# chrischoy/DeepGlobalRegistration

Measured on AMD Instinct MI355X. Metric: pair registrations/sec (FCGF x2 + 1-NN + 6-D inlier net + gate + weighted Procrustes + SE(3) refinement), higher is better.
Workload: dtype f32 results via 2 x f16 split operands (3 f16 MFMA products per MAC, f32 accumulate); k = 1 convs, kNN re-evaluation and registration in exact f32, SVD in f64

## Files before the change

### deepglobalregistration_amd/_lib.py

```python
import ctypes as C
import os
import threading

import torch

_HERE = os.path.dirname(os.path.abspath(__file__))
LIB_PATH = os.environ.get('DGR_HIP_LIB') or os.path.join(_HERE, 'lib', 'libdgr_hip.so')

DGR_OK, DGR_EINVAL, DGR_EHIP, DGR_ENOMEM, DGR_ESVD, DGR_EINTERNAL = 0, -1, -2, -3, -4, -5
STATUS_OK, STATUS_LOW_CONFIDENCE, STATUS_SVD_FAILED, STATUS_SAFEGUARD = 0, 1, 2, 3
STATUS_FLAG_ICP_SKIPPED, STATUS_MASK = 0x100, 0xff

c_i32p, c_i64p, c_f32p, c_f64p = (C.POINTER(C.c_int32), C.POINTER(C.c_int64),
                                  C.POINTER(C.c_float), C.POINTER(C.c_double))
vp = C.c_void_p


class WeightDesc(C.Structure):
    _fields_ = [('name', C.c_char_p), ('data', vp), ('numel', C.c_int64)]


class Params(C.Structure):
    _fields_ = [('clip_weight_thresh', C.c_float), ('voxel_size', C.c_float),
                ('inlier_feature_type', C.c_int), ('max_iter', C.c_int),
                ('max_break_count', C.c_int), ('break_threshold_ratio', C.c_double),
                ('skip_refinement', C.c_int), ('safeguard', C.c_int), ('ransac_hypotheses', C.c_int64),
                ('ransac_seed', C.c_uint32), ('use_icp', C.c_int)]


class PgParams(C.Structure):
    _fields_ = [('mu', C.c_double), ('reference_node', C.c_int), ('max_iter', C.c_int), ('rel_tol', C.c_double)]


SIGNATURES = {
    'dgr_last_error': (C.c_char_p, []),
    'dgr_version': (C.c_char_p, []),
    'dgr_ctx_create': (C.c_int, [C.c_int, C.POINTER(vp)]),
    'dgr_ctx_destroy': (None, [vp]),
    'dgr_ctx_workspace_bytes': (C.c_int64, [vp]),
    'dgr_ctx_create_partition_stream': (C.c_int, [vp, C.c_int, C.c_int, C.POINTER(vp)]),
    'dgr_voxelize': (C.c_int, [vp, vp, C.c_int, C.c_int64, C.c_double, C.c_int32, vp, vp, vp, c_i64p, vp]),
    'dgr_net_create': (C.c_int, [vp, C.c_int, C.c_int, C.c_int, C.c_int, C.c_int,
                                 C.POINTER(WeightDesc), C.c_int, C.POINTER(vp)]),
    'dgr_net_create_device': (C.c_int, [vp, C.c_int, C.c_int, C.c_int, C.c_int, C.c_int,
                                        C.POINTER(WeightDesc), C.c_int, C.POINTER(vp)]),
    'dgr_net_destroy': (None, [vp]),
    'dgr_net_param_bytes': (C.c_int64, [vp]),
    'dgr_net_share': (C.c_int, [vp, vp, C.POINTER(vp)]),
    'dgr_net_sharers': (C.c_int, [vp]),
    'dgr_resunet_forward': (C.c_int, [vp, vp, vp, vp, C.c_int64, vp, vp]),
    'dgr_net_get_intermediate': (C.c_int, [vp, vp, C.c_char_p, vp, C.c_int64, c_i64p, c_i64p]),
    'dgr_net_get_tensor': (C.c_int, [vp, vp, C.c_char_p, C.c_int, vp, C.c_int64, c_i64p, c_i64p]),
    'dgr_net_layer_stats': (C.c_int, [vp, vp, C.c_int, c_i64p]),
    'dgr_net_num_layers': (C.c_int, [vp]),
    'dgr_net_rerun_layer': (C.c_int, [vp, vp, C.c_int, C.c_int, c_f32p, c_f32p]),
    'dgr_maps_create': (C.c_int, [vp, vp, C.c_int64, C.c_int, C.c_int, C.POINTER(vp), vp]),
    'dgr_maps_destroy': (None, [vp]),
    'dgr_maps_get_coords': (C.c_int, [vp, C.c_int, vp, C.c_int64, c_i64p]),
    'dgr_maps_get_kernel_map': (C.c_int, [vp, C.c_int, C.c_int, vp, C.c_int64, vp, vp, C.c_int64,
                                          c_i64p, c_i64p]),
    'dgr_maps_create_ex': (C.c_int, [vp, vp, C.c_int64, C.c_int, C.c_int, C.c_int, C.POINTER(vp), vp]),
    'dgr_maps_get_raw': (C.c_int, [vp, C.c_char_p, C.c_int, C.c_char_p, vp, C.c_int64, c_i64p, c_i64p]),
    'dgr_knn1_l2': (C.c_int, [vp, vp, C.c_int64, vp, C.c_int64, C.c_int, C.c_int, vp, vp, vp]),
    'dgr_knn1_l2_batch': (C.c_int, [vp, vp, c_i64p, vp, c_i64p, C.c_int, C.c_int, C.c_int, vp, vp, vp]),
    'dgr_knn_l2': (C.c_int, [vp, vp, C.c_int64, vp, C.c_int64, C.c_int, C.c_int, C.c_int, vp, vp, vp]),
    'dgr_knn_l2_batch': (C.c_int, [vp, vp, c_i64p, vp, c_i64p, C.c_int, C.c_int, C.c_int, C.c_int, vp, vp,
                                   vp]),
    'dgr_inlier_inputs': (C.c_int, [vp, vp, vp, C.c_int64, vp, vp, C.c_int64, vp, C.c_int, vp, vp, vp]),
    'dgr_sigmoid_clip_sum': (C.c_int, [vp, vp, C.c_int64, C.c_float, vp, c_f64p, vp]),
    'dgr_gather_rows3': (C.c_int, [vp, vp, vp, C.c_int64, vp, vp]),
    'dgr_weighted_procrustes': (C.c_int, [vp, vp, vp, vp, C.c_int64, C.c_float, c_f32p, c_f32p, vp]),
    'dgr_se3_refine': (C.c_int, [vp, vp, vp, vp, C.c_int64, C.c_float, C.c_int, C.c_int, C.c_double,
                                 c_f32p, c_f32p, c_i32p, c_f32p, c_i32p, vp]),
    'dgr_register_batch': (C.c_int, [vp, vp, vp, vp, vp, c_i64p, vp, vp, c_i64p, C.c_int,
                                     C.POINTER(Params), vp, vp, c_f32p, c_i32p, c_f32p, vp]),
    'dgr_register_pairs': (C.c_int, [vp, vp, vp, vp, vp, c_i64p, C.c_int, C.c_int, c_i32p, C.c_int,
                                     C.POINTER(Params), vp, vp, c_f32p, c_i32p, c_f32p, vp]),
    'dgr_register_batch_f64': (C.c_int, [vp, c_f64p, C.c_int64, c_i64p]),
    'dgr_register_batch_output': (C.c_int, [vp, C.c_int, vp, C.c_int64, c_i64p, vp]),
    'dgr_ctx_set_profiling': (C.c_int, [vp, C.c_int]),
    'dgr_icp_point_to_point': (C.c_int, [vp, vp, C.c_int64, vp, C.c_int64, C.c_double, c_f64p, C.c_int, C.c_double,
                                          C.c_double, c_f64p, c_f64p, vp]),
    'dgr_ransac_correspondence': (C.c_int, [vp, vp, vp, C.c_int64, C.c_double, C.c_int64, C.c_uint32, c_f64p, c_f64p, vp]),
    'dgr_ctx_stage_times': (C.c_int, [vp, c_f32p]),
    'dgr_ctx_stage_times_v2': (C.c_int, [vp, c_f32p, C.c_int, C.POINTER(C.c_int)]),
    'dgr_ctx_conv_launches': (C.c_int64, [vp]),
    'dgr_ctx_conv_launch_times': (C.c_int, [vp, c_f32p, c_f32p, C.c_int64, C.POINTER(C.c_int64)]),
    'dgr_ctx_conv_launch_kernel_us': (C.c_int, [vp, c_f32p, C.c_int64, C.POINTER(C.c_int64)]),
    'dgr_ctx_conv_launch_kinds': (C.c_int, [vp, C.c_char_p, C.c_int64, C.POINTER(C.c_int64)]),
    'dgr_radius_pairs_batch': (C.c_int, [vp, vp, c_i64p, vp, c_i64p, C.c_int, c_f64p, C.c_double, C.c_int, vp, vp,
                                         C.c_int64, c_i64p, vp]),
    'dgr_pairs_isin_batch': (C.c_int, [vp, vp, c_i64p, vp, c_i64p, C.c_int, c_i64p, vp, vp]),
    'dgr_validation_counts': (C.c_int, [vp, vp, vp, C.c_float, c_i64p, C.c_int, c_i64p, vp]),
    'dgr_score_pairs': (C.c_int, [vp, vp, c_i64p, C.c_int, c_i32p, C.c_int, c_f64p, C.c_double, c_f64p, vp]),
    'dgr_pose_graph_optimize': (C.c_int, [vp, C.c_int, c_i64p, c_i64p, c_i32p, c_f64p, c_f64p, C.POINTER(C.c_uint8), c_f64p,
                                          C.POINTER(PgParams), c_f64p, c_f64p, c_f64p, vp]),
    'dgr_voxel_mean': (C.c_int, [vp, vp, C.c_int, c_i64p, C.c_int, c_i32p, C.c_int, c_f64p, c_f64p, C.c_double, vp, vp, vp, vp,
                                 vp, c_i64p, c_i64p, vp]),
    'dgr_tsdf_fragment': (C.c_int, [vp, vp, C.c_int, C.c_int, C.c_int, c_f64p, c_f64p, c_f64p, C.c_double, C.c_double,
                                    C.c_double, C.c_double, C.c_int, C.c_int, C.c_int, vp, C.c_int64, vp, vp, vp, C.c_int64,
                                    c_i64p, c_i64p, c_i64p, vp]),
    'dgr_tsdf_mesh': (C.c_int, [vp, vp, C.c_int64, vp, vp, C.c_int, C.c_double, C.c_int, vp, vp, C.c_int64, vp, C.c_int64,
                                c_i64p, c_i64p, vp]),
    'dgr_debug_ortho2rotation': (C.c_int, [vp, vp, C.c_int64, vp, vp, vp, vp]),
    'dgr_debug_se3_refine_from': (C.c_int, [vp, vp, vp, vp, C.c_int64, C.c_float, C.c_int, C.c_int, C.c_double,
                                            c_f64p, c_f64p, vp]),
    'dgr_debug_smooth_l1': (C.c_int, [vp, vp, vp, C.c_int64, C.c_float, vp, vp]),
    'dgr_debug_conv_layer': (C.c_int, [vp, vp, C.c_int, vp, vp, C.c_int, C.c_int64, vp, vp]),
}

_lib = None


def load():
    global _lib
    if _lib is not None:
        return _lib
    if not os.path.exists(LIB_PATH):
        raise RuntimeError(
            f'{LIB_PATH} not found: the HIP extension is not built.  Run '
            '`python -c "import __graft_entry__ as g; g.build()"` (or `make -C '
            'deepglobalregistration_amd/csrc`).  There is no CPU fallback.')
    lib = C.CDLL(LIB_PATH)
    for name, (res, args) in SIGNATURES.items():
        fn = getattr(lib, name)
        fn.restype = res
        fn.argtypes = args
    _lib = lib
    return lib


class DgrError(RuntimeError):
    def __init__(self, code, message):
        super().__init__(f'libdgr_hip error {code}: {message}')
        self.code = code


class DgrInvalidArgument(DgrError, ValueError):

    def __init__(self, message):
        RuntimeError.__init__(self, f'libdgr_hip: {message}')
        self.code = DGR_EINVAL


def check(rc):
    if rc == DGR_OK:
        return
    msg = load().dgr_last_error().decode('utf-8', 'replace')
    if rc == DGR_EINVAL:
        raise DgrInvalidArgument(msg)
    raise DgrError(rc, msg)


_ctxs = {}
_tls = threading.local()


def new_ctx(device):
    lib = load()
    device = torch.device(device)
    idx = device.index if device.index is not None else torch.cuda.current_device()
    h = vp()
    check(lib.dgr_ctx_create(idx, C.byref(h)))
    return h


def use_ctx(handle):
    _tls.ctx = handle


def get_ctx(device=None):
    lib = load()
    if getattr(_tls, 'ctx', None) is not None:
        return _tls.ctx
    if not torch.cuda.is_available():
        raise RuntimeError('deepglobalregistration_amd needs a ROCm GPU (torch.cuda.is_available() is '
                           'False); there is no CPU fallback')
    if device is None:
        idx = torch.cuda.current_device()
    else:
        device = torch.device(device)
        if device.type != 'cuda':
            raise RuntimeError(f'deepglobalregistration_amd runs on the GPU only, got device {device}')
        idx = device.index if device.index is not None else torch.cuda.current_device()
    if idx not in _ctxs:
        h = vp()
        check(lib.dgr_ctx_create(idx, C.byref(h)))
        _ctxs[idx] = h
    return _ctxs[idx]


def stream_ptr(device_index=None):
    return vp(torch.cuda.current_stream(device_index).cuda_stream)


def ptr(t):
    if t is None:
        return vp(0)
    assert t.is_contiguous(), 'tensor must be contiguous'
    return vp(t.data_ptr())
```

### deepglobalregistration_amd/csrc/dgr_internal.h

```cpp
#pragma once
#include <hip/hip_runtime.h>
#include <stdint.h>
#include <stdio.h>
#include <stdlib.h>
#include <string>
#include <vector>

#include "../../include/dgr_hip.h"

void dgr_set_error(const char *fmt, ...);

#define DGR_HIP_CHECK(expr)                                                                  \
  do {                                                                                       \
    hipError_t _e = (expr);                                                                  \
    if (_e != hipSuccess) {                                                                  \
      dgr_set_error("%s:%d: %s failed: %s", __FILE__, __LINE__, #expr, hipGetErrorString(_e)); \
      return DGR_EHIP;                                                                       \
    }                                                                                        \
  } while (0)

#define DGR_CHECK(expr)          \
  do {                           \
    int _r = (expr);             \
    if (_r != DGR_OK) return _r; \
  } while (0)

#define DGR_REQUIRE(cond, ...)     \
  do {                             \
    if (!(cond)) {                 \
      dgr_set_error(__VA_ARGS__);  \
      return DGR_EINVAL;           \
    }                              \
  } while (0)

#define DGR_LAUNCH_CHECK() DGR_HIP_CHECK(hipGetLastError())

inline bool dgr_exact_f32() {
  static const bool on = getenv("DGR_EXACT_F32") != nullptr;
  return on;
}

struct DgrArena {
  struct Chunk {
    char *base;
    size_t size;
  };
  std::vector<Chunk> chunks;
  size_t cur = 0;
  size_t offset = 0;
  size_t high_water = 0, used_total = 0;
  uint64_t generation = 0;

  struct Mark {
    size_t cur, offset, used_total;
  };
  Mark mark() const { return {cur, offset, used_total}; }
  void rewind(const Mark &m) { cur = m.cur; offset = m.offset; used_total = m.used_total; }
  void *alloc(size_t bytes);
  int reset();
  void release();
  size_t reserved() const;
  template <typename T>
  T *get(size_t n) {
    return static_cast<T *>(alloc(n * sizeof(T)));
  }
};

#define DGR_ALLOC(ptr, arena, T, n)                       \
  do {                                                    \
    (ptr) = (arena).get<T>((size_t)(n) > 0 ? (size_t)(n) : 1); \
    if (!(ptr)) return DGR_ENOMEM;                        \
  } while (0)

constexpr int DGR_TILE_M = 64;

struct DgrCoordMap {
  int32_t *coords = nullptr;
  int32_t *n_dev = nullptr;
  int64_t n_cap = 0;
  int ts = 1;
  int32_t *table = nullptr;
  uint32_t table_mask = 0;
  int32_t *canon = nullptr;
};

struct DgrHalfBuckets {
  int32_t *bkeys = nullptr;
  int32_t *table = nullptr;
  uint32_t mask = 0;
  int32_t *start = nullptr;
  int4 *second = nullptr;
  bool built = false;
};

struct DgrKernelMap {
  int K = 0;
  int32_t *rule_ptr = nullptr;
  int32_t *tile_ptr = nullptr;
  int4 *tile_desc = nullptr;
  int64_t tile_cap = 0;
  int32_t *pair_in = nullptr;
  int32_t *pair_out = nullptr;
  int32_t *out_ptr = nullptr, *out_pos = nullptr;
  uint16_t *pair_k = nullptr;
  int32_t *in_ptr = nullptr, *in_pos = nullptr;
  int64_t pair_cap = 0;
  bool built = false;
};

constexpr int DGR_OS_ROWS = 64;
struct DgrNbrTable {
  int32_t *nbr = nullptr;
  int64_t n_pad = 0;
  int K = 27;
  bool built = false;
  int32_t *perm = nullptr, *cls_count = nullptr;
  int64_t cls_cap = 0;
};

struct DgrMapSet {
  int D = 3, nc = 4, conv1_ks = 3;
  bool use_nbr = false;
  DgrNbrTable nsame[4];
  DgrNbrTable ndown[3];
  DgrNbrTable nup[3];
  DgrCoordMap cm[4];
  DgrHalfBuckets hb[4];
  DgrKernelMap same[4];
  DgrKernelMap conv1;
  DgrKernelMap down[3];
  int32_t *overflow = nullptr;
};

int dgr_build_maps(DgrArena &arena, const int32_t *coords, int64_t N, int D, int conv1_ks,
                   DgrMapSet *ms, hipStream_t stream, bool skip_conv1_map = false, bool lean = false,
                   bool nbr_tables = false);
int dgr_nbr_counts(const DgrNbrTable &t, const int32_t *n_out_dev, int64_t counts[27]);
int dgr_conv1_probe(DgrArena &arena, const DgrCoordMap &cm, int ks, const float *in, int in_ld, int cin,
                    const float *w_tiled, const float *shift, float *out, int out_ld, int32_t *pair_count,
                    hipStream_t stream, const float *w_compact = nullptr, const char **kernel_name = nullptr,
                    uint32_t *out_amax = nullptr);
constexpr int32_t DGR_ROW_DROPPED = -1, DGR_ROW_PENDING = -2;
int dgr_unique_rows(DgrArena &arena, const int32_t *keys, int64_t n, int nc, const int32_t *state, int32_t *held,
                    int32_t *first_flag, int32_t *rank, int32_t *n_unique_dev, int32_t **table_out, uint32_t *mask_out,
                    hipStream_t stream);
int dgr_exclusive_scan_i32(DgrArena &arena, const int32_t *in, int32_t *out, int64_t n,
                           int32_t *total_out, hipStream_t stream);
constexpr int DGR_SCAN_MAX = 24;
int dgr_exclusive_scan_multi(DgrArena &arena, int count, const int32_t *const *in, int32_t *const *out, const int64_t *n,
                             int32_t *const *total_out, hipStream_t stream);

struct DgrConvLaunch {
  const float *in;
  int in_ld;
  int in_relu;
  float *out;
  int out_ld;
  float *y;
  const float *shift;
  const float *w;
  int cin, cin_pad, cout, cout_pad, K;
  const int32_t *pair_in, *pair_out, *tile_ptr, *rule_ptr;
  const int4 *tile_desc;
  const int32_t *n_rows_dev;
  int64_t tile_bound;
  int l2_normalize = 0;
  unsigned long long *clk = nullptr;
};
int dgr_conv_launch(const DgrConvLaunch &a, int num_cus, hipStream_t stream, const char **kernel_name = nullptr);
struct DgrSplitRows {
  unsigned char *planes = nullptr;
  float *scale = nullptr;
  int channels = 0;
};
bool dgr_conv_wide_supported(int cin_pad, int cin, int cout);
int dgr_conv_wide_launch(const DgrConvLaunch &a, const DgrSplitRows &in, const void *wb, int64_t piece_stride,
                         float w_unscale, int num_cus, hipStream_t stream, const char **kernel_name = nullptr);
int dgr_row_amax(const float *in, int in_ld, int cin, int relu, const int32_t *n_dev, int64_t n_cap, uint32_t *out,
                 hipStream_t stream);
int dgr_split_rows(const float *in, int in_ld, int relu, const int32_t *n_dev, int64_t n_cap, const DgrSplitRows &out,
                   hipStream_t stream);
int dgr_reduce_rows(const float *y, int cout, const int32_t *ptr, const int32_t *pos, const int32_t *n_dev,
                    int64_t n_cap, float *out, int out_ld, const float *shift, const float *res, int res_ld,
                    int res_relu, hipStream_t stream, const DgrSplitRows *split = nullptr, int out_relu = 0);
int dgr_conv_small_cin(const float *in, int in_ld, int in_relu, int cin, const float *w_tiled, const float *w_quad,
                       const float *shift, const DgrKernelMap &km, const int32_t *n_out_dev, int64_t n_out_cap, float *out,
                       int out_ld, hipStream_t stream);
struct DgrConvOsLaunch {
  const float *in; int in_ld, in_relu;
  float *out; int out_ld, out_relu;
  const float *w16, *shift;
  const void *wb3; int64_t piece_stride;
  const void *wbd = nullptr;
  const uint32_t *row_amax = nullptr; float w_unscale = 1.f;
  uint32_t *out_amax = nullptr, *out_amax2 = nullptr;
  int64_t n_in_cap = 0;
  const float *res; int res_ld, res_relu;
  int rows_per_block;
  int phase_channels = 64;
  const DgrNbrTable *nbr;
  const int32_t *n_out_dev;
  int64_t n_out_cap;
  int cin, cin_pad, cout;
  bool dense = false;
  bool up = false;
  const unsigned char *in_dsplit = nullptr;
  unsigned char *out_dsplit = nullptr;
};
inline bool dgr_fits_32bit_offsets(int64_t rows, int64_t ld) { return rows * ld * 4 < (1ll << 31); }
int dgr_conv_os_launch(const DgrConvOsLaunch &a, hipStream_t stream, const char **kernel_name = nullptr);
bool dgr_conv_dense_supported(int cin, int cin_pad, int cout);
int dgr_conv_dense_launch(const DgrConvOsLaunch &a, hipStream_t stream, const char **kernel_name = nullptr);
bool dgr_conv_up_supported(int cin, int cin_pad, int cout);
int dgr_conv_up_launch(const DgrConvOsLaunch &a, hipStream_t stream, const char **kernel_name = nullptr);
int dgr_l2_normalize_rows(const float *in, int in_ld, float *out, int out_ld, int c, int relu,
                          const int32_t *n_dev, int64_t n_cap, hipStream_t stream);

struct DgrBatchOutputs {
  const void *ptr[5] = {nullptr, nullptr, nullptr, nullptr, nullptr};
  int64_t numel[5] = {0, 0, 0, 0, 0};
  uint64_t generation = 0;
};

struct DgrEventPool {
  std::vector<hipEvent_t> ev;
  size_t used = 0;
  hipEvent_t next();
  void release();
};

struct dgr_ctx {
  int device = 0;
  int num_cus = 256;
  DgrArena arena;
  bool profiling = false;
  float stage_ms[9] = {0, 0, 0, 0, 0, 0, 0, 0, 0};
  int64_t conv_launches = 0;
  DgrBatchOutputs last;
  std::vector<double> last_T64;
  DgrEventPool events;
  std::vector<std::pair<hipEvent_t, hipEvent_t>> conv_spans, gemm_spans, map3_spans, map6_spans;
  std::vector<float> conv_span_ms, gemm_span_ms;
  std::vector<unsigned long long *> conv_clks;
  std::vector<float> conv_clk_us;
  std::vector<const char *> conv_kinds;
  int32_t *flag_dev = nullptr;
  hipEvent_t wait_ev = nullptr;
  long last_wait_ns = 0;
  double batch_ns_per_row = 0;
  double pairs_ns_per_row = 0;
  unsigned char *pin = nullptr;
  size_t pin_bytes = 0;
  hipStream_t part_stream = nullptr;
  int all_cus = 256;
};

int dgr_ctx_pinned(dgr_ctx *ctx, size_t bytes, unsigned char **out);
int dgr_flag_error(int32_t flag);

int dgr_ctx_wait(dgr_ctx *ctx, hipStream_t stream, long predicted_ns = 0);

int dgr_resunet_forward_impl(dgr_ctx *ctx, dgr_net *net, const int32_t *coords, const float *feats,
                             int64_t N, float *out, hipStream_t stream);
int dgr_ctx_collect_profile(dgr_ctx *ctx);
void dgr_ctx_begin_profile(dgr_ctx *ctx);

int dgr_knn1_batch_impl(dgr_ctx *ctx, const float *F0, const int64_t *off0, const float *F1, const int64_t *off1,
                        int npairs, int C, int squared, int64_t *idx_out, float *dist_out, hipStream_t stream);
int dgr_knn1_impl(dgr_ctx *ctx, const float *F0, int64_t N0, const float *F1, int64_t N1, int C,
                  int squared, int64_t *idx_out, float *dist_out, hipStream_t stream);
int dgr_inlier_inputs_impl(const int32_t *coords0, const float *xyz0, int64_t N0,
                           const int32_t *coords1, const float *xyz1, const int64_t *idx1,
                           int feature_type, int32_t *coords6, float *feats, hipStream_t stream);
int dgr_icp_impl(dgr_ctx *ctx, const float *src, int64_t N0, const float *dst, int64_t N1, double max_dist,
                 const double *T_init, int max_iter, double rel_fitness, double rel_rmse, double *T_out,
                 double *stats_out, hipStream_t stream);
int dgr_ransac_impl(dgr_ctx *ctx, const float *X, const float *Y, int64_t N, double max_dist, int64_t num_hypotheses,
                    uint32_t seed, double *T_out, double *stats_out, hipStream_t stream);
struct DgrIcpJob {
  const float *src = nullptr, *dst = nullptr;
  int64_t N0 = 0, N1 = 0;
  double max_dist = 0;
  int nblocks = 0;
  void *st = nullptr;
  double *P = nullptr, *sorted = nullptr, *partial = nullptr;
  int32_t ncell = 0;
  double host_state[64];
};
int dgr_icp_begin(dgr_ctx *ctx, const float *src, int64_t N0, const float *dst, int64_t N1, double max_dist,
                  const double *T_init_dev , DgrIcpJob *job, hipStream_t stream);
int dgr_icp_run(dgr_ctx *ctx, DgrIcpJob *job, int max_iter, double rel_fitness, double rel_rmse, hipStream_t stream);
void dgr_icp_finish(const DgrIcpJob *job, double *T_out, double *stats_out);
constexpr int DGR_RANSAC_RESULT_DOUBLES = 19;
int dgr_ransac_begin(dgr_ctx *ctx, const float *X, const float *Y, int64_t N, double max_dist, int64_t num_hypotheses,
                     uint32_t seed, double **result_dev, hipStream_t stream);
struct DgrRegResult {
  float R[9];
  float t[3];
  float loss;
  float wsum;
  int32_t iterations;
  int32_t break_count;
  int32_t status;
  int32_t pad;
};
static inline int64_t dgr_ceil_div(int64_t a, int64_t b) { return (a + b - 1) / b; }
```

### deepglobalregistration_amd/csrc/kmap.hip

```cpp
#include <string.h>

#include <algorithm>

#include "dgr_internal.h"
#include "hash.h"

constexpr int KM_THREADS = 256;

template <int D>
__device__ __forceinline__ void offset_of(int k, int ks, int ts, int32_t *delta) {
  const int half = ks >> 1;
#pragma unroll
  for (int d = 0; d < D; ++d) {
    delta[d] = ((k % ks) - half) * ts;
    k /= ks;
  }
}

template <int D>
__device__ __forceinline__ int probe(const int32_t *__restrict__ out_coords, int64_t o,
                                     const int32_t *delta, const int32_t *__restrict__ in_coords,
                                     const int32_t *__restrict__ in_table, uint32_t in_mask) {
  constexpr int NC = D + 1;
  int32_t q[NC];
// ... 504 lines not shown
}

struct Kmap6Job {
  const DgrCoordMap *in, *out;
  const DgrHalfBuckets *hb;
  const DgrHalfBuckets *hb_out;
  bool need_in_csr, want_pair_out, want_pair_k;
  DgrKernelMap *km;
};
static int build_kernel_maps6(DgrArena &arena, const Kmap6Job *jobs, int nj, int max_pairs_per_row, int32_t *overflow,
                              hipStream_t stream) {
  constexpr int K = 729, KW = (K + 31) / 32;
  DGR_REQUIRE(nj >= 1 && nj <= KM_MAXJOBS, "6-D kernel maps: %d jobs", nj);
  struct Tr {
    int RB, symmetric;
    int64_t n_cap, n_in_cap, hit_waves;
    int32_t *counts, *base, *total, *cnt_out, *cnt_in;
    uint32_t *mask_out, *mask_in;
    int4 *cell;
    HitList hl;
    unsigned short *wpre_out, *wpre_in;
  } t[KM_MAXJOBS];
  for (int m = 0; m < nj; ++m) {
    const Kmap6Job &J = jobs[m];
    t[m].n_cap = J.out->n_cap; t[m].n_in_cap = J.in->n_cap;
    DGR_REQUIRE(t[m].n_cap < (1ll << 27) && t[m].n_in_cap < (1ll << 27), "6-D kernel maps: more than 2^27 rows");
    DGR_CHECK(alloc_kernel_map(arena, K, t[m].n_cap, t[m].n_in_cap, max_pairs_per_row, J.need_in_csr, J.want_pair_out,
                               J.want_pair_k, J.km));
  }
  DgrArena::Mark mk = arena.mark();
  {
    size_t words = 0;
    for (int m = 0; m < nj; ++m)
      words += (size_t)(t[m].n_cap + 1) * KW + (jobs[m].need_in_csr ? (size_t)(t[m].n_in_cap + 1) * KW : 0) + (size_t)(t[m].n_cap + 1);
    uint32_t *pool;
    DGR_ALLOC(pool, arena, uint32_t, words);
    DGR_HIP_CHECK(hipMemsetAsync(pool, 0, words * sizeof(uint32_t), stream));
    for (int m = 0; m < nj; ++m) {
      t[m].mask_out = pool; pool += (size_t)(t[m].n_cap + 1) * KW;
      t[m].mask_in = nullptr;
      if (jobs[m].need_in_csr) { t[m].mask_in = pool; pool += (size_t)(t[m].n_in_cap + 1) * KW; }
      t[m].cnt_out = reinterpret_cast<int32_t *>(pool); pool += (size_t)(t[m].n_cap + 1);
    }
  }
  for (int m = 0; m < nj; ++m) {
    const Kmap6Job &J = jobs[m];
    Tr &r = t[m];
    r.RB = (int)dgr_ceil_div(r.n_cap, KM_THREADS);
    r.symmetric = (J.in->coords == J.out->coords && !J.need_in_csr) ? 1 : 0;
    DGR_REQUIRE(J.hb && J.hb->built && J.hb_out && J.hb_out->built, "6-D kernel map: first-half buckets missing");
    DGR_ALLOC(r.counts, arena, int32_t, (int64_t)K * r.RB);
    DGR_ALLOC(r.base, arena, int32_t, (int64_t)K * r.RB);
    DGR_ALLOC(r.total, arena, int32_t, 1);
    r.cnt_in = nullptr;
    if (J.need_in_csr) DGR_ALLOC(r.cnt_in, arena, int32_t, r.n_in_cap + 1);
    DGR_ALLOC(r.cell, arena, int4, (int64_t)r.RB * (KM_THREADS / 64) * K);
    const int64_t search_blocks = dgr_ceil_div(r.n_cap * (r.symmetric ? 14 : 27), KM_THREADS);
    r.hit_waves = search_blocks * (KM_THREADS / 64);
    r.hl.region = (J.in->ts >= 8 && r.symmetric) ? 2 * KM_REGION : KM_REGION / 2;
    DGR_REQUIRE(r.hit_waves < (1ll << 31), "6-D kernel map: too many search waves");
    DGR_ALLOC(r.hl.recs, arena, unsigned long long, r.hit_waves * r.hl.region);
    DGR_ALLOC(r.hl.wave_count, arena, int32_t, r.hit_waves);
    DGR_ALLOC(r.wpre_out, arena, unsigned short, (r.n_cap + 1) * KW);
    r.wpre_in = nullptr;
    if (J.need_in_csr) DGR_ALLOC(r.wpre_in, arena, unsigned short, (r.n_in_cap + 1) * KW);
  }
  static_assert(KM_JOBS6 >= KM_MAXJOBS, "multi-job launch tables");
  {
    Bits6Jobs bj = {};
    Colmask6Jobs cj = {};
    int max_sb = 0, max_rb = 0;
    for (int m = 0; m < nj; ++m) {
      const Kmap6Job &J = jobs[m];
      Tr &r = t[m];
      bj.pa[m] = PrunedArgs{J.out->coords, J.out->n_dev, J.hb_out->second, r.n_cap, *J.hb, J.in->ts, r.symmetric};
      bj.mask_out[m] = r.mask_out; bj.mask_in[m] = r.mask_in; bj.hl[m] = r.hl;
      bj.blocks[m] = (int)(r.hit_waves / (KM_THREADS / 64));
      max_sb = std::max(max_sb, bj.blocks[m]);
      cj.mask_out[m] = r.mask_out; cj.n_out_dev[m] = J.out->n_dev; cj.RB[m] = r.RB; cj.cell[m] = r.cell;
      cj.counts[m] = r.counts; cj.row_cnt[m] = r.cnt_out; cj.wpre[m] = r.wpre_out;
      max_rb = std::max(max_rb, r.RB);
    }
    kmap_bits_pruned6<<<dim3((unsigned)max_sb, (unsigned)nj), KM_THREADS, 0, stream>>>(bj, KW);
    kmap_colmask<<<dim3((unsigned)max_rb, (unsigned)nj), KM_THREADS, 0, stream>>>(cj, K, KW);
    {
      MaskCountJobs mj = {};
      int nm = 0;
      long long max_rows = 0;
      for (int m = 0; m < nj; ++m)
        if (jobs[m].need_in_csr) {
          mj.mask[nm] = t[m].mask_in; mj.n_dev[nm] = jobs[m].in->n_dev; mj.n_cap[nm] = t[m].n_in_cap + 1;
          mj.cnt[nm] = t[m].cnt_in; mj.wpre[nm] = t[m].wpre_in;
          max_rows = std::max(max_rows, mj.n_cap[nm]);
          ++nm;
        }
      static_assert(KM_MC_JOBS >= KM_MAXJOBS, "mask-count job table");
      if (nm) mask_count_multi<KW><<<dim3((unsigned)dgr_ceil_div(max_rows, 256), (unsigned)nm), 256, 0, stream>>>(mj);
    }
  }
  DGR_LAUNCH_CHECK();
  {
    const int32_t *ins[DGR_SCAN_MAX];
    int32_t *outs[DGR_SCAN_MAX], *tots[DGR_SCAN_MAX];
    int64_t ns[DGR_SCAN_MAX];
    int c = 0;
    for (int m = 0; m < nj; ++m) {
      ins[c] = t[m].cnt_out; outs[c] = jobs[m].km->out_ptr; tots[c] = nullptr; ns[c++] = t[m].n_cap + 1;
      ins[c] = t[m].counts; outs[c] = t[m].base; tots[c] = t[m].total; ns[c++] = (int64_t)K * t[m].RB;
      if (jobs[m].need_in_csr) { ins[c] = t[m].cnt_in; outs[c] = jobs[m].km->in_ptr; tots[c] = nullptr; ns[c++] = t[m].n_in_cap + 1; }
    }
    DGR_CHECK(dgr_exclusive_scan_multi(arena, c, ins, outs, ns, tots, stream));
  }
  FinalizeJobs fj = {};
  int64_t max_tiles = 0;
  for (int m = 0; m < nj; ++m) {
    finalize_job(fj, m, t[m].base, t[m].total, K, t[m].RB, jobs[m].km);
    max_tiles = std::max<int64_t>(max_tiles, jobs[m].km->tile_cap);
  }
  kmap_finalize<<<nj, 1024, 0, stream>>>(fj);
  tile_desc_kernel<<<dim3((unsigned)dgr_ceil_div(max_tiles, 256), nj), 256, 0, stream>>>(fj);
  {
    Place6Jobs pj = {};
    int max_pb = 0;
    for (int m = 0; m < nj; ++m) {
      const Kmap6Job &J = jobs[m];
      Tr &r = t[m];
      DgrKernelMap *km = J.km;
      pj.p[m] = PlaceArgs{K, KW, r.RB, r.mask_out, km->out_ptr, r.cell, r.base, km->pair_in, km->pair_out, km->pair_k, km->out_pos,
                          km->pair_cap, overflow, r.mask_in, km->in_ptr, km->in_pos, r.wpre_out, r.wpre_in};
      pj.replay[m] = PrunedArgs{J.out->coords, J.out->n_dev, J.hb_out->second, r.n_cap, *J.hb, J.in->ts, r.symmetric};
      pj.h[m] = r.hl;
      pj.n_waves[m] = (int)r.hit_waves;
      pj.blocks[m] = (int)std::min<int64_t>(dgr_ceil_div(r.hit_waves, KM_THREADS / 64), 16384);
      max_pb = std::max(max_pb, pj.blocks[m]);
      km->built = true;
    }
    kmap_place_hits<<<dim3((unsigned)max_pb, (unsigned)nj), KM_THREADS, 0, stream>>>(pj);
  }
  DGR_LAUNCH_CHECK();
  arena.rewind(mk);
  return DGR_OK;
}

constexpr int NBR_JOBS = 10;
struct NbrJobs {
  const int32_t *out_coords[NBR_JOBS], *n_out_dev[NBR_JOBS], *in_coords[NBR_JOBS], *in_table[NBR_JOBS];
  uint32_t in_mask[NBR_JOBS];
  int ts[NBR_JOBS];
  long long n_pad[NBR_JOBS];
  int32_t *nbr[NBR_JOBS];
};
__global__ void __launch_bounds__(KM_THREADS) nbr_search3(NbrJobs J) {
  const int jm = blockIdx.z;
  const int64_t n_pad = J.n_pad[jm];
  const int64_t o = (int64_t)blockIdx.x * KM_THREADS + threadIdx.x;
  if (o >= n_pad) return;
  int32_t *__restrict__ nbr = J.nbr[jm];
  const int kz = blockIdx.y;
  if (o >= *J.n_out_dev[jm]) {
#pragma unroll
    for (int u = 0; u < 9; ++u) nbr[(int64_t)(9 * kz + u) * n_pad + o] = -1;
    return;
  }
  const int sts = J.ts[jm];
  const int4 c = *reinterpret_cast<const int4 *>(J.out_coords[jm] + o * 4);
  int32_t q[9][4];
#pragma unroll
  for (int u = 0; u < 9; ++u) {
    q[u][0] = c.x;
    q[u][1] = c.y + ((u % 3) - 1) * sts;
    q[u][2] = c.z + ((u / 3) - 1) * sts;
    q[u][3] = c.w + (kz - 1) * sts;
  }
  int hit[9];
  dgr_lookup_many<4, 9>(J.in_table[jm], J.in_mask[jm], J.in_coords[jm], q, hit);
#pragma unroll
  for (int u = 0; u < 9; ++u) nbr[(int64_t)(9 * kz + u) * n_pad + o] = hit[u];
}

struct ClsJobs {
  const int32_t *coords[3], *n_dev[3];
  int ts[3], nb[3];
  int32_t *blk_cnt[3], *perm[3], *cls_count[3];
  long long cls_cap[3];
};
__device__ __forceinline__ int parity_class(const int32_t *coords, int64_t o, int ts) {
  const int4 c = *reinterpret_cast<const int4 *>(coords + o * 4);
  return ((c.y / ts) & 1) | (((c.z / ts) & 1) << 1) | (((c.w / ts) & 1) << 2);
}
__global__ void __launch_bounds__(KM_THREADS) cls_count_kernel(ClsJobs J) {
  __shared__ int wcnt[KM_THREADS / 64][8];
  const int l = blockIdx.y, b = blockIdx.x;
  if (b >= J.nb[l]) return;
  const int64_t o = (int64_t)b * KM_THREADS + threadIdx.x;
  const int cls = o < *J.n_dev[l] ? parity_class(J.coords[l], o, J.ts[l]) : 8;
#pragma unroll
  for (int c = 0; c < 8; ++c) {
    const unsigned long long m = __ballot(cls == c);
    if ((threadIdx.x & 63) == 0) wcnt[threadIdx.x >> 6][c] = __popcll(m);
  }
  __syncthreads();
  if (threadIdx.x < 8) {
    int n = 0;
    for (int w = 0; w < KM_THREADS / 64; ++w) n += wcnt[w][threadIdx.x];
    J.blk_cnt[l][b * 8 + threadIdx.x] = n;
  }
}
__global__ void __launch_bounds__(KM_THREADS) cls_fill_kernel(ClsJobs J) {
  __shared__ int part[KM_THREADS / 64][8], before[8], wcnt[KM_THREADS / 64][8];
  const int l = blockIdx.y, b = blockIdx.x;
  if (b >= J.nb[l]) return;
  const int lane = threadIdx.x & 63, wave = threadIdx.x >> 6;
  int acc[8] = {0, 0, 0, 0, 0, 0, 0, 0};
  for (int bb = threadIdx.x; bb < b; bb += KM_THREADS) {
    const int4 lo = *reinterpret_cast<const int4 *>(J.blk_cnt[l] + bb * 8), hi = *reinterpret_cast<const int4 *>(J.blk_cnt[l] + bb * 8 + 4);
    acc[0] += lo.x; acc[1] += lo.y; acc[2] += lo.z; acc[3] += lo.w;
    acc[4] += hi.x; acc[5] += hi.y; acc[6] += hi.z; acc[7] += hi.w;
  }
#pragma unroll
  for (int c = 0; c < 8; ++c) {
    int v = acc[c];
    for (int d = 32; d > 0; d >>= 1) v += __shfl_down(v, d, 64);
    if (lane == 0) part[wave][c] = v;
  }
  const int64_t o = (int64_t)b * KM_THREADS + threadIdx.x;
  const int cls = o < *J.n_dev[l] ? parity_class(J.coords[l], o, J.ts[l]) : 8;
  int rank = 0;
#pragma unroll
  for (int c = 0; c < 8; ++c) {
    const unsigned long long m = __ballot(cls == c);
    if (lane == 0) wcnt[wave][c] = __popcll(m);
    if (cls == c) rank = __popcll(m & ((1ull << lane) - 1ull));
  }
  __syncthreads();
  if (threadIdx.x < 8) {
    int n = 0;
    for (int w = 0; w < KM_THREADS / 64; ++w) n += part[w][threadIdx.x];
    before[threadIdx.x] = n;
    if (b == J.nb[l] - 1) {
      for (int w = 0; w < KM_THREADS / 64; ++w) n += wcnt[w][threadIdx.x];
      J.cls_count[l][threadIdx.x] = n;
    }
  }
  __syncthreads();
  if (cls < 8) {
    int pos = before[cls] + rank;
    for (int w = 0; w < wave; ++w) pos += wcnt[w][cls];
    J.perm[l][(int64_t)cls * J.cls_cap[l] + pos] = (int32_t)o;
  }
}

static int build_nbr_table(DgrArena &arena, const DgrCoordMap &in, const DgrCoordMap &out, int ts, int sign,
                           DgrNbrTable *t, NbrJobs *jobs, int *nj, int32_t *cls_count = nullptr) {
  t->K = 27;
  t->n_pad = dgr_ceil_div(out.n_cap, DGR_OS_ROWS) * DGR_OS_ROWS;
  DGR_ALLOC(t->nbr, arena, int32_t, t->n_pad * 27);
  t->perm = nullptr; t->cls_count = nullptr; t->cls_cap = 0;
  if (cls_count) {
    t->cls_cap = t->n_pad;
    t->cls_count = cls_count;
    DGR_ALLOC(t->perm, arena, int32_t, 8 * t->cls_cap);
  }
  DGR_REQUIRE(*nj < NBR_JOBS, "neighbour tables: more than %d per launch", NBR_JOBS);
  const int m = (*nj)++;
  jobs->out_coords[m] = out.coords; jobs->n_out_dev[m] = out.n_dev; jobs->in_coords[m] = in.coords;
  jobs->in_table[m] = in.table; jobs->in_mask[m] = in.table_mask; jobs->ts[m] = sign > 0 ? ts : -ts;
  jobs->n_pad[m] = t->n_pad; jobs->nbr[m] = t->nbr;
  t->built = true;
  return DGR_OK;
}
static int nbr_tables_launch(const NbrJobs &jobs, int nj, hipStream_t stream) {
  long long n_max = 0;
  for (int m = 0; m < nj; ++m) n_max = std::max(n_max, jobs.n_pad[m]);
  if (nj == 0) return DGR_OK;
  nbr_search3<<<dim3((unsigned)dgr_ceil_div(n_max, KM_THREADS), 3, (unsigned)nj), KM_THREADS, 0, stream>>>(jobs);
  DGR_LAUNCH_CHECK();
  return DGR_OK;
}

__global__ void nbr_count_kernel(const int32_t *__restrict__ nbr, int64_t n_pad, const int32_t *n_out_dev,
                                 unsigned long long *__restrict__ counts) {
  const int k = blockIdx.y;
  const int n = *n_out_dev;
  int c = 0;
  for (int64_t o = (int64_t)blockIdx.x * blockDim.x + threadIdx.x; o < n; o += (int64_t)gridDim.x * blockDim.x)
    c += nbr[(int64_t)k * n_pad + o] >= 0;
  for (int d = 32; d > 0; d >>= 1) c += __shfl_down(c, d, 64);
  if ((threadIdx.x & 63) == 0 && c) atomicAdd(&counts[k], (unsigned long long)c);
}

int dgr_nbr_counts(const DgrNbrTable &t, const int32_t *n_out_dev, int64_t counts[27]) {
  unsigned long long *dev;
  DGR_HIP_CHECK(hipMalloc((void **)&dev, 27 * sizeof(unsigned long long)));
  DGR_HIP_CHECK(hipMemset(dev, 0, 27 * sizeof(unsigned long long)));
  nbr_count_kernel<<<dim3(64, 27), 256>>>(t.nbr, t.n_pad, n_out_dev, dev);
  unsigned long long host[27];
  hipError_t e = hipMemcpy(host, dev, sizeof(host), hipMemcpyDeviceToHost);
  (void)hipFree(dev);
  DGR_HIP_CHECK(e);
  for (int k = 0; k < 27; ++k) counts[k] = (int64_t)host[k];
  return DGR_OK;
}

int dgr_build_coord_maps(DgrArena &arena, const int32_t *coords, int64_t N, DgrMapSet *ms,
                         hipStream_t stream);
int dgr_build_half_buckets(DgrArena &arena, DgrCoordMap *cm, DgrHalfBuckets *hb, int levels, int renumber_from, hipStream_t stream);

int dgr_build_maps(DgrArena &arena, const int32_t *coords, int64_t N, int D, int conv1_ks,
                   DgrMapSet *ms, hipStream_t stream, bool skip_conv1_map, bool lean, bool nbr_tables) {
  DGR_REQUIRE(D == 3 || D == 6, "D=%d not supported (the DGR path uses D=3 and D=6)", D);
  DGR_REQUIRE(conv1_ks % 2 == 1 && conv1_ks >= 1, "conv1 kernel size must be odd");
  DGR_REQUIRE(N > 0 && N < (1ll << 30), "N=%lld out of range", (long long)N);
  ms->D = D;
  ms->nc = D + 1;
  ms->conv1_ks = conv1_ks;
  if (!ms->overflow) {
    DGR_ALLOC(ms->overflow, arena, int32_t, 1);
    DGR_HIP_CHECK(hipMemsetAsync(ms->overflow, 0, sizeof(int32_t), stream));
  }
  DGR_CHECK(dgr_build_coord_maps(arena, coords, N, ms, stream));
  if (nbr_tables) {
    DGR_REQUIRE(D == 3, "neighbour tables are a D = 3 structure");
    ms->use_nbr = true;
    NbrJobs nbj = {};
    int n_nbj = 0;
    int32_t *cls;
    DGR_ALLOC(cls, arena, int32_t, 3 * 8);
    for (int l = 0; l < 4; ++l) DGR_CHECK(build_nbr_table(arena, ms->cm[l], ms->cm[l], ms->cm[l].ts, +1, &ms->nsame[l], &nbj, &n_nbj));
    for (int l = 0; l < 3; ++l) {
      DGR_CHECK(build_nbr_table(arena, ms->cm[l], ms->cm[l + 1], ms->cm[l].ts, +1, &ms->ndown[l], &nbj, &n_nbj));
      DGR_CHECK(build_nbr_table(arena, ms->cm[l + 1], ms->cm[l], ms->cm[l].ts, -1, &ms->nup[l], &nbj, &n_nbj, cls + 8 * l));
    }
    DGR_CHECK(nbr_tables_launch(nbj, n_nbj, stream));
    {
      ClsJobs cj = {};
      int max_nb = 0;
      for (int l = 0; l < 3; ++l) {
        cj.coords[l] = ms->cm[l].coords; cj.n_dev[l] = ms->cm[l].n_dev; cj.ts[l] = ms->cm[l].ts;
        cj.nb[l] = (int)dgr_ceil_div(ms->cm[l].n_cap, KM_THREADS);
        DGR_ALLOC(cj.blk_cnt[l], arena, int32_t, (int64_t)cj.nb[l] * 8);
        cj.perm[l] = ms->nup[l].perm; cj.cls_count[l] = ms->nup[l].cls_count; cj.cls_cap[l] = ms->nup[l].cls_cap;
        max_nb = std::max(max_nb, cj.nb[l]);
      }
      cls_count_kernel<<<dim3((unsigned)max_nb, 3), KM_THREADS, 0, stream>>>(cj);
      cls_fill_kernel<<<dim3((unsigned)max_nb, 3), KM_THREADS, 0, stream>>>(cj);
      DGR_LAUNCH_CHECK();
    }
    if (lean) {
      if (conv1_ks != 3 && !skip_conv1_map)
        DGR_CHECK(build_kernel_map3(arena, ms->cm[0], ms->cm[0], conv1_ks, 1024, false, false, true, &ms->conv1, ms->overflow,
                                    stream));
      return DGR_OK;
    }
  }
  const int cap_row = (D == 3) ? 1024 : 160;
  if (D == 6) {
    DGR_REQUIRE(conv1_ks == 3, "6-D kernel maps support kernel size 3 only (got %d)", conv1_ks);
    DGR_CHECK(dgr_build_half_buckets(arena, ms->cm, ms->hb, 4, 1, stream));
    Kmap6Job jobs[7];
    for (int l = 0; l < 4; ++l) jobs[l] = {&ms->cm[l], &ms->cm[l], &ms->hb[l], &ms->hb[l], false, !lean, !lean || l == 0, &ms->same[l]};
    for (int l = 0; l < 3; ++l) jobs[4 + l] = {&ms->cm[l], &ms->cm[l + 1], &ms->hb[l], &ms->hb[l + 1], true, true, !lean, &ms->down[l]};
    DGR_CHECK(build_kernel_maps6(arena, jobs, 7, cap_row, ms->overflow, stream));
    ms->conv1 = ms->same[0];
    return DGR_OK;
  }
  auto build = [&](const DgrCoordMap &in, const DgrCoordMap &out, int ks, bool rev, bool want_k, DgrKernelMap *km) -> int {
    const bool want_out = !lean || rev, want_pk = !lean || want_k;
    return build_kernel_map3(arena, in, out, ks, cap_row, rev, want_out, want_pk, km, ms->overflow, stream);
  };
  for (int l = 0; l < 4; ++l) DGR_CHECK(build(ms->cm[l], ms->cm[l], 3, false, l == 0, &ms->same[l]));
  if (conv1_ks == 3)
    ms->conv1 = ms->same[0];
  else if (!skip_conv1_map)
    DGR_CHECK(build(ms->cm[0], ms->cm[0], conv1_ks, false, true, &ms->conv1));
  for (int l = 0; l < 3; ++l) DGR_CHECK(build(ms->cm[l], ms->cm[l + 1], 3, true, false, &ms->down[l]));
  return DGR_OK;
}

struct dgr_maps {
  dgr_ctx *ctx;
  DgrArena arena;
  DgrMapSet ms;
  int32_t *coords_copy = nullptr;
  hipStream_t stream;
};

static int maps_create(dgr_ctx *ctx, const int32_t *coords, int64_t N, int D, int conv1_kernel_size, int flags,
                       dgr_maps **out, dgr_stream stream_) {
  DGR_REQUIRE(ctx && coords && out, "dgr_maps_create: NULL argument");
  DGR_REQUIRE((flags & ~DGR_MAPS_LEAN) == 0, "dgr_maps_create_ex: unknown flags 0x%x", flags);
  const bool lean = (flags & DGR_MAPS_LEAN) != 0;
  const bool skip_conv1_map = lean && D == 3;
  hipStream_t stream = (hipStream_t)stream_;
  DGR_HIP_CHECK(hipSetDevice(ctx->device));
  dgr_maps *m = new dgr_maps();
  m->ctx = ctx;
  m->stream = stream;
  int rc = DGR_OK;
  do {
    m->coords_copy = m->arena.get<int32_t>((size_t)N * (D + 1));
    if (!m->coords_copy) { rc = DGR_ENOMEM; break; }
    if (hipMemcpyAsync(m->coords_copy, coords, (size_t)N * (D + 1) * sizeof(int32_t),
                       hipMemcpyDeviceToDevice, stream) != hipSuccess) { rc = DGR_EHIP; break; }
    rc = dgr_build_maps(m->arena, m->coords_copy, N, D, conv1_kernel_size, &m->ms, stream, skip_conv1_map, lean, D == 3);
    if (rc != DGR_OK) break;
    int32_t flag = 0;
    if (hipMemcpyAsync(&flag, m->ms.overflow, sizeof(int32_t), hipMemcpyDeviceToHost, stream) != hipSuccess ||
        hipStreamSynchronize(stream) != hipSuccess) { rc = DGR_EHIP; dgr_set_error("maps sync failed"); break; }
    if (flag == 1) { dgr_set_error("duplicate coordinates in the sparse tensor input"); rc = DGR_EINVAL; break; }
    if (flag == 2) { dgr_set_error("kernel-map capacity exceeded"); rc = DGR_ENOMEM; break; }
  } while (0);
  if (rc != DGR_OK) {
    m->arena.release();
    delete m;
    return rc;
  }
  *out = m;
  return DGR_OK;
}

extern "C" int dgr_maps_create(dgr_ctx *ctx, const int32_t *coords, int64_t N, int D,
                               int conv1_kernel_size, dgr_maps **out, dgr_stream stream_) {
  return maps_create(ctx, coords, N, D, conv1_kernel_size, 0, out, stream_);
}

extern "C" int dgr_maps_create_ex(dgr_ctx *ctx, const int32_t *coords, int64_t N, int D, int conv1_kernel_size,
                                  int flags, dgr_maps **out, dgr_stream stream_) {
  return maps_create(ctx, coords, N, D, conv1_kernel_size, flags, out, stream_);
}

extern "C" void dgr_maps_destroy(dgr_maps *m) {
  if (!m) return;
  (void)hipDeviceSynchronize();
  m->arena.release();
  delete m;
}

static int level_of(int ts) { return ts == 1 ? 0 : ts == 2 ? 1 : ts == 4 ? 2 : ts == 8 ? 3 : -1; }

extern "C" int dgr_maps_get_coords(dgr_maps *m, int ts, int32_t *host_out, int64_t capacity,
                                   int64_t *n) {
  DGR_REQUIRE(m && n, "NULL argument");
  int l = level_of(ts);
  DGR_REQUIRE(l >= 0, "tensor stride %d not in {1,2,4,8}", ts);
  int32_t n32 = 0;
  DGR_HIP_CHECK(hipMemcpy(&n32, m->ms.cm[l].n_dev, sizeof(int32_t), hipMemcpyDeviceToHost));
  *n = n32;
  if (host_out) {
    DGR_REQUIRE(capacity >= (int64_t)n32 * m->ms.nc, "host buffer too small");
    const int nc = m->ms.nc;
    if (!m->ms.cm[l].canon) {
      DGR_HIP_CHECK(hipMemcpy(host_out, m->ms.cm[l].coords, (size_t)n32 * nc * sizeof(int32_t), hipMemcpyDeviceToHost));
    } else {
      std::vector<int32_t> tmp((size_t)n32 * nc), canon(n32);
      DGR_HIP_CHECK(hipMemcpy(tmp.data(), m->ms.cm[l].coords, tmp.size() * sizeof(int32_t), hipMemcpyDeviceToHost));
      DGR_HIP_CHECK(hipMemcpy(canon.data(), m->ms.cm[l].canon, canon.size() * sizeof(int32_t), hipMemcpyDeviceToHost));
      for (int32_t p = 0; p < n32; ++p) memcpy(host_out + (size_t)canon[p] * nc, tmp.data() + (size_t)p * nc, nc * sizeof(int32_t));
    }
  }
  return DGR_OK;
}

extern "C" int dgr_maps_get_kernel_map(dgr_maps *m, int kind, int ts, int32_t *rule_ptr,
                                       int64_t rule_cap, int32_t *pair_in, int32_t *pair_out,
                                       int64_t pair_cap, int64_t *K, int64_t *P) {
  DGR_REQUIRE(m && K && P, "NULL argument");
  int l = level_of(ts);
  DGR_REQUIRE(l >= 0, "tensor stride %d not in {1,2,4,8}", ts);
  if (kind >= 3 && kind <= 5) {
    const DgrNbrTable *t = kind == 3 ? &m->ms.nsame[l] : (l < 3 ? (kind == 4 ? &m->ms.ndown[l] : &m->ms.nup[l]) : nullptr);
    DGR_REQUIRE(t && t->built, "no such neighbour table (kind %d, ts %d)", kind, ts);
    const DgrCoordMap &om = kind == 4 ? m->ms.cm[l + 1] : m->ms.cm[l];
    int32_t n_out = 0;
    DGR_HIP_CHECK(hipMemcpy(&n_out, om.n_dev, sizeof(int32_t), hipMemcpyDeviceToHost));
    std::vector<int32_t> tab((size_t)t->n_pad * 27);
    DGR_HIP_CHECK(hipMemcpy(tab.data(), t->nbr, tab.size() * sizeof(int32_t), hipMemcpyDeviceToHost));
    *K = 27;
    int64_t total = 0;
    for (int k = 0; k < 27; ++k) {
      if (rule_ptr && k < rule_cap) rule_ptr[k] = (int32_t)total;
      for (int o = 0; o < n_out; ++o) {
        const int32_t v = tab[(size_t)k * t->n_pad + o];
        if (v < 0) continue;
        if (pair_in && pair_out) {
          DGR_REQUIRE(total < pair_cap, "pair buffers too small");
          pair_in[total] = v;
          pair_out[total] = o;
        }
        ++total;
      }
    }
    if (rule_ptr) {
      DGR_REQUIRE(rule_cap >= 28, "rule_ptr buffer too small");
      rule_ptr[27] = (int32_t)total;
    }
    for (int64_t o = n_out; o < t->n_pad; ++o)
      for (int k = 0; k < 27; ++k) DGR_REQUIRE(tab[(size_t)k * t->n_pad + o] == -1, "neighbour table padding is not -1");
    *P = total;
    return DGR_OK;
  }
  const DgrKernelMap *km = nullptr;
  if (kind == 0) km = &m->ms.same[l];
  else if (kind == 1) km = &m->ms.conv1;
  else if (kind == 2 && l < 3) km = &m->ms.down[l];
  DGR_REQUIRE(km && km->built, "no such kernel map (kind %d, ts %d)", kind, ts);
  *K = km->K;
  int32_t total = 0;
  DGR_HIP_CHECK(hipMemcpy(&total, km->rule_ptr + km->K, sizeof(int32_t), hipMemcpyDeviceToHost));
  *P = total;
  if (rule_ptr) {
    DGR_REQUIRE(rule_cap >= km->K + 1, "rule_ptr buffer too small");
    DGR_HIP_CHECK(hipMemcpy(rule_ptr, km->rule_ptr, (size_t)(km->K + 1) * sizeof(int32_t),
                            hipMemcpyDeviceToHost));
  }
  if (pair_in && pair_out) {
    DGR_REQUIRE(pair_cap >= total, "pair buffers too small");
    DGR_REQUIRE(km->pair_out, "this build kept no pair_out for the map (kind %d, ts %d): read it raw", kind, ts);
    DGR_HIP_CHECK(hipMemcpy(pair_in, km->pair_in, (size_t)total * sizeof(int32_t), hipMemcpyDeviceToHost));
    DGR_HIP_CHECK(hipMemcpy(pair_out, km->pair_out, (size_t)total * sizeof(int32_t), hipMemcpyDeviceToHost));
    const DgrCoordMap &cin = m->ms.cm[l], &cout = m->ms.cm[kind == 2 ? l + 1 : l];
    if (cin.canon || cout.canon) {
      auto fetch = [&](const DgrCoordMap &c, std::vector<int32_t> &v) -> int {
        if (!c.canon) return DGR_OK;
        int32_t n = 0;
        DGR_HIP_CHECK(hipMemcpy(&n, c.n_dev, sizeof(int32_t), hipMemcpyDeviceToHost));
        v.resize(n);
        DGR_HIP_CHECK(hipMemcpy(v.data(), c.canon, (size_t)n * sizeof(int32_t), hipMemcpyDeviceToHost));
        return DGR_OK;
      };
      std::vector<int32_t> ci, co, rp(km->K + 1);
      DGR_CHECK(fetch(cin, ci));
      DGR_CHECK(fetch(cout, co));
      DGR_HIP_CHECK(hipMemcpy(rp.data(), km->rule_ptr, rp.size() * sizeof(int32_t), hipMemcpyDeviceToHost));
      std::vector<std::pair<int32_t, int32_t>> tmp;
      for (int k = 0; k < km->K; ++k) {
        tmp.clear();
        for (int32_t q = rp[k]; q < rp[k + 1]; ++q)
          tmp.push_back({cout.canon ? co[pair_out[q]] : pair_out[q], cin.canon ? ci[pair_in[q]] : pair_in[q]});
        std::sort(tmp.begin(), tmp.end());
        for (size_t u = 0; u < tmp.size(); ++u) { pair_out[rp[k] + u] = tmp[u].first; pair_in[rp[k] + u] = tmp[u].second; }
      }
    }
  }
  return DGR_OK;
}

extern "C" int dgr_maps_get_raw(dgr_maps *m, const char *kind, int ts, const char *field, void *host_out,
                                int64_t capacity_bytes, int64_t *count, int64_t *elem_bytes) {
  DGR_REQUIRE(m && kind && field && count && elem_bytes, "dgr_maps_get_raw: NULL argument");
  const int l = level_of(ts);
  DGR_REQUIRE(l >= 0, "tensor stride %d not in {1,2,4,8}", ts);
  DGR_HIP_CHECK(hipSetDevice(m->ctx->device));
  DGR_HIP_CHECK(hipStreamSynchronize(m->stream));
  const DgrMapSet &ms = m->ms;
  const auto is = [](const char *a, const char *b) { return strcmp(a, b) == 0; };
  const void *dev = nullptr;
  int64_t n = 0, eb = 4;
  bool scalar = false;
  int64_t value = 0;
  const auto rows_of = [](const DgrCoordMap &c, int64_t *rows) -> int {
    int32_t n32 = 0;
    DGR_HIP_CHECK(hipMemcpy(&n32, c.n_dev, sizeof(int32_t), hipMemcpyDeviceToHost));
    *rows = n32;
    return DGR_OK;
  };
  if (is(kind, "level")) {
    const DgrCoordMap &c = ms.cm[l];
    int64_t rows = 0;
    DGR_CHECK(rows_of(c, &rows));
    if (is(field, "coords")) { dev = c.coords; n = rows * ms.nc; }
    else if (is(field, "canon")) {
      DGR_REQUIRE(c.canon, "level ts %d is not renumbered: it has no canon", ts);
      dev = c.canon; n = rows;
    }
    else if (is(field, "table")) { dev = c.table; n = (int64_t)c.table_mask + 1; }
    else if (is(field, "n")) { scalar = true; value = rows; }
    else if (is(field, "mask")) { scalar = true; value = c.table_mask; }
    else DGR_REQUIRE(false, "no field '%s' in a level", field);
  } else if (is(kind, "same") || is(kind, "conv1") || is(kind, "down")) {
    const bool down = is(kind, "down");
    DGR_REQUIRE(!down || l < 3, "no strided map at ts %d", ts);
    DGR_REQUIRE(!is(kind, "conv1") || l == 0, "the conv1 map lives at ts 1");
    const DgrKernelMap *km = down ? &ms.down[l] : is(kind, "conv1") ? &ms.conv1 : &ms.same[l];
    DGR_REQUIRE(km->built, "this build made no '%s' map at ts %d", kind, ts);
    const DgrCoordMap &cin = ms.cm[l], &cout = ms.cm[down ? l + 1 : l];
    int32_t tot[2] = {0, 0};
    DGR_HIP_CHECK(hipMemcpy(&tot[0], km->rule_ptr + km->K, sizeof(int32_t), hipMemcpyDeviceToHost));
    DGR_HIP_CHECK(hipMemcpy(&tot[1], km->tile_ptr + km->K, sizeof(int32_t), hipMemcpyDeviceToHost));
    const int64_t P = std::min<int64_t>(std::max<int64_t>(tot[0], 0), km->pair_cap);
    const int64_t T = std::min<int64_t>(std::max<int64_t>(tot[1], 0), km->tile_cap);
    if (is(field, "rule_ptr")) { dev = km->rule_ptr; n = km->K + 1; }
    else if (is(field, "tile_ptr")) { dev = km->tile_ptr; n = km->K + 1; }
    else if (is(field, "tile_desc")) { dev = km->tile_desc; n = 4 * T; }
    else if (is(field, "pair_in")) { dev = km->pair_in; n = P; }
    else if (is(field, "pair_out")) {
      DGR_REQUIRE(km->pair_out, "this build kept no pair_out for the '%s' map at ts %d", kind, ts);
      dev = km->pair_out; n = P;
    }
    else if (is(field, "pair_k")) {
      DGR_REQUIRE(km->pair_k, "this build kept no pair_k for the '%s' map at ts %d", kind, ts);
      dev = km->pair_k; n = P; eb = 2;
    }
    else if (is(field, "out_ptr")) { dev = km->out_ptr; n = cout.n_cap + 1; }
    else if (is(field, "out_pos")) { dev = km->out_pos; n = P; }
    else if (is(field, "in_ptr") || is(field, "in_pos")) {
      DGR_REQUIRE(km->in_ptr && km->in_pos, "the '%s' map at ts %d has no in-major CSR", kind, ts);
      if (is(field, "in_ptr")) { dev = km->in_ptr; n = cin.n_cap + 1; } else { dev = km->in_pos; n = P; }
    }
    else if (is(field, "pair_cap")) { scalar = true; value = km->pair_cap; }
    else if (is(field, "n_cap")) { scalar = true; value = cout.n_cap; }
    else if (is(field, "K")) { scalar = true; value = km->K; }
    else DGR_REQUIRE(false, "no field '%s' in a kernel map", field);
  } else if (is(kind, "nbr_same") || is(kind, "nbr_down") || is(kind, "nbr_up")) {
    DGR_REQUIRE(is(kind, "nbr_same") || l < 3, "no such neighbour table at ts %d", ts);
    const DgrNbrTable *t = is(kind, "nbr_same") ? &ms.nsame[l] : is(kind, "nbr_down") ? &ms.ndown[l] : &ms.nup[l];
    DGR_REQUIRE(t->built, "this build made no '%s' table at ts %d", kind, ts);
    if (is(field, "nbr")) { dev = t->nbr; n = t->n_pad * t->K; }
    else if (is(field, "n_pad")) { scalar = true; value = t->n_pad; }
    else if (is(field, "perm") || is(field, "cls_count") || is(field, "cls_cap")) {
      DGR_REQUIRE(t->perm && t->cls_count, "the '%s' table at ts %d has no parity classes", kind, ts);
      if (is(field, "perm")) { dev = t->perm; n = 8 * t->cls_cap; }
      else if (is(field, "cls_count")) { dev = t->cls_count; n = 8; }
      else { scalar = true; value = t->cls_cap; }
    }
    else DGR_REQUIRE(false, "no field '%s' in a neighbour table", field);
  } else {
    DGR_REQUIRE(false, "no kind '%s'", kind);
  }
  if (scalar) { n = 1; eb = 8; }
  *count = n;
  *elem_bytes = eb;
  if (!host_out) return DGR_OK;
  DGR_REQUIRE(capacity_bytes >= n * eb, "host buffer too small (%lld < %lld bytes)", (long long)capacity_bytes, (long long)(n * eb));
  if (scalar) {
    memcpy(host_out, &value, sizeof(int64_t));
  } else if (n > 0) {
    DGR_REQUIRE(dev, "field '%s' of '%s' at ts %d was not built", field, kind, ts);
    DGR_HIP_CHECK(hipMemcpy(host_out, dev, (size_t)(n * eb), hipMemcpyDeviceToHost));
  }
  return DGR_OK;
}
```

### deepglobalregistration_amd/csrc/net.hip

```cpp
#include <math.h>
#include <stdlib.h>
#include <string.h>

#include <algorithm>
#include <map>
#include <memory>
#include <string>

#include "dgr_internal.h"

static const int CH[5] = {0, 32, 64, 128, 256};
static const int TR[5] = {0, 64, 64, 64, 128};
static constexpr float BN_EPS = 1e-5f;

struct DgrLayer {
  std::string name;
  int K, cin, cout, cin_pad, cout_pad;
  float *w = nullptr;
  float *w16 = nullptr;
  void *w16b = nullptr;
  void *w16d = nullptr;
  int64_t w16b_piece = 0;
  float *wc = nullptr;
  float *wq = nullptr;
  void *wb = nullptr;
  int64_t wb_piece = 0;
  float w_unscale = 1.f;
  float *shift = nullptr;
};

struct LayerRun {
  const int32_t *rule_ptr = nullptr;
  const int32_t *n_in = nullptr, *n_out = nullptr;
  int K = 1;
  DgrConvLaunch launch;
  DgrSplitRows split_in, split_out;
  int out_relu = 0;
  bool split_only = false;
  bool small_cin = false;
  const int32_t *fused_pairs = nullptr;
  bool os = false;
  DgrConvOsLaunch os_launch;
  DgrNbrTable nbr;
  DgrKernelMap km;
  bool has_reduce = false;
  const int32_t *red_ptr = nullptr, *red_pos = nullptr;
  int64_t n_out_cap = 0;
  const float *res = nullptr;
  int res_ld = 0, res_relu = 0;
};

struct DgrTensorRef {
  const float *ptr = nullptr;
  int ld = 0, cols = 0;
  const int32_t *n_dev = nullptr;
  const int32_t *canon = nullptr;
};

struct DgrTensorRec {
  const float *f32 = nullptr;
  int ld = 0, cols = 0;
  const uint32_t *amax = nullptr;
  const unsigned char *planes = nullptr;
  const float *scale = nullptr;
  const unsigned char *dsplit = nullptr;
  const int32_t *n_dev = nullptr, *canon = nullptr;
};

struct DgrWeights {
  std::vector<DgrLayer> layers;
  std::vector<void *> allocs;
  int64_t param_bytes = 0;
  int device = 0;
  template <class T> int alloc(T **p, size_t n) {
    DGR_HIP_CHECK(hipMalloc((void **)p, n * sizeof(T)));
    allocs.push_back(*p);
    return DGR_OK;
  }
  ~DgrWeights() {
    int cur = -1;
    (void)hipGetDevice(&cur);
    (void)hipSetDevice(device);
    (void)hipDeviceSynchronize();
    for (void *p : allocs) (void)hipFree(p);
    if (cur >= 0 && cur != device) (void)hipSetDevice(cur);
  }
};

struct dgr_net {
  dgr_ctx *ctx;
  int D, cin, cout, conv1_ks, normalize;
  std::shared_ptr<DgrWeights> W;
  LayerRun runs[23];
  std::map<std::string, DgrTensorRef> inter;
  std::map<std::string, DgrTensorRec> tensors;
  uint64_t run_generation = 0;
};

static int round_up(int v, int m) { return (v + m - 1) / m * m; }

static const dgr_weight_desc *find_desc(const dgr_weight_desc *w, int n, const std::string &name) {
  for (int i = 0; i < n; ++i)
    if (name == w[i].name) return &w[i];
  return nullptr;
}

template <class F>
__global__ void __launch_bounds__(256) dgr_fill_kernel(int64_t n, F f) {
  for (int64_t o = (int64_t)blockIdx.x * 256 + threadIdx.x; o < n; o += (int64_t)gridDim.x * 256) f(o);
}
template <class F>
static int dgr_fill(hipStream_t s, int64_t n, F f) {
  if (n <= 0) return DGR_OK;
  const int64_t blocks = std::min<int64_t>((n + 255) / 256, 1 << 16);
  dgr_fill_kernel<<<(int)blocks, 256, 0, s>>>(n, f);
  DGR_LAUNCH_CHECK();
  return DGR_OK;
}
__device__ __forceinline__ uint16_t dgr_f16_bits_dev(float x) {
  const _Float16 h = (_Float16)x;
  return __builtin_bit_cast(uint16_t, h);
}
__device__ __forceinline__ float dgr_f16_val_dev(float x) { return (float)(_Float16)x; }
__global__ void __launch_bounds__(256) dgr_absmax_scaled_kernel(const float *__restrict__ w, const float *__restrict__ scale,
                                                                int64_t n, int cout, uint32_t *out_bits) {
  float mx = 0.f;
  for (int64_t o = (int64_t)blockIdx.x * 256 + threadIdx.x; o < n; o += (int64_t)gridDim.x * 256)
    mx = fmaxf(mx, fabsf(__fmul_rn(w[o], scale[o % cout])));
  for (int d = 32; d > 0; d >>= 1) mx = fmaxf(mx, __shfl_xor(mx, d, 64));
  if ((threadIdx.x & 63) == 0) atomicMax(out_bits, __float_as_uint(mx));
}

struct WeightPrep {
  bool dev;
  hipStream_t s = nullptr;
  float *sc = nullptr;
  uint32_t *mxb = nullptr;
  float *staging = nullptr;
  size_t staging_n = 0;
  ~WeightPrep() {
    if (s) (void)hipStreamSynchronize(s);
    (void)hipFree(sc); (void)hipFree(mxb); (void)hipFree(staging);
    if (s) (void)hipStreamDestroy(s);
  }
};

static int make_layer(dgr_net *net, WeightPrep &P, const dgr_weight_desc *descs, int nd, const std::string &name, int K,
                      int cin, int cout, const char *bn, bool bias) {
  DgrLayer L;
  L.name = name;
  L.K = K; L.cin = cin; L.cout = cout;
  L.cin_pad = round_up(cin, 8);
  L.cout_pad = cout <= 32 ? 32 : cout <= 64 ? 64 : cout <= 128 ? 128 : 256;
  if (L.cout_pad == 32 && L.cin_pad > 8) {
    DGR_REQUIRE(cin <= 64, "%s: %d input channels (at most 64 into a 32-channel layer)", name.c_str(), cin);
    L.cin_pad = cin <= 32 ? 32 : 64;
  }
  DGR_REQUIRE(cout <= 256 && cin <= 256, "%s: channel count above 256 not supported", name.c_str());
  const dgr_weight_desc *kd = find_desc(descs, nd, name + ".kernel");
  DGR_REQUIRE(kd != nullptr, "state_dict is missing '%s.kernel'", name.c_str());
  DGR_REQUIRE(kd->numel == (int64_t)K * cin * cout, "'%s.kernel' has %lld elements, expected %d x %d x %d",
              name.c_str(), (long long)kd->numel, K, cin, cout);
  std::vector<float> scale(cout, 1.f), shift(cout, 0.f);
  bool has_shift = false;
  std::vector<std::vector<float>> small;
  auto host_of = [&](const dgr_weight_desc *d) -> const float * {
    if (!P.dev) return d->data;
    small.emplace_back((size_t)d->numel);
    if (hipMemcpy(small.back().data(), d->data, (size_t)d->numel * sizeof(float), hipMemcpyDeviceToHost) != hipSuccess) return nullptr;
    return small.back().data();
  };
  if (bn) {
    std::string p = std::string(bn) + ".bn.";
    const dgr_weight_desc *g = find_desc(descs, nd, p + "weight"), *b = find_desc(descs, nd, p + "bias"),
                          *m = find_desc(descs, nd, p + "running_mean"),
                          *v = find_desc(descs, nd, p + "running_var");
    DGR_REQUIRE(g && b && m && v, "state_dict is missing batch-norm tensors '%s*'", p.c_str());
    DGR_REQUIRE(g->numel == cout && b->numel == cout && m->numel == cout && v->numel == cout,
                "batch-norm '%s' has the wrong width", p.c_str());
    const float *gd = host_of(g), *bd2 = host_of(b), *md = host_of(m), *vd = host_of(v);
    DGR_REQUIRE(gd && bd2 && md && vd, "batch-norm '%s': device tensors could not be read", p.c_str());
    for (int c = 0; c < cout; ++c) {
      float s = gd[c] / sqrtf(vd[c] + BN_EPS);
      scale[c] = s;
      shift[c] = bd2[c] - md[c] * s;
    }
    has_shift = true;
  }
  if (bias) {
    const dgr_weight_desc *bd = find_desc(descs, nd, name + ".bias");
    DGR_REQUIRE(bd && bd->numel == cout, "state_dict is missing '%s.bias' [1,%d]", name.c_str(), cout);
    const float *bh = host_of(bd);
    DGR_REQUIRE(bh, "'%s.bias': device tensor could not be read", name.c_str());
    for (int c = 0; c < cout; ++c) shift[c] += bh[c];
    has_shift = true;
  }
  DgrWeights &W = *net->W;
  hipStream_t s = P.s;
  const float *src = kd->data;
  if (!P.dev) {
    const size_t n = (size_t)kd->numel;
    if (n > P.staging_n) {
      DGR_HIP_CHECK(hipStreamSynchronize(s));
      DGR_HIP_CHECK(hipFree(P.staging));
      P.staging = nullptr;
      DGR_HIP_CHECK(hipMalloc((void **)&P.staging, n * sizeof(float)));
      P.staging_n = n;
    }
    DGR_HIP_CHECK(hipMemcpyAsync(P.staging, kd->data, n * sizeof(float), hipMemcpyHostToDevice, s));
    src = P.staging;
  }
  const float *sc = P.sc;
  DGR_HIP_CHECK(hipMemcpyAsync(P.sc, scale.data(), (size_t)cout * sizeof(float), hipMemcpyHostToDevice, s));
  if (has_shift) {
    DGR_CHECK(W.alloc(&L.shift, cout));
    DGR_HIP_CHECK(hipMemcpyAsync(L.shift, shift.data(), (size_t)cout * sizeof(float), hipMemcpyHostToDevice, s));
  }
  const int64_t nw = (int64_t)K * cin * cout;
  DGR_HIP_CHECK(hipMemsetAsync(P.mxb, 0, sizeof(uint32_t), s));
  dgr_absmax_scaled_kernel<<<(int)std::min<int64_t>((nw + 255) / 256, 4096), 256, 0, s>>>(src, sc, nw, cout, P.mxb);
  DGR_LAUNCH_CHECK();
  uint32_t bits = 0;
  DGR_HIP_CHECK(hipMemcpyAsync(&bits, P.mxb, sizeof(bits), hipMemcpyDeviceToHost, s));
  DGR_HIP_CHECK(hipStreamSynchronize(s));
  float mx;
  memcpy(&mx, &bits, 4);
  int ex = 0;
  if (mx > 0.f && std::isfinite(mx)) (void)frexpf(mx, &ex);
  ex = std::min(std::max(ex, -100), 100);
  const float w_scale = ldexpf(1.f, 15 - ex);
  L.w_unscale = ldexpf(1.f, ex - 15);
  const bool use_wide = K > 1 && !dgr_exact_f32() && dgr_conv_wide_supported(L.cin_pad, cin, cout) && !(net->D == 3 && K == 27);
  if (use_wide) {
    const int S16 = cin / 16, NB32 = cout / 32;
    L.wb_piece = (int64_t)K * S16 * NB32 * 64;
    const int64_t ne = L.wb_piece * 8;
    uint16_t *dst;
    DGR_CHECK(W.alloc(&dst, (size_t)2 * ne));
    L.wb = dst;
    DGR_CHECK(dgr_fill(s, ne, [=] __device__(int64_t o) {
      const int e = (int)(o & 7), lane = (int)((o >> 3) & 63);
      const int64_t r = o >> 9;
      const int nb = (int)(r % NB32), s2 = (int)((r / NB32) % S16), k = (int)(r / ((int64_t)NB32 * S16));
      const int col = 32 * nb + (lane & 31), row = 16 * s2 + 8 * (lane >> 5) + e;
      const float xs = __fmul_rn(__fmul_rn(src[((size_t)k * cin + row) * cout + col], sc[col]), w_scale);
      dst[o] = dgr_f16_bits_dev(xs);
      dst[ne + o] = dgr_f16_bits_dev(xs - dgr_f16_val_dev(xs));
    }));
    W.param_bytes += (size_t)2 * ne * sizeof(uint16_t);
  } else {
    const int S = L.cin_pad / 8, NBLK = L.cout_pad / 32;
    const int64_t ne = (int64_t)K * S * NBLK * 256;
    DGR_CHECK(W.alloc(&L.w, ne));
    float *const dst = L.w;
    DGR_CHECK(dgr_fill(s, ne, [=] __device__(int64_t o) {
      const int c = (int)(o & 3), lane = (int)((o >> 2) & 63);
      const int64_t r = o >> 8;
      const int nb = (int)(r % NBLK), s2 = (int)((r / NBLK) % S), k = (int)(r / ((int64_t)NBLK * S));
      const int row = 8 * s2 + 4 * (lane >> 5) + c, col = 32 * nb + (lane & 31);
      dst[o] = (row < cin && col < cout) ? __fmul_rn(src[((size_t)k * cin + row) * cout + col], sc[col]) : 0.f;
    }));
    W.param_bytes += (size_t)ne * sizeof(float);
  }
  if (net->D == 3 && K == 27 && L.cin_pad % 16 == 0 && cout % 32 == 0) {
    const int GT = L.cin_pad / 16, NB = cout / 16;
    {
      const int64_t ne = (int64_t)K * GT * NB * 256;
      DGR_CHECK(W.alloc(&L.w16, ne));
      float *const dst = L.w16;
      DGR_CHECK(dgr_fill(s, ne, [=] __device__(int64_t o) {
        const int c = (int)(o & 3), lane = (int)((o >> 2) & 63);
        const int64_t r = o >> 8;
        const int jb = (int)(r % NB), g = (int)((r / NB) % GT), k = (int)(r / ((int64_t)NB * GT));
        const int col = 16 * jb + (lane & 15), row = 16 * g + 4 * (lane >> 4) + c;
        dst[o] = row < cin ? __fmul_rn(src[((size_t)k * cin + row) * cout + col], sc[col]) : 0.f;
      }));
      W.param_bytes += (size_t)ne * sizeof(float);
    }
    if (cin % 32 == 0) {
      const int S32 = cin / 32;
      L.w16b_piece = (int64_t)K * S32 * NB * 64;
      const int64_t ne = L.w16b_piece * 8;
      uint16_t *pcs;
      DGR_CHECK(W.alloc(&pcs, (size_t)2 * ne));
      L.w16b = pcs;
      DGR_CHECK(dgr_fill(s, ne, [=] __device__(int64_t o) {
        const int e = (int)(o & 7), lane = (int)((o >> 3) & 63);
        const int64_t r = o >> 9;
        const int jb = (int)(r % NB), sI = (int)((r / NB) % S32), k = (int)(r / ((int64_t)NB * S32));
        const int col = 16 * jb + (lane & 15), row = 32 * sI + 8 * (lane >> 4) + e;
        const float xs = __fmul_rn(__fmul_rn(src[((size_t)k * cin + row) * cout + col], sc[col]), w_scale);
        pcs[o] = dgr_f16_bits_dev(xs);
        pcs[ne + o] = dgr_f16_bits_dev(xs - dgr_f16_val_dev(xs));
      }));
      W.param_bytes += (size_t)2 * ne * sizeof(uint16_t);
      if (net->D == 3 && K == 27 && (dgr_conv_dense_supported(cin, L.cin_pad, cout) || dgr_conv_up_supported(cin, L.cin_pad, cout))) {
        uint16_t *pd;
        DGR_CHECK(W.alloc(&pd, (size_t)2 * ne));
        L.w16d = pd;
        DGR_CHECK(dgr_fill(s, 2 * ne, [=] __device__(int64_t o) {
          const int e = (int)(o & 3), h = (int)((o >> 2) & 1);
          const int64_t f = o >> 3, base = f & ~(int64_t)63;
          const int lane = (int)(f & 63), col = lane & 15, lq = lane >> 4;
          const int64_t srcf = base + col + 16 * ((lq >> 1) + 2 * h);
          pd[o] = pcs[srcf * 8 + 4 * (lq & 1) + e];
        }));
        W.param_bytes += (size_t)2 * ne * sizeof(uint16_t);
      }
    }
  }
  if (net->D == 3 && name == "conv1" && cin == 1 && cout == 32 && K <= 343) {
    int ks = 1;
    while (ks * ks * ks < K) ++ks;
    const int ks2 = ks * ks, steps = (ks2 + 3) / 4;
    const int64_t ne = (int64_t)ks * steps * 128;
    DGR_CHECK(W.alloc(&L.wc, ne));
    float *const dst = L.wc;
    DGR_CHECK(dgr_fill(s, ne, [=] __device__(int64_t o) {
      const int j = (int)(o & 1), lane = (int)((o >> 1) & 63);
      const int64_t r = o >> 7;
      const int s2 = (int)(r % steps), kz = (int)(r / steps);
      const int kk = 4 * s2 + (lane >> 4), col = (lane & 15) + 16 * j;
      dst[o] = kk < ks2 ? __fmul_rn(src[(size_t)(kz * ks2 + kk) * cout + col], sc[col]) : 0.f;
    }));
  }
  if (name == "conv1" && cin == 6 && cout == 32 && K > 1) {
    const int64_t ne = (int64_t)K * 192;
    DGR_CHECK(W.alloc(&L.wq, ne));
    float *const dst = L.wq;
    DGR_CHECK(dgr_fill(s, ne, [=] __device__(int64_t o) {
      const int e = (int)(o & 3), q = (int)((o >> 2) & 3);
      const int i = (int)((o >> 4) % 12), k = (int)(o / 192);
      const int ci = i >> 1, co = 8 * q + 4 * (i & 1) + e;
      dst[o] = __fmul_rn(src[((size_t)k * cin + ci) * cout + co], sc[co]);
    }));
    W.param_bytes += (size_t)ne * sizeof(float);
  }
  W.layers.push_back(L);
  return DGR_OK;
}

static int net_create(dgr_ctx *ctx, int D, int in_channels, int out_channels, int conv1_kernel_size, int normalize_feature,
                      const dgr_weight_desc *weights, int n_weights, dgr_net **out, bool dev) {
  DGR_REQUIRE(ctx && weights && out, "dgr_net_create: NULL argument");
  if (dev) {
    for (int i = 0; i < n_weights; ++i) {
      hipPointerAttribute_t at;
      const hipError_t e = hipPointerGetAttributes(&at, weights[i].data);
      if (e != hipSuccess) (void)hipGetLastError();
      DGR_REQUIRE(e == hipSuccess && at.type == hipMemoryTypeDevice && at.device == ctx->device,
                  "dgr_net_create_device: '%s' is not a device pointer on device %d (use dgr_net_create for host tensors)",
                  weights[i].name ? weights[i].name : "?", ctx->device);
    }
  }
  DGR_REQUIRE(D == 3 || D == 6, "dgr_net_create: D=%d (ResUNetBN2C is used with D=3 and D=6)", D);
  DGR_REQUIRE(in_channels >= 1 && in_channels <= 256 && out_channels >= 1 && out_channels <= 64,
              "dgr_net_create: unsupported channel counts in=%d out=%d", in_channels, out_channels);
  DGR_REQUIRE(conv1_kernel_size % 2 == 1, "conv1 kernel size must be odd");
  DGR_HIP_CHECK(hipSetDevice(ctx->device));
  WeightPrep P{dev};
  DGR_HIP_CHECK(hipStreamCreate(&P.s));
  DGR_HIP_CHECK(hipMalloc((void **)&P.sc, 256 * sizeof(float)));
  DGR_HIP_CHECK(hipMalloc((void **)&P.mxb, sizeof(uint32_t)));
  dgr_net *net = new dgr_net();
  net->ctx = ctx;
  net->W = std::make_shared<DgrWeights>();
  net->W->device = ctx->device;
  net->D = D; net->cin = in_channels; net->cout = out_channels;
  net->conv1_ks = conv1_kernel_size; net->normalize = normalize_feature;
  int k3 = 1, k1 = 1;
  for (int d = 0; d < D; ++d) { k3 *= 3; k1 *= conv1_kernel_size; }
  int rc = DGR_OK;
  auto L = [&](const std::string &name, int K, int ci, int co, const char *bn, bool bias = false) {
    if (rc == DGR_OK) rc = make_layer(net, P, weights, n_weights, name, K, ci, co, bn, bias);
  };
  auto block = [&](const std::string &b, int c) {
    L(b + ".conv1", k3, c, c, (b + ".norm1").c_str());
    L(b + ".conv2", k3, c, c, (b + ".norm2").c_str());
  };
  L("conv1", k1, in_channels, CH[1], "norm1");          block("block1", CH[1]);
  L("conv2", k3, CH[1], CH[2], "norm2");                block("block2", CH[2]);
  L("conv3", k3, CH[2], CH[3], "norm3");                block("block3", CH[3]);
  L("conv4", k3, CH[3], CH[4], "norm4");                block("block4", CH[4]);
  L("conv4_tr", k3, CH[4], TR[4], "norm4_tr");          block("block4_tr", TR[4]);
  L("conv3_tr", k3, CH[3] + TR[4], TR[3], "norm3_tr");  block("block3_tr", TR[3]);
  L("conv2_tr", k3, CH[2] + TR[3], TR[2], "norm2_tr");  block("block2_tr", TR[2]);
  L("conv1_tr", 1, CH[1] + TR[2], TR[1], nullptr);
  L("final", 1, TR[1], out_channels, nullptr, true);
  if (rc == DGR_OK) rc = [&] { DGR_HIP_CHECK(hipStreamSynchronize(P.s)); return DGR_OK; }();
  if (rc != DGR_OK) {
    dgr_net_destroy(net);
    return rc;
  }
  *out = net;
  return DGR_OK;
}

extern "C" int dgr_net_create(dgr_ctx *ctx, int D, int in_channels, int out_channels,
                              int conv1_kernel_size, int normalize_feature,
                              const dgr_weight_desc *weights, int n_weights, dgr_net **out) {
  return net_create(ctx, D, in_channels, out_channels, conv1_kernel_size, normalize_feature, weights, n_weights, out, false);
}

extern "C" int dgr_net_create_device(dgr_ctx *ctx, int D, int in_channels, int out_channels,
                                     int conv1_kernel_size, int normalize_feature,
                                     const dgr_weight_desc *weights, int n_weights, dgr_net **out) {
  return net_create(ctx, D, in_channels, out_channels, conv1_kernel_size, normalize_feature, weights, n_weights, out, true);
}

extern "C" void dgr_net_destroy(dgr_net *net) {
  if (!net) return;
  delete net;
}

extern "C" int dgr_net_share(dgr_ctx *ctx, const dgr_net *src, dgr_net **out) {
  DGR_REQUIRE(ctx && src && out, "dgr_net_share: NULL argument");
  DGR_REQUIRE(ctx->device == src->W->device, "dgr_net_share: the weights live on device %d, the context on device %d",
              src->W->device, ctx->device);
  dgr_net *net = new dgr_net();
  net->ctx = ctx;
  net->D = src->D; net->cin = src->cin; net->cout = src->cout;
  net->conv1_ks = src->conv1_ks; net->normalize = src->normalize;
  net->W = src->W;
  *out = net;
  return DGR_OK;
}

extern "C" int dgr_net_sharers(const dgr_net *net) { return net ? (int)net->W.use_count() : 0; }
extern "C" int64_t dgr_net_param_bytes(const dgr_net *net) { return net ? net->W->param_bytes : 0; }
extern "C" int dgr_net_num_layers(const dgr_net *net) { return net ? (int)net->W->layers.size() : 0; }

struct Tensor {
  float *ptr;
  int ld;
  int relu;
  DgrSplitRows split;
  bool split_only = false;
  uint32_t *amax = nullptr, *amax2 = nullptr;
  unsigned char *dsplit = nullptr;
  bool dsplit_only = false;
};

struct Fwd {
  dgr_ctx *ctx;
  dgr_net *net;
  hipStream_t stream;
  DgrMapSet ms;
  bool prof;
  bool l2_next = false;

  float *ybuf = nullptr;

  int conv(int li, const Tensor &in, const DgrKernelMap *km, bool swapped, int lvl_in, int lvl_out,
           const Tensor &out, const Tensor *res) {
    const DgrLayer &L = net->W->layers[li];
    const DgrCoordMap &cin_map = ms.cm[lvl_in], &cout_map = ms.cm[lvl_out];
    DgrConvLaunch a;
    a.in = in.ptr; a.in_ld = in.ld; a.in_relu = in.relu;
    a.out = out.ptr; a.out_ld = out.ld;
    a.y = ybuf; a.shift = L.shift;
    a.w = L.w;
    a.cin = L.cin; a.cin_pad = L.cin_pad; a.cout = L.cout; a.cout_pad = L.cout_pad; a.K = L.K;
    if (km && ms.use_nbr) {
      a.pair_in = a.pair_out = a.tile_ptr = a.rule_ptr = nullptr;
      a.tile_desc = nullptr; a.n_rows_dev = nullptr; a.tile_bound = 0;
    } else if (km) {
      a.pair_in = swapped ? km->pair_out : km->pair_in;
      a.pair_out = swapped ? km->pair_in : km->pair_out;
      a.tile_ptr = km->tile_ptr; a.rule_ptr = km->rule_ptr; a.tile_desc = km->tile_desc;
      a.n_rows_dev = nullptr;
      a.tile_bound = km->pair_cap / DGR_TILE_M + km->K;
      DGR_REQUIRE(km->K == L.K, "layer %s: kernel volume mismatch", L.name.c_str());
      DGR_REQUIRE(!swapped || km->in_ptr, "layer %s: map has no in-major CSR", L.name.c_str());
    } else {
      DGR_REQUIRE(res == nullptr, "identity conv with residual not supported");
      a.pair_in = a.pair_out = a.tile_ptr = a.rule_ptr = nullptr;
      a.tile_desc = nullptr;
      a.n_rows_dev = cout_map.n_dev;
      a.tile_bound = dgr_ceil_div(cout_map.n_cap, DGR_TILE_M);
      a.l2_normalize = l2_next ? 1 : 0;
      l2_next = false;
    }
    hipEvent_t e0 = nullptr, em = nullptr, e1 = nullptr;
    if (prof) {
      e0 = ctx->events.next(); em = ctx->events.next(); e1 = ctx->events.next();
      if (!e0 || !em || !e1) return DGR_EHIP;
      DGR_HIP_CHECK(hipEventRecord(e0, stream));
    }
    if (km && ms.use_nbr) {
      const DgrNbrTable *t = nullptr;
      for (int l = 0; l < 4; ++l)
        if (km == &ms.same[l]) t = &ms.nsame[l];
      for (int l = 0; l < 3; ++l)
        if (km == &ms.down[l]) t = swapped ? &ms.nup[l] : &ms.ndown[l];
      DGR_REQUIRE(t && t->built && L.w16, "layer %s: no neighbour table / 16x16 weights", L.name.c_str());
      DgrConvOsLaunch o;
      o.in = in.ptr; o.in_ld = in.ld; o.in_relu = in.relu;
      o.out = out.ptr; o.out_ld = out.ld; o.out_relu = out.relu;
      o.rows_per_block = lvl_out <= 1 ? 64 : lvl_out == 2 ? (L.cin_pad >= 128 ? 64 : 32) : 16;
      o.phase_channels = (L.cin_pad >= 256 || (L.cin_pad == 128 && lvl_out >= 2)) ? 128 : 64;
      if (const char *e = getenv(lvl_out == 2 ? "DGR_OS_MB2" : lvl_out == 3 ? "DGR_OS_MB3" : "DGR_OS_MB01")) o.rows_per_block = atoi(e);
      if (const char *e = getenv("DGR_OS_CK")) o.phase_channels = atoi(e);
      o.w16 = L.w16; o.shift = L.shift;
      o.wb3 = L.w16b; o.piece_stride = L.w16b_piece;
      o.wbd = L.w16d;
      o.w_unscale = L.w_unscale; o.n_in_cap = cin_map.n_cap;
      if (L.w16b && !dgr_exact_f32()) {
        o.row_amax = in.amax;
        if (!o.row_amax) {
          uint32_t *mx;
          DGR_ALLOC(mx, ctx->arena, uint32_t, cin_map.n_cap);
          DGR_CHECK(dgr_row_amax(in.ptr, in.ld, L.cin, in.relu, cin_map.n_dev, cin_map.n_cap, mx, stream));
          o.row_amax = mx;
        }
      }
      o.out_amax = out.amax; o.out_amax2 = out.amax2;
      o.res = res ? res->ptr : nullptr; o.res_ld = res ? res->ld : 0; o.res_relu = res ? res->relu : 0;
      o.nbr = t; o.n_out_dev = cout_map.n_dev; o.n_out_cap = cout_map.n_cap;
      o.cin = L.cin; o.cin_pad = L.cin_pad; o.cout = L.cout;
      static const bool os_lists = getenv("DGR_OS_LISTS") != nullptr;
      bool same_stride = false;
      for (int l = 0; l < 4; ++l) same_stride = same_stride || t == &ms.nsame[l];
      o.dense = same_stride && o.row_amax && o.wbd && !os_lists && dgr_conv_dense_supported(L.cin, L.cin_pad, L.cout) &&
                dgr_fits_32bit_offsets(cin_map.n_cap, in.ld);
      DGR_REQUIRE(o.dense || (!in.dsplit_only && !out.dsplit_only), "layer %s: dense split rows outside the dense-tile kernel", L.name.c_str());
      static const bool no_up = getenv("DGR_NO_UP") != nullptr;
      o.up = swapped && !o.dense && !no_up && !os_lists && o.row_amax && o.wbd && t->perm && res == nullptr &&
             dgr_conv_up_supported(L.cin, L.cin_pad, L.cout) && dgr_fits_32bit_offsets(cin_map.n_cap, in.ld);
      if (o.dense) {
        o.in_dsplit = in.dsplit;
        o.out_dsplit = out.dsplit;
        if (out.dsplit_only) o.out = nullptr;
      }
      const char *kname = "sparse_conv_os";
      DGR_CHECK(dgr_conv_os_launch(o, stream, &kname));
      if (prof) {
        DGR_HIP_CHECK(hipEventRecord(e1, stream));
        ctx->conv_spans.push_back({e0, e1});
        ctx->gemm_spans.push_back({e0, e1});
        ctx->conv_kinds.push_back(kname);
      }
      LayerRun &r = net->runs[li];
      r = LayerRun();
      r.os = true;
      r.os_launch = o;
      r.nbr = *t;
      r.os_launch.nbr = &r.nbr;
      r.n_in = cin_map.n_dev; r.n_out = cout_map.n_dev; r.K = L.K;
      r.n_out_cap = cout_map.n_cap;
      return DGR_OK;
    }
    const bool small_cin = km && !swapped && !res && L.cin <= 8 && L.cout == 32 && L.cin_pad == 8;
    const char *kname = (L.cin == 6 && L.wq) ? "conv_cin6_quad_kernel" : L.cin == 1 ? "conv_small_cin_row_kernel" : "conv_small_cin_kernel";
    unsigned long long *clk = nullptr;
    const bool wide = L.wb && km;
    if (small_cin)
      DGR_CHECK(dgr_conv_small_cin(in.ptr, in.ld, in.relu, L.cin, L.w, L.wq, L.shift, *km, cout_map.n_dev, cout_map.n_cap,
                                   out.ptr, out.ld, stream));
    else if (wide) {
      DGR_REQUIRE(in.split.planes, "layer %s: the wide-layer kernel needs its input as split rows", L.name.c_str());
      if (prof) {
        DGR_ALLOC(a.clk, ctx->arena, unsigned long long, 2);
        DGR_HIP_CHECK(hipMemsetAsync(a.clk, 0xff, sizeof(unsigned long long), stream));
        DGR_HIP_CHECK(hipMemsetAsync(a.clk + 1, 0, sizeof(unsigned long long), stream));
        clk = a.clk;
      }
      DGR_CHECK(dgr_conv_wide_launch(a, in.split, L.wb, L.wb_piece, L.w_unscale, ctx->num_cus, stream, &kname));
    } else
      DGR_CHECK(dgr_conv_launch(a, ctx->num_cus, stream, &kname));
    if (prof) DGR_HIP_CHECK(hipEventRecord(em, stream));
    DGR_REQUIRE(!out.split.planes || (km && !small_cin), "layer %s: only a reduction can write split rows", L.name.c_str());
    if (km && !small_cin)
      DGR_CHECK(dgr_reduce_rows(ybuf, L.cout, swapped ? km->in_ptr : km->out_ptr, swapped ? km->in_pos : km->out_pos,
                                cout_map.n_dev, cout_map.n_cap, out.split_only ? nullptr : out.ptr, out.ld, L.shift, res ? res->ptr : nullptr,
                                res ? res->ld : 0, res ? res->relu : 0, stream, out.split.planes ? &out.split : nullptr,
                                out.relu));
    if (prof) {
      DGR_HIP_CHECK(hipEventRecord(e1, stream));
      ctx->conv_spans.push_back({e0, e1});
      ctx->gemm_spans.push_back({e0, em});
      ctx->conv_kinds.push_back(kname);
      ctx->conv_clks.resize(ctx->conv_spans.size(), nullptr);
      ctx->conv_clks.back() = clk;
    }
    LayerRun &r = net->runs[li];
    a.clk = nullptr;
    r.launch = a;
    r.split_in = wide ? in.split : DgrSplitRows();
    r.split_out = out.split;
    r.out_relu = out.relu;
    r.split_only = out.split_only;
    r.has_reduce = km != nullptr;
    r.small_cin = small_cin;
    if (km) r.km = *km;
    if (km) {
      r.red_ptr = swapped ? km->in_ptr : km->out_ptr;
      r.red_pos = swapped ? km->in_pos : km->out_pos;
    }
    r.n_out_cap = cout_map.n_cap;
    r.res = res ? res->ptr : nullptr; r.res_ld = res ? res->ld : 0; r.res_relu = res ? res->relu : 0;
    r.rule_ptr = km ? km->rule_ptr : nullptr;
    r.n_in = cin_map.n_dev; r.n_out = cout_map.n_dev; r.K = L.K;
    return DGR_OK;
  }
};

int dgr_resunet_forward_impl(dgr_ctx *ctx, dgr_net *net, const int32_t *coords, const float *feats,
                             int64_t N, float *out, hipStream_t stream) {
  DgrArena &A = ctx->arena;
  Fwd f;
  f.ctx = ctx; f.net = net; f.stream = stream; f.prof = ctx->profiling;
  hipEvent_t m0 = nullptr, m1 = nullptr;
  if (f.prof) {
    m0 = ctx->events.next(); m1 = ctx->events.next();
    DGR_HIP_CHECK(hipEventRecord(m0, stream));
  }
  f.ms.overflow = ctx->flag_dev;
  const bool use_nbr = net->D == 3 && net->cin <= 8 && net->conv1_ks <= 7;
  const bool conv1_fused = use_nbr;
  DGR_CHECK(dgr_build_maps(A, coords, N, net->D, net->conv1_ks, &f.ms, stream, conv1_fused, true, use_nbr));
  if (f.prof) {
    DGR_HIP_CHECK(hipEventRecord(m1, stream));
    (net->D == 3 ? ctx->map3_spans : ctx->map6_spans).push_back({m0, m1});
  }
  {
    const DgrMapSet &m = f.ms;
    int64_t need = m.use_nbr ? 64 : m.conv1.pair_cap * 32;
    const int64_t same_c[4] = {64, 64, 128, 256}, down_c[3] = {64, 128, 256};
    for (int l = 0; l < 4; ++l) need = std::max(need, m.same[l].pair_cap * same_c[l]);
    for (int l = 0; l < 3; ++l) need = std::max(need, m.down[l].pair_cap * down_c[l]);
    DGR_ALLOC(f.ybuf, A, float, need);
  }
  const DgrMapSet &ms = f.ms;
  const int64_t n1 = ms.cm[0].n_cap, n2 = ms.cm[1].n_cap, n4 = ms.cm[2].n_cap, n8 = ms.cm[3].n_cap;
  auto buf = [&](int64_t rows, int cols) -> float * { return A.get<float>((size_t)rows * cols); };
  float *t1 = buf(n1, 32), *y1 = buf(n1, 32), *cat1 = buf(n1, 96);
  float *t2 = buf(n2, 64), *y2 = buf(n2, 64), *cat2 = buf(n2, 128);
  float *t4 = buf(n4, 128), *y4 = buf(n4, 128), *cat4 = buf(n4, 256);
  float *t8 = buf(n8, 256), *y8 = buf(n8, 256), *s8 = buf(n8, 256);
  float *u4 = buf(n4, 128), *v4 = buf(n4, 128);
  float *u2 = buf(n2, 64), *v2 = buf(n2, 64);
  float *u1 = buf(n1, 64), *v1 = buf(n1, 64);
  float *h = buf(n1, 64);
  const bool fuse_l2 = net->normalize && net->cout <= 32;
  float *fin = (net->normalize && !fuse_l2) ? buf(n1, net->cout) : out;
  if (!t1 || !y1 || !cat1 || !t2 || !y2 || !cat2 || !t4 || !y4 || !cat4 || !t8 || !y8 || !s8 || !u4 ||
      !v4 || !u2 || !v2 || !u1 || !v1 || !h || !fin)
    return DGR_ENOMEM;

  const Tensor X{const_cast<float *>(feats), net->cin, 0};
  Tensor T1{t1, 32, 0}, Y1{y1, 32, 1}, S1{cat1 + 64, 96, 1};
  Tensor T2{t2, 64, 0}, Y2{y2, 64, 1};
  Tensor S2{cat2 + 64, 128, 1};
  Tensor T4{t4, 128, 0}, Y4{y4, 128, 1}, S4{cat4 + 128, 256, 1};
  Tensor T8{t8, 256, 0}, Y8{y8, 256, 1}, S8{s8, 256, 1};
  Tensor U4{u4, 128, 0}, V4{v4, 128, 1};
  Tensor U2{u2, 64, 0}, V2{v2, 64, 1};
  Tensor U1{u1, 64, 0}, V1{v1, 64, 1};
  Tensor S4T{cat4, 256, 1};
  {
    struct { Tensor *t; int consumer, channels; int64_t rows; bool middle; } sp[] = {
        {&T2, 4, 64, n2, false}, {&Y2, 5, 64, n2, true},
        {&S2, 6, 64, n2, false}, {&T4, 7, 128, n4, false}, {&Y4, 8, 128, n4, true}, {&S4, 9, 128, n4, false},
        {&T8, 10, 256, n8, false}, {&Y8, 11, 256, n8, true}, {&S8, 12, 256, n8, false}, {&U4, 13, 128, n4, false},
        {&V4, 14, 128, n4, true}, {&U2, 16, 64, n2, false}, {&V2, 17, 64, n2, true}, {&U1, 19, 64, n1, false},
        {&V1, 20, 64, n1, true}};
    for (auto &e : sp) {
      if (!net->W->layers[e.consumer].wb) continue;
      e.t->split.channels = e.channels;
      e.t->split_only = e.middle;
      DGR_ALLOC(e.t->split.planes, A, unsigned char, (size_t)e.rows * 4 * e.channels);
      DGR_ALLOC(e.t->split.scale, A, float, e.rows);
    }
  }
  Tensor S2T{cat2, 128, 1};
  const Tensor S1T{cat1, 96, 1};
  const Tensor H{h, 64, 1}, FIN{fin, net->cout, 0};
  Tensor CAT4{cat4, 256, 1}, CAT2{cat2, 128, 1};
  if (use_nbr) {
    const int64_t words = 5 * n1 + 6 * n2 + 6 * n4 + 3 * n8;
    uint32_t *pool;
    DGR_ALLOC(pool, A, uint32_t, words);
    DGR_HIP_CHECK(hipMemsetAsync(pool, 0, (size_t)words * sizeof(uint32_t), stream));
    auto take = [&](int64_t n) { uint32_t *p = pool; pool += n; return p; };
    for (Tensor *t : {&T1, &Y1, &S1, &U1, &V1}) t->amax = take(n1);
    for (Tensor *t : {&T2, &Y2, &S2, &CAT2, &U2, &V2}) t->amax = take(n2);
    for (Tensor *t : {&T4, &Y4, &S4, &CAT4, &U4, &V4}) t->amax = take(n4);
    for (Tensor *t : {&T8, &Y8, &S8}) t->amax = take(n8);
    S2.amax2 = CAT2.amax; S2T.amax2 = CAT2.amax;
    S4.amax2 = CAT4.amax; S4T.amax2 = CAT4.amax;
  }

  if (use_nbr && !getenv("DGR_NO_DSPLIT")) {
    static const bool os_lists = getenv("DGR_OS_LISTS") != nullptr;
    auto dense_layer = [&](int l, int64_t rows) {
      const DgrLayer &L = net->W->layers[l];
      return L.w16b && L.w16d && !dgr_exact_f32() && !os_lists && dgr_conv_dense_supported(L.cin, L.cin_pad, L.cout) &&
             dgr_fits_32bit_offsets(rows, L.cin);
    };
    struct { Tensor *t; int producer; int64_t rows; } mid[] = {{&Y1, 1, n1}, {&Y2, 4, n2}, {&V2, 16, n2}, {&V1, 19, n1}};
    for (auto &e : mid)
      if (dense_layer(e.producer, e.rows) && dense_layer(e.producer + 1, e.rows) && e.t->ld == net->W->layers[e.producer].cout) {
        e.t->dsplit = reinterpret_cast<unsigned char *>(e.t->ptr);
        e.t->dsplit_only = true;
      }
  }

  int li = 0;
  if (conv1_fused) {
    const DgrLayer &L0 = net->W->layers[0];
    int32_t *pc;
    DGR_ALLOC(pc, A, int32_t, 1);
    hipEvent_t e0 = nullptr, e1 = nullptr;
    if (f.prof) {
      e0 = ctx->events.next(); e1 = ctx->events.next();
      DGR_HIP_CHECK(hipEventRecord(e0, stream));
    }
    const char *k1name = "conv1_grid_kernel";
    DGR_CHECK(dgr_conv1_probe(A, ms.cm[0], net->conv1_ks, feats, net->cin, net->cin, L0.w, L0.shift, t1, 32, pc, stream,
                              L0.wc, &k1name, T1.amax));
    if (f.prof) {
      DGR_HIP_CHECK(hipEventRecord(e1, stream));
      ctx->conv_spans.push_back({e0, e1});
      ctx->gemm_spans.push_back({e0, e1});
      ctx->conv_kinds.push_back(k1name);
    }
    LayerRun &r0 = net->runs[0];
    r0 = LayerRun();
    r0.n_in = r0.n_out = ms.cm[0].n_dev;
    r0.K = L0.K;
    r0.fused_pairs = pc;
    li++;
  } else {
    DGR_CHECK(f.conv(li++, X, &ms.conv1, false, 0, 0, T1, nullptr));
  }
  DGR_CHECK(f.conv(li++, T1, &ms.same[0], false, 0, 0, Y1, nullptr));
  DGR_CHECK(f.conv(li++, Y1, &ms.same[0], false, 0, 0, S1, &T1));
  DGR_CHECK(f.conv(li++, S1, &ms.down[0], false, 0, 1, T2, nullptr));
  DGR_CHECK(f.conv(li++, T2, &ms.same[1], false, 1, 1, Y2, nullptr));
  DGR_CHECK(f.conv(li++, Y2, &ms.same[1], false, 1, 1, S2, &T2));
  DGR_CHECK(f.conv(li++, S2, &ms.down[1], false, 1, 2, T4, nullptr));
  DGR_CHECK(f.conv(li++, T4, &ms.same[2], false, 2, 2, Y4, nullptr));
  DGR_CHECK(f.conv(li++, Y4, &ms.same[2], false, 2, 2, S4, &T4));
  DGR_CHECK(f.conv(li++, S4, &ms.down[2], false, 2, 3, T8, nullptr));
  DGR_CHECK(f.conv(li++, T8, &ms.same[3], false, 3, 3, Y8, nullptr));
  DGR_CHECK(f.conv(li++, Y8, &ms.same[3], false, 3, 3, S8, &T8));
  DGR_CHECK(f.conv(li++, S8, &ms.down[2], true, 3, 2, U4, nullptr));
  DGR_CHECK(f.conv(li++, U4, &ms.same[2], false, 2, 2, V4, nullptr));
  DGR_CHECK(f.conv(li++, V4, &ms.same[2], false, 2, 2, S4T, &U4));
  DGR_CHECK(f.conv(li++, CAT4, &ms.down[1], true, 2, 1, U2, nullptr));
  DGR_CHECK(f.conv(li++, U2, &ms.same[1], false, 1, 1, V2, nullptr));
  DGR_CHECK(f.conv(li++, V2, &ms.same[1], false, 1, 1, S2T, &U2));
  DGR_CHECK(f.conv(li++, CAT2, &ms.down[0], true, 1, 0, U1, nullptr));
  DGR_CHECK(f.conv(li++, U1, &ms.same[0], false, 0, 0, V1, nullptr));
  DGR_CHECK(f.conv(li++, V1, &ms.same[0], false, 0, 0, S1T, &U1));
  const Tensor CAT1{cat1, 96, 1};
  DGR_CHECK(f.conv(li++, CAT1, nullptr, false, 0, 0, H, nullptr));
  f.l2_next = fuse_l2;
  DGR_CHECK(f.conv(li++, H, nullptr, false, 0, 0, FIN, nullptr));
  if (net->normalize && !fuse_l2)
    DGR_CHECK(dgr_l2_normalize_rows(fin, net->cout, out, net->cout, net->cout, 0, ms.cm[0].n_dev, n1, stream));

  auto &I = net->inter;
  net->run_generation = ctx->arena.generation;
  I.clear();
  I["s1"] = {S1.ptr, 96, 32, ms.cm[0].n_dev};
  I["s2"] = {S2.ptr, 128, 64, ms.cm[1].n_dev, ms.cm[1].canon};
  I["s4"] = {S4.ptr, 256, 128, ms.cm[2].n_dev, ms.cm[2].canon};
  I["s8"] = {S8.ptr, 256, 256, ms.cm[3].n_dev, ms.cm[3].canon};
  I["s4_tr"] = {cat4, 256, 128, ms.cm[2].n_dev, ms.cm[2].canon};
  I["s2_tr"] = {cat2, 128, 64, ms.cm[1].n_dev, ms.cm[1].canon};
  I["s1_tr"] = {cat1, 96, 64, ms.cm[0].n_dev};
  auto reg =[&](const char *name, const Tensor &t, int cols, int lvl) {
    DgrTensorRec r;
    r.f32 = (t.split_only || t.dsplit_only) ? nullptr : t.ptr;
    r.ld = t.ld; r.cols = cols;
    r.amax = t.amax;
    r.planes = t.split.planes; r.scale = t.split.scale;
    r.dsplit = t.dsplit;
    r.n_dev = ms.cm[lvl].n_dev; r.canon = ms.cm[lvl].canon;
    net->tensors[name] = r;
  };
  reg("T1", T1, 32, 0); reg("Y1", Y1, 32, 0); reg("S1", S1, 32, 0);
  reg("T2", T2, 64, 1); reg("Y2", Y2, 64, 1); reg("S2", S2, 64, 1);
  reg("T4", T4, 128, 2); reg("Y4", Y4, 128, 2); reg("S4", S4, 128, 2);
  reg("T8", T8, 256, 3); reg("Y8", Y8, 256, 3); reg("S8", S8, 256, 3);
  reg("U4", U4, 128, 2); reg("V4", V4, 128, 2); reg("S4T", S4T, 128, 2); reg("CAT4", CAT4, 256, 2);
  reg("U2", U2, 64, 1); reg("V2", V2, 64, 1); reg("S2T", S2T, 64, 1); reg("CAT2", CAT2, 128, 1);
  reg("U1", U1, 64, 0); reg("V1", V1, 64, 0); reg("S1T", S1T, 64, 0); reg("CAT1", CAT1, 96, 0);
  reg("H", H, 64, 0);
  reg("OUT", Tensor{out, net->cout, 0}, net->cout, 0);

  return DGR_OK;
}

void dgr_ctx_begin_profile(dgr_ctx *ctx) {
  ctx->events.used = 0;
  ctx->conv_spans.clear();
  ctx->gemm_spans.clear();
  ctx->conv_kinds.clear();
  ctx->conv_clks.clear();
  ctx->map3_spans.clear();
  ctx->map6_spans.clear();
  ctx->conv_launches = 0;
}

int dgr_ctx_collect_profile(dgr_ctx *ctx) {
  auto total = [](const std::vector<std::pair<hipEvent_t, hipEvent_t>> &v, float *out) -> int {
    float s = 0.f, t = 0.f;
    for (auto &sp : v) {
      DGR_HIP_CHECK(hipEventElapsedTime(&t, sp.first, sp.second));
      s += t;
    }
    *out = s;
    return DGR_OK;
  };
  DGR_CHECK(total(ctx->map3_spans, &ctx->stage_ms[5]));
  DGR_CHECK(total(ctx->map6_spans, &ctx->stage_ms[6]));
  DGR_CHECK(total(ctx->conv_spans, &ctx->stage_ms[7]));
  ctx->conv_launches = (int64_t)ctx->conv_spans.size();
  ctx->conv_span_ms.clear();
  ctx->gemm_span_ms.clear();
  for (auto &sp : ctx->conv_spans) {
    float t = 0.f;
    DGR_HIP_CHECK(hipEventElapsedTime(&t, sp.first, sp.second));
    ctx->conv_span_ms.push_back(t);
  }
  for (auto &sp : ctx->gemm_spans) {
    float t = 0.f;
    DGR_HIP_CHECK(hipEventElapsedTime(&t, sp.first, sp.second));
    ctx->gemm_span_ms.push_back(t);
  }
  ctx->conv_clk_us.assign(ctx->conv_spans.size(), 0.f);
  for (size_t i = 0; i < ctx->conv_clks.size() && i < ctx->conv_clk_us.size(); ++i)
    if (ctx->conv_clks[i]) {
      unsigned long long c[2] = {0, 0};
      DGR_HIP_CHECK(hipMemcpy(c, ctx->conv_clks[i], sizeof(c), hipMemcpyDeviceToHost));
      if (c[1] > c[0]) ctx->conv_clk_us[i] = (float)((double)(c[1] - c[0]) * 0.01);
    }
  return DGR_OK;
}

int dgr_flag_error(int32_t flag) {
  if (flag == 1) {
    dgr_set_error("duplicate coordinates in the sparse tensor input");
    return DGR_EINVAL;
  }
  if (flag == 2) {
    dgr_set_error("kernel-map capacity exceeded (more than the reserved pairs per output row)");
    return DGR_ENOMEM;
  }
  return DGR_OK;
}

static int check_flag(dgr_ctx *ctx, const int32_t *flag_dev, hipStream_t stream) {
  unsigned char *pin;
  DGR_CHECK(dgr_ctx_pinned(ctx, 64, &pin));
  DGR_HIP_CHECK(hipMemcpyAsync(pin, flag_dev, sizeof(int32_t), hipMemcpyDeviceToHost, stream));
  DGR_CHECK(dgr_ctx_wait(ctx, stream));
  return dgr_flag_error(*reinterpret_cast<volatile int32_t *>(pin));
}

int dgr_ctx_new_flag(dgr_ctx *ctx, hipStream_t stream) {
  DGR_ALLOC(ctx->flag_dev, ctx->arena, int32_t, 1);
  DGR_HIP_CHECK(hipMemsetAsync(ctx->flag_dev, 0, sizeof(int32_t), stream));
  return DGR_OK;
}

int dgr_ctx_check_flag(dgr_ctx *ctx, hipStream_t stream) {
  if (!ctx->flag_dev) return DGR_OK;
  return check_flag(ctx, ctx->flag_dev, stream);
}

void dgr_net_invalidate_runs(dgr_net *net) { net->run_generation = ~0ull; }
int dgr_net_out_channels(const dgr_net *net) { return net->cout; }
int dgr_net_in_channels(const dgr_net *net) { return net->cin; }
int dgr_net_dim(const dgr_net *net) { return net->D; }
const dgr_ctx *dgr_net_ctx(const dgr_net *net) { return net->ctx; }

extern "C" int dgr_resunet_forward(dgr_ctx *ctx, dgr_net *net, const int32_t *coords, const float *feats,
                                   int64_t N, float *out, dgr_stream stream_) {
  DGR_REQUIRE(ctx && net && coords && feats && out, "dgr_resunet_forward: NULL argument");
  DGR_REQUIRE(net->ctx == ctx, "dgr_resunet_forward: the net object belongs to another context (one dgr_net per context: "
                               "dgr_net_share gives a second context its own over the same weights)");
  DGR_REQUIRE(N > 0, "dgr_resunet_forward: empty sparse tensor (N=%lld)", (long long)N);
  hipStream_t stream = (hipStream_t)stream_;
  DGR_HIP_CHECK(hipSetDevice(ctx->device));
  DGR_CHECK(ctx->arena.reset());
  DGR_CHECK(dgr_ctx_new_flag(ctx, stream));
  dgr_ctx_begin_profile(ctx);
  DGR_CHECK(dgr_resunet_forward_impl(ctx, net, coords, feats, N, out, stream));
  DGR_CHECK(dgr_ctx_check_flag(ctx, stream));
  if (ctx->profiling) {
    memset(ctx->stage_ms, 0, sizeof(ctx->stage_ms));
    DGR_CHECK(dgr_ctx_collect_profile(ctx));
  }
  return DGR_OK;
}

extern "C" int dgr_debug_conv_layer(dgr_ctx *ctx, dgr_net *net, int layer, const int32_t *coords, const float *in,
                                    int in_relu, int64_t N, float *out, dgr_stream stream_) {
  DGR_REQUIRE(ctx && net && coords && in && out && N > 0, "dgr_debug_conv_layer: bad argument");
  DGR_REQUIRE(layer >= 0 && layer < (int)net->W->layers.size(), "layer %d out of range", layer);
  const DgrLayer &L = net->W->layers[layer];
  int k3 = 1;
  for (int d = 0; d < net->D; ++d) k3 *= 3;
  DGR_REQUIRE(L.K == k3 && L.cin >= 32, "dgr_debug_conv_layer: layer %s is not a 3^D conv with >= 32 input channels", L.name.c_str());
  hipStream_t stream = (hipStream_t)stream_;
  DGR_HIP_CHECK(hipSetDevice(ctx->device));
  DGR_CHECK(ctx->arena.reset());
  DGR_CHECK(dgr_ctx_new_flag(ctx, stream));
  dgr_ctx_begin_profile(ctx);
  DgrArena &A = ctx->arena;
  Fwd f;
  f.ctx = ctx; f.net = net; f.stream = stream; f.prof = false;
  f.ms.overflow = ctx->flag_dev;
  DGR_CHECK(dgr_build_maps(A, coords, N, net->D, 3, &f.ms, stream, false, true, net->D == 3));
  const int64_t n_cap = f.ms.cm[0].n_cap;
  if (!f.ms.use_nbr) DGR_ALLOC(f.ybuf, A, float, f.ms.same[0].pair_cap * L.cout);
  Tensor tin{const_cast<float *>(in), L.cin, in_relu}, tout{out, L.cout, 0};
  if (L.wb) {
    tin.split.channels = L.cin;
    DGR_ALLOC(tin.split.planes, A, unsigned char, (size_t)n_cap * 4 * L.cin);
    DGR_ALLOC(tin.split.scale, A, float, n_cap);
    DGR_CHECK(dgr_split_rows(in, L.cin, in_relu, f.ms.cm[0].n_dev, n_cap, tin.split, stream));
  }
  DGR_CHECK(f.conv(layer, tin, &f.ms.same[0], false, 0, 0, tout, nullptr));
  DGR_CHECK(dgr_ctx_check_flag(ctx, stream));
  dgr_net_invalidate_runs(net);
  return DGR_OK;
}

extern "C" int dgr_net_get_intermediate(dgr_ctx *ctx, dgr_net *net, const char *name, float *host_out,
                                        int64_t capacity, int64_t *rows, int64_t *cols) {
  DGR_REQUIRE(ctx && net && name && rows && cols, "NULL argument");
  auto it = net->inter.find(name);
  DGR_REQUIRE(it != net->inter.end() && it->second.n_dev, "no intermediate named '%s' (run a forward first)", name);
  DGR_REQUIRE(net->run_generation == ctx->arena.generation,
              "the activations of the last forward are gone: a later call on this context reused its workspace");
  const DgrTensorRef &t = it->second;
  int32_t n = 0;
  DGR_HIP_CHECK(hipDeviceSynchronize());
  DGR_HIP_CHECK(hipMemcpy(&n, t.n_dev, sizeof(int32_t), hipMemcpyDeviceToHost));
  *rows = n;
  *cols = t.cols;
  if (host_out) {
    DGR_REQUIRE(capacity >= (int64_t)n * t.cols, "host buffer too small");
    if (!t.canon) {
      DGR_HIP_CHECK(hipMemcpy2D(host_out, (size_t)t.cols * sizeof(float), t.ptr, (size_t)t.ld * sizeof(float),
                                (size_t)t.cols * sizeof(float), (size_t)n, hipMemcpyDeviceToHost));
    } else {
      std::vector<float> tmp((size_t)n * t.cols);
      std::vector<int32_t> canon(n);
      DGR_HIP_CHECK(hipMemcpy2D(tmp.data(), (size_t)t.cols * sizeof(float), t.ptr, (size_t)t.ld * sizeof(float),
                                (size_t)t.cols * sizeof(float), (size_t)n, hipMemcpyDeviceToHost));
      DGR_HIP_CHECK(hipMemcpy(canon.data(), t.canon, (size_t)n * sizeof(int32_t), hipMemcpyDeviceToHost));
      for (int32_t p = 0; p < n; ++p)
        memcpy(host_out + (size_t)canon[p] * t.cols, tmp.data() + (size_t)p * t.cols, (size_t)t.cols * sizeof(float));
    }
    for (int64_t i = 0; i < (int64_t)n * t.cols; ++i) host_out[i] = host_out[i] > 0.f ? host_out[i] : 0.f;
  }
  return DGR_OK;
}

extern "C" int dgr_net_get_tensor(dgr_ctx *ctx, dgr_net *net, const char *name, int repr, void *host_out,
                                  int64_t capacity_bytes, int64_t *rows, int64_t *row_bytes) {
  DGR_REQUIRE(ctx && net && name && rows && row_bytes, "NULL argument");
  auto it = net->tensors.find(name);
  DGR_REQUIRE(it != net->tensors.end() && it->second.n_dev, "no tensor named '%s' (run a forward first)", name);
  DGR_REQUIRE(net->run_generation == ctx->arena.generation,
              "the activations of the last forward are gone: a later call on this context reused its workspace");
  const DgrTensorRec &t = it->second;
  const void *src = nullptr;
  size_t rb = 0, ld = 0;
  const char *what = "";
  switch (repr) {
    case DGR_TENSOR_F32: src = t.f32; rb = (size_t)t.cols * 4; ld = (size_t)t.ld * 4; what = "f32 rows"; break;
    case DGR_TENSOR_AMAX: src = t.amax; rb = ld = 4; what = "row maxima"; break;
    case DGR_TENSOR_SPLIT_PLANES: src = t.planes; rb = ld = (size_t)t.cols * 4; what = "split rows"; break;
    case DGR_TENSOR_SPLIT_SCALE: src = t.scale; rb = ld = 4; what = "split-row scales"; break;
    case DGR_TENSOR_DENSE_SPLIT: src = t.dsplit; rb = ld = (size_t)t.cols * 4; what = "dense split rows"; break;
    default: DGR_REQUIRE(false, "dgr_net_get_tensor: unknown representation %d", repr);
  }
  DGR_REQUIRE(src != nullptr, "the last forward did not write tensor '%s' as %s", name, what);
  int32_t n = 0;
  DGR_HIP_CHECK(hipDeviceSynchronize());
  DGR_HIP_CHECK(hipMemcpy(&n, t.n_dev, sizeof(int32_t), hipMemcpyDeviceToHost));
  *rows = n;
  *row_bytes = (int64_t)rb;
  if (!host_out) return DGR_OK;
  DGR_REQUIRE(capacity_bytes >= (int64_t)n * (int64_t)rb, "host buffer too small");
  if (!t.canon) {
    DGR_HIP_CHECK(hipMemcpy2D(host_out, rb, src, ld, rb, (size_t)n, hipMemcpyDeviceToHost));
  } else {
    std::vector<unsigned char> tmp((size_t)n * rb);
    std::vector<int32_t> canon(n);
    DGR_HIP_CHECK(hipMemcpy2D(tmp.data(), rb, src, ld, rb, (size_t)n, hipMemcpyDeviceToHost));
    DGR_HIP_CHECK(hipMemcpy(canon.data(), t.canon, (size_t)n * sizeof(int32_t), hipMemcpyDeviceToHost));
    for (int32_t p = 0; p < n; ++p) {
      DGR_REQUIRE(canon[p] >= 0 && canon[p] < n, "dgr_net_get_tensor: row numbering out of range");
      memcpy(static_cast<unsigned char *>(host_out) + (size_t)canon[p] * rb, tmp.data() + (size_t)p * rb, rb);
    }
  }
  return DGR_OK;
}

extern "C" int dgr_net_layer_stats(dgr_ctx *ctx, dgr_net *net, int layer, int64_t stats[8]) {
  DGR_REQUIRE(ctx && net && stats, "NULL argument");
  DGR_REQUIRE(layer >= 0 && layer < (int)net->W->layers.size(), "layer %d out of range", layer);
  const LayerRun &r = net->runs[layer];
  DGR_REQUIRE(r.n_in && r.n_out, "run a forward first");
  DGR_REQUIRE(net->run_generation == ctx->arena.generation,
              "the kernel maps of the last forward are gone: a later call on this context reused its workspace");
  const DgrLayer &L = net->W->layers[layer];
  DGR_HIP_CHECK(hipDeviceSynchronize());
  int32_t n_in = 0, n_out = 0;
  DGR_HIP_CHECK(hipMemcpy(&n_in, r.n_in, sizeof(int32_t), hipMemcpyDeviceToHost));
  DGR_HIP_CHECK(hipMemcpy(&n_out, r.n_out, sizeof(int32_t), hipMemcpyDeviceToHost));
  int64_t P = n_out, kne = 1;
  if (r.os) {
    int64_t counts[27];
    DGR_CHECK(dgr_nbr_counts(r.nbr, r.n_out, counts));
    P = 0;
    kne = 0;
    for (int k = 0; k < 27; ++k) { P += counts[k]; kne += counts[k] > 0; }
  } else if (r.fused_pairs) {
    int32_t pc = 0;
    DGR_HIP_CHECK(hipMemcpy(&pc, r.fused_pairs, sizeof(int32_t), hipMemcpyDeviceToHost));
    P = pc;
    kne = r.K;
  } else if (r.rule_ptr) {
    std::vector<int32_t> rp(r.K + 1);
    DGR_HIP_CHECK(hipMemcpy(rp.data(), r.rule_ptr, (size_t)(r.K + 1) * sizeof(int32_t), hipMemcpyDeviceToHost));
    P = rp[r.K];
    kne = 0;
    for (int k = 0; k < r.K; ++k) kne += rp[k + 1] > rp[k];
  }
  stats[0] = P; stats[1] = kne; stats[2] = n_in; stats[3] = n_out;
  stats[4] = L.cin; stats[5] = L.cout; stats[6] = L.K; stats[7] = 0;
  return DGR_OK;
}

extern "C" int dgr_net_rerun_layer(dgr_ctx *ctx, dgr_net *net, int layer, int reps, float *gemm_ms, float *reduce_ms) {
  DGR_REQUIRE(ctx && net && gemm_ms && reduce_ms && reps > 0, "bad argument");
  DGR_REQUIRE(layer >= 0 && layer < (int)net->W->layers.size(), "layer %d out of range", layer);
  const LayerRun &r = net->runs[layer];
  DGR_REQUIRE(r.n_in && r.n_out, "run a forward first");
  DGR_REQUIRE(net->run_generation == ctx->arena.generation,
              "the kernel maps of the last forward are gone: a later call on this context reused its workspace");
  DGR_REQUIRE(!r.fused_pairs, "layer %d ran fused with its neighbour search; not re-runnable", layer);
  const DgrLayer &L = net->W->layers[layer];
  hipStream_t st = ctx->part_stream;
  hipEvent_t e0, e1, e2;
  DGR_HIP_CHECK(hipEventCreate(&e0)); DGR_HIP_CHECK(hipEventCreate(&e1)); DGR_HIP_CHECK(hipEventCreate(&e2));
  float tg = 0.f, tr = 0.f;
  for (int i = 0; i < reps + 1; ++i) {
    DGR_HIP_CHECK(hipEventRecord(e0, st));
    if (r.os)
      DGR_CHECK(dgr_conv_os_launch(r.os_launch, st));
    else if (r.small_cin)
      DGR_CHECK(dgr_conv_small_cin(r.launch.in, r.launch.in_ld, r.launch.in_relu, L.cin, L.w, L.wq, L.shift, r.km, r.n_out,
                                   r.n_out_cap, r.launch.out, r.launch.out_ld, st));
    else if (L.wb && r.has_reduce)
      DGR_CHECK(dgr_conv_wide_launch(r.launch, r.split_in, L.wb, L.wb_piece, L.w_unscale, ctx->num_cus, st));
    else
      DGR_CHECK(dgr_conv_launch(r.launch, ctx->num_cus, st));
    DGR_HIP_CHECK(hipEventRecord(e1, st));
    if (r.has_reduce && !r.small_cin && !r.os)
      DGR_CHECK(dgr_reduce_rows(r.launch.y, L.cout, r.red_ptr, r.red_pos, r.n_out, r.n_out_cap,
                                r.split_only ? nullptr : r.launch.out, r.launch.out_ld, L.shift, r.res, r.res_ld, r.res_relu, st,
                                r.split_out.planes ? &r.split_out : nullptr, r.out_relu));
    DGR_HIP_CHECK(hipEventRecord(e2, st));
    DGR_HIP_CHECK(hipEventSynchronize(e2));
    float a = 0.f, b = 0.f;
    DGR_HIP_CHECK(hipEventElapsedTime(&a, e0, e1));
    DGR_HIP_CHECK(hipEventElapsedTime(&b, e1, e2));
    if (i > 0) { tg += a; tr += b; }
  }
  (void)hipEventDestroy(e0); (void)hipEventDestroy(e1); (void)hipEventDestroy(e2);
  *gemm_ms = tg / reps;
  *reduce_ms = tr / reps;
  return DGR_OK;
}
```

### deepglobalregistration_amd/model/resunet.py

```python
import numpy as np
import torch

from .. import ops
from ..sparse import SparseTensor
from . import me_conventions


class ResUNet2:
    NORM_TYPE = None
    BLOCK_NORM_TYPE = 'BN'
    CHANNELS = [None, 32, 64, 128, 256]
    TR_CHANNELS = [None, 32, 64, 64, 128]

    def __init__(self, in_channels=3, out_channels=32, bn_momentum=0.1, conv1_kernel_size=3,
                 normalize_feature=False, D=3):
        if (self.NORM_TYPE, self.CHANNELS, self.TR_CHANNELS) != ('BN', [None, 32, 64, 128, 256],
                                                                   [None, 64, 64, 64, 128]):
            raise NotImplementedError('only the ResUNetBN2C configuration is on the DGR inference path')
        self.in_channels, self.out_channels = in_channels, out_channels
        self.bn_momentum = bn_momentum
        self.conv1_kernel_size = conv1_kernel_size
        self.normalize_feature = normalize_feature
        self.D = D
        self.device = torch.device('cuda')
        self._state = None
        self._net = None
        self.training = True
        self.me_conventions = dict(me_conventions.DEFAULT)

    def load_state_dict(self, state_dict, strict=True):
        default_conv = (self.me_conventions['kernel_order'] == me_conventions.DEFAULT['kernel_order']
                        and not self.me_conventions['transposed_mirrored'])
        if default_conv and state_dict and all(torch.is_tensor(v) and v.is_cuda for v in state_dict.values()):
            self._state = dict(state_dict)
        else:
            self._state = {k: (v.detach().cpu().numpy() if torch.is_tensor(v) else np.asarray(v))
                           for k, v in state_dict.items()}
            self._state = me_conventions.convert_state_dict(self._state, self.D, self.me_conventions['kernel_order'],
                                                            self.me_conventions['transposed_mirrored'])
        self._net = None
        self._share = None
        return self

    def to(self, device):
        self.device = torch.device(device)
        self._net = None
        return self

    def cuda(self):
        return self.to('cuda')

    def eval(self):
        self.training = False
        return self

    def train(self, mode=True):
        if mode:
            raise NotImplementedError('libdgr_hip implements the inference path only (eval-mode batch norm)')
        return self.eval()

    def share_weights(self, other):
        if (type(other), other.D, other.in_channels, other.out_channels, other.conv1_kernel_size) != \
                (type(self), self.D, self.in_channels, self.out_channels, self.conv1_kernel_size):
            raise ValueError('share_weights: the other model is a different network')
        if other._net is None:
            raise RuntimeError('share_weights: the other model has no device-resident weights yet -- run it once, or call '
                               'its _handle(), on the thread that owns it before sharing')
        self.normalize_feature = other.normalize_feature
        self._state = None
        self._share = other
        self._net = None
        return self

    def _handle(self):
        if self._net is None:
            share = getattr(self, '_share', None)
            if share is not None:
                self._net = ops.NetHandle(None, self.D, self.in_channels, self.out_channels, self.conv1_kernel_size,
                                          self.normalize_feature, self.device, share_from=share._net)
                return self._net
            if self._state is None:
                raise RuntimeError('load_state_dict() must be called before the first forward')
            self._net = ops.NetHandle(self._state, self.D, self.in_channels, self.out_channels,
                                      self.conv1_kernel_size, self.normalize_feature, self.device)
        return self._net

    def forward(self, x):
        if not isinstance(x, SparseTensor):
            raise TypeError('expected a deepglobalregistration_amd.SparseTensor')
        out = self._handle().forward(x.C, x.F)
        return SparseTensor(out, coordinates=x.C, device=self.device)

    __call__ = forward


class ResUNetBN2C(ResUNet2):
    NORM_TYPE = 'BN'
    CHANNELS = [None, 32, 64, 128, 256]
    TR_CHANNELS = [None, 64, 64, 64, 128]
```

### deepglobalregistration_amd/ops.py

```python
import ctypes as C

import numpy as np
import torch

from . import _lib
from ._lib import check, get_ctx, ptr, stream_ptr, vp

F32_EPS = float(np.finfo(np.float32).eps)


def _dev(t):
    if not (torch.is_tensor(t) and t.is_cuda):
        raise ValueError('expected a CUDA(ROCm) tensor')
    return t.device


def _as(t, dtype, device):
    if not torch.is_tensor(t):
        t = torch.as_tensor(np.asarray(t))
    return t.to(device=device, dtype=dtype).contiguous()


def voxelize(xyz, voxel_size, batch_index=0, device='cuda'):
    lib = _lib.load()
    device = torch.device(device)
    if not torch.is_tensor(xyz):
        xyz = torch.from_numpy(np.ascontiguousarray(xyz))
    if xyz.dtype not in (torch.float32, torch.float64):
        xyz = xyz.double()
    if xyz.dim() != 2 or xyz.shape[1] != 3:
        raise ValueError(f'expected an [M,3] point array, got {tuple(xyz.shape)}')
    xyz = xyz.to(device).contiguous()
    M = xyz.shape[0]
    if M == 0:
        raise ValueError('empty point cloud')
    sel = torch.empty(M, dtype=torch.int64, device=device)
    coords = torch.empty((M, 4), dtype=torch.int32, device=device)
    out = torch.empty((M, 3), dtype=torch.float32, device=device)
    n = C.c_int64(0)
    check(lib.dgr_voxelize(get_ctx(device), ptr(xyz), int(xyz.dtype == torch.float64), M,
                           float(voxel_size), int(batch_index), ptr(sel), ptr(coords), ptr(out),
                           C.byref(n), stream_ptr(device.index)))
    n = n.value
    return out[:n], coords[:n], sel[:n]


class NetHandle:

    def __init__(self, state_dict, D, in_channels, out_channels, conv1_kernel_size,
                 normalize_feature, device='cuda', share_from=None):
        lib = _lib.load()
        self.device = torch.device(device)
        self.D, self.cin, self.cout = D, in_channels, out_channels
        self.conv1_ks, self.normalize = int(conv1_kernel_size), bool(normalize_feature)
        if share_from is not None:
            if (share_from.D, share_from.cin, share_from.cout, share_from.conv1_ks, share_from.normalize) != \
                    (D, in_channels, out_channels, self.conv1_ks, self.normalize):
                raise ValueError('share_from is a different network')
            h = vp()
            with torch.cuda.device(self.device):
                check(lib.dgr_net_share(get_ctx(self.device), share_from.handle, C.byref(h)))
            self.handle = h
            return
        keep, descs = [], []
        items = [(n, t) for n, t in state_dict.items() if not n.endswith('num_batches_tracked')]
        on_device = bool(items) and all(torch.is_tensor(t) and t.is_cuda and t.device.index == (self.device.index or 0)
                                        for _, t in items)
        self.created_on_device = on_device
        for name, t in items:
            if on_device:
                a = t.detach().to(torch.float32).contiguous()
                keep.append(a)
                descs.append(_lib.WeightDesc(name.encode(), a.data_ptr(), a.numel()))
            else:
                a = t.detach().cpu().numpy() if torch.is_tensor(t) else np.asarray(t)
                a = np.ascontiguousarray(a, dtype=np.float32)
                keep.append(a)
                descs.append(_lib.WeightDesc(name.encode(), a.ctypes.data, a.size))
        arr = (_lib.WeightDesc * len(descs))(*descs)
        h = vp()
        with torch.cuda.device(self.device):
            if on_device:
                torch.cuda.current_stream(self.device).synchronize()
            create = lib.dgr_net_create_device if on_device else lib.dgr_net_create
            check(create(get_ctx(self.device), D, in_channels, out_channels,
                         conv1_kernel_size, int(bool(normalize_feature)), arr, len(descs),
                         C.byref(h)))
        self.handle = h

    def __del__(self):
        try:
            if getattr(self, 'handle', None):
                _lib.load().dgr_net_destroy(self.handle)
                self.handle = None
        except Exception:
            pass

    @property
    def param_bytes(self):
        return _lib.load().dgr_net_param_bytes(self.handle)

    @property
    def sharers(self):
        return _lib.load().dgr_net_sharers(self.handle)

    def forward(self, coords, feats):
        lib = _lib.load()
        dev = self.device
        coords = _as(coords, torch.int32, dev)
        feats = _as(feats, torch.float32, dev)
        if coords.dim() != 2 or coords.shape[1] != self.D + 1:
            raise ValueError(f'coords must be [N,{self.D + 1}] (batch column first), got {tuple(coords.shape)}')
        if feats.dim() != 2 or feats.shape != (coords.shape[0], self.cin):
            raise ValueError(f'feats must be [{coords.shape[0]},{self.cin}], got {tuple(feats.shape)}')
        N = coords.shape[0]
        if N == 0:
            raise ValueError('empty sparse tensor')
        out = torch.empty((N, self.cout), dtype=torch.float32, device=dev)
        check(lib.dgr_resunet_forward(get_ctx(dev), self.handle, ptr(coords), ptr(feats), N, ptr(out),
                                      stream_ptr(dev.index)))
        return out

    def intermediate(self, name):
        lib = _lib.load()
        rows, cols = C.c_int64(0), C.c_int64(0)
        ctx = get_ctx(self.device)
        check(lib.dgr_net_get_intermediate(ctx, self.handle, name.encode(), None, 0, C.byref(rows), C.byref(cols)))
        buf = np.empty((rows.value, cols.value), np.float32)
        check(lib.dgr_net_get_intermediate(ctx, self.handle, name.encode(), buf.ctypes.data, buf.size,
                                           C.byref(rows), C.byref(cols)))
        return buf

    TENSOR_REPRS = {'f32': (0, np.float32), 'amax': (1, np.uint32), 'split_planes': (2, np.uint8),
                    'split_scale': (3, np.float32), 'dense_split': (4, np.uint8)}

    def tensor(self, name, repr='f32'):
        lib = _lib.load()
        code, dtype = self.TENSOR_REPRS[repr]
        rows, rb = C.c_int64(0), C.c_int64(0)
        ctx = get_ctx(self.device)
        check(lib.dgr_net_get_tensor(ctx, self.handle, name.encode(), code, None, 0, C.byref(rows), C.byref(rb)))
        buf = np.empty((rows.value, rb.value // np.dtype(dtype).itemsize), dtype)
        check(lib.dgr_net_get_tensor(ctx, self.handle, name.encode(), code, buf.ctypes.data, buf.nbytes,
                                     C.byref(rows), C.byref(rb)))
        return buf[:, 0] if repr in ('amax', 'split_scale') else buf

    def debug_conv_layer(self, layer, coords, feats, relu=False):
        dev = self.device
        coords = _as(coords, torch.int32, dev)
        feats = _as(feats, torch.float32, dev)
        lay = _lib.load()
        st_cout = None
        ch, tr = [None, 32, 64, 128, 256], [None, 64, 64, 64, 128]
        widths = [ch[1]] * 3 + [ch[2]] * 3 + [ch[3]] * 3 + [ch[4]] * 3 + [tr[4]] * 3 + [tr[3]] * 3 + [tr[2]] * 3 + [tr[1], self.cout]
        st_cout = widths[layer]
        out = torch.empty((coords.shape[0], st_cout), dtype=torch.float32, device=dev)
        check(lay.dgr_debug_conv_layer(get_ctx(dev), self.handle, int(layer), ptr(coords), ptr(feats), int(bool(relu)),
                                       coords.shape[0], ptr(out), stream_ptr(dev.index)))
        return out

    def rerun_layer(self, layer, reps=5):
        lib = _lib.load()
        g, r = C.c_float(0), C.c_float(0)
        check(lib.dgr_net_rerun_layer(get_ctx(self.device), self.handle, layer, reps, C.byref(g), C.byref(r)))
        return g.value, r.value

    def layer_stats(self):
        lib = _lib.load()
        out = []
        for li in range(lib.dgr_net_num_layers(self.handle)):
            st = (C.c_int64 * 8)()
            check(lib.dgr_net_layer_stats(get_ctx(self.device), self.handle, li, st))
            out.append(dict(pairs=st[0], nonempty=st[1], n_in=st[2], n_out=st[3], cin=st[4], cout=st[5], K=st[6]))
        return out


class Maps:

    def __init__(self, coords, D, conv1_kernel_size=3, device='cuda', lean=False):
        lib = _lib.load()
        self.device = torch.device(device)
        coords = _as(coords, torch.int32, self.device)
        self.D, self.lean = D, bool(lean)
        h = vp()
        if lean:
            check(lib.dgr_maps_create_ex(get_ctx(self.device), ptr(coords), coords.shape[0], D, conv1_kernel_size, 1,
                                         C.byref(h), stream_ptr(self.device.index)))
        else:
            check(lib.dgr_maps_create(get_ctx(self.device), ptr(coords), coords.shape[0], D, conv1_kernel_size,
                                      C.byref(h), stream_ptr(self.device.index)))
        self.handle = h

    def raw(self, kind, ts, field):
        lib = _lib.load()
        n, eb = C.c_int64(0), C.c_int64(0)
        check(lib.dgr_maps_get_raw(self.handle, kind.encode(), ts, field.encode(), None, 0, C.byref(n), C.byref(eb)))
        scalar = eb.value == 8
        buf = np.empty(n.value, np.int64 if scalar else np.uint16 if eb.value == 2 else np.int32)
        check(lib.dgr_maps_get_raw(self.handle, kind.encode(), ts, field.encode(), buf.ctypes.data, buf.nbytes,
                                   C.byref(n), C.byref(eb)))
        if scalar:
            return int(buf[0])
        shape = {'coords': (-1, self.D + 1), 'tile_desc': (-1, 4), 'nbr': (27, -1), 'perm': (8, -1)}.get(field)
        return buf.reshape(shape) if shape else buf

    def __del__(self):
        try:
            if getattr(self, 'handle', None):
                _lib.load().dgr_maps_destroy(self.handle)
                self.handle = None
        except Exception:
            pass

    def coords(self, ts):
        lib = _lib.load()
        n = C.c_int64(0)
        check(lib.dgr_maps_get_coords(self.handle, ts, None, 0, C.byref(n)))
        out = np.empty((n.value, self.D + 1), np.int32)
        check(lib.dgr_maps_get_coords(self.handle, ts, out.ctypes.data, out.size, C.byref(n)))
        return out

    def kernel_map(self, kind, ts):
        lib = _lib.load()
        kid = {'same': 0, 'conv1': 1, 'down': 2, 'nbr_same': 3, 'nbr_down': 4, 'nbr_up': 5}[kind]
        K, P = C.c_int64(0), C.c_int64(0)
        check(lib.dgr_maps_get_kernel_map(self.handle, kid, ts, None, 0, None, None, 0, C.byref(K), C.byref(P)))
        rule = np.empty(K.value + 1, np.int32)
        pin = np.empty(P.value, np.int32)
        pout = np.empty(P.value, np.int32)
        check(lib.dgr_maps_get_kernel_map(self.handle, kid, ts, rule.ctypes.data, rule.size, pin.ctypes.data,
                                          pout.ctypes.data, pin.size, C.byref(K), C.byref(P)))
        k = np.repeat(np.arange(K.value), np.diff(rule))
        return k.astype(np.int64), pin.astype(np.int64), pout.astype(np.int64)


def knn1(F0, F1, squared=False, return_distance=False):
    lib = _lib.load()
    dev = _dev(F0)
    F0 = _as(F0, torch.float32, dev)
    F1 = _as(F1, torch.float32, dev)
    if F0.dim() != 2 or F1.dim() != 2 or F0.shape[1] != F1.shape[1]:
        raise ValueError('F0 [N0,C] and F1 [N1,C] must share the feature width')
    N0, N1 = F0.shape[0], F1.shape[0]
    idx = torch.empty(N0, dtype=torch.int64, device=dev)
    dist = torch.empty(N0, dtype=torch.float32, device=dev) if return_distance else None
    check(lib.dgr_knn1_l2(get_ctx(dev), ptr(F0), N0, ptr(F1), N1, F0.shape[1], int(squared), ptr(idx),
                          ptr(dist), stream_ptr(dev.index)))
    return (idx, dist) if return_distance else idx


def knn1_batch(F0, F1, off0, off1, squared=False, return_distance=False):
    lib = _lib.load()
    dev = _dev(F0)
    F0 = _as(F0, torch.float32, dev)
    F1 = _as(F1, torch.float32, dev)
    if F0.dim() != 2 or F1.dim() != 2 or F0.shape[1] != F1.shape[1]:
        raise ValueError('F0 [N0,C] and F1 [N1,C] must share the feature width')
    o0 = np.ascontiguousarray(off0, dtype=np.int64)
    o1 = np.ascontiguousarray(off1, dtype=np.int64)
    if len(o0) != len(o1) or len(o0) < 2 or o0[0] != 0 or o1[0] != 0 or o0[-1] != F0.shape[0] or o1[-1] != F1.shape[0]:
        raise ValueError('off0 / off1 must be [npairs+1] row offsets covering F0 / F1')
    idx = torch.empty(F0.shape[0], dtype=torch.int64, device=dev)
    dist = torch.empty(F0.shape[0], dtype=torch.float32, device=dev) if return_distance else None
    check(lib.dgr_knn1_l2_batch(get_ctx(dev), ptr(F0), o0.ctypes.data_as(_lib.c_i64p), ptr(F1),
                                o1.ctypes.data_as(_lib.c_i64p), len(o0) - 1, F0.shape[1], int(squared), ptr(idx),
                                ptr(dist), stream_ptr(dev.index)))
    return (idx, dist) if return_distance else idx


KNN_MAX_K = 32


def check_knn_k(k):
    if isinstance(k, (bool, np.bool_)) or not isinstance(k, (int, np.integer)):
        raise ValueError(f'knn must be an integer in [1, {KNN_MAX_K}], got {k!r}')
    if not 1 <= int(k) <= KNN_MAX_K:
        raise ValueError(f'knn must be an integer in [1, {KNN_MAX_K}], got {int(k)}')
    return int(k)


def knn(F0, F1, k, squared=False, return_distance=False):
    k = check_knn_k(k)
    lib = _lib.load()
    dev = _dev(F0)
    F0 = _as(F0, torch.float32, dev)
    F1 = _as(F1, torch.float32, dev)
    if F0.dim() != 2 or F1.dim() != 2 or F0.shape[1] != F1.shape[1]:
        raise ValueError('F0 [N0,C] and F1 [N1,C] must share the feature width')
    N0, N1 = F0.shape[0], F1.shape[0]
    idx = torch.empty((N0, k), dtype=torch.int64, device=dev)
    dist = torch.empty((N0, k), dtype=torch.float32, device=dev) if return_distance else None
    check(lib.dgr_knn_l2(get_ctx(dev), ptr(F0), N0, ptr(F1), N1, F0.shape[1], k, int(squared), ptr(idx), ptr(dist),
                         stream_ptr(dev.index)))
    return (idx, dist) if return_distance else idx


def knn_batch(F0, F1, off0, off1, k, squared=False, return_distance=False):
    k = check_knn_k(k)
    lib = _lib.load()
    dev = _dev(F0)
    F0 = _as(F0, torch.float32, dev)
    F1 = _as(F1, torch.float32, dev)
    if F0.dim() != 2 or F1.dim() != 2 or F0.shape[1] != F1.shape[1]:
        raise ValueError('F0 [N0,C] and F1 [N1,C] must share the feature width')
    o0 = np.ascontiguousarray(off0, dtype=np.int64)
    o1 = np.ascontiguousarray(off1, dtype=np.int64)
    if len(o0) != len(o1) or len(o0) < 2 or o0[0] != 0 or o1[0] != 0 or o0[-1] != F0.shape[0] or o1[-1] != F1.shape[0]:
        raise ValueError('off0 / off1 must be [npairs+1] row offsets covering F0 / F1')
    idx = torch.empty((F0.shape[0], k), dtype=torch.int64, device=dev)
    dist = torch.empty((F0.shape[0], k), dtype=torch.float32, device=dev) if return_distance else None
    check(lib.dgr_knn_l2_batch(get_ctx(dev), ptr(F0), o0.ctypes.data_as(_lib.c_i64p), ptr(F1),
                               o1.ctypes.data_as(_lib.c_i64p), len(o0) - 1, F0.shape[1], k, int(squared), ptr(idx),
                               ptr(dist), stream_ptr(dev.index)))
    return (idx, dist) if return_distance else idx


def inlier_inputs(coords0, xyz0, coords1, xyz1, idx1, feature_type='coords'):
    lib = _lib.load()
    dev = _dev(xyz0)
    ft = {'ones': 0, 'coords': 1}.get(feature_type)
    if ft is None:
        raise TypeError('Undefined feature type')
    coords0, coords1 = _as(coords0, torch.int32, dev), _as(coords1, torch.int32, dev)
    xyz0, xyz1 = _as(xyz0, torch.float32, dev), _as(xyz1, torch.float32, dev)
    idx1 = _as(idx1, torch.int64, dev).reshape(-1)
    N0 = coords0.shape[0]
    if idx1.shape[0] != N0:
        raise ValueError('one correspondence per row of fragment 0 expected')
    coords6 = torch.empty((N0, 7), dtype=torch.int32, device=dev)
    feats = torch.empty((N0, 6 if ft == 1 else 1), dtype=torch.float32, device=dev)
    check(lib.dgr_inlier_inputs(get_ctx(dev), ptr(coords0), ptr(xyz0), N0, ptr(coords1), ptr(xyz1),
                                coords1.shape[0], ptr(idx1), ft, ptr(coords6), ptr(feats),
                                stream_ptr(dev.index)))
    return coords6, feats


def sigmoid_clip_sum(logit, clip):
    lib = _lib.load()
    dev = _dev(logit)
    logit = _as(logit, torch.float32, dev).reshape(-1)
    w = torch.empty_like(logit)
    s = C.c_double(0)
    check(lib.dgr_sigmoid_clip_sum(get_ctx(dev), ptr(logit), logit.shape[0], float(clip), ptr(w), C.byref(s),
                                   stream_ptr(dev.index)))
    return w.reshape(-1, 1), s.value


def gather_rows3(src, idx):
    lib = _lib.load()
    dev = _dev(src)
    src = _as(src, torch.float32, dev)
    idx = _as(idx, torch.int64, dev).reshape(-1)
    out = torch.empty((idx.shape[0], 3), dtype=torch.float32, device=dev)
    check(lib.dgr_gather_rows3(get_ctx(dev), ptr(src), ptr(idx), idx.shape[0], ptr(out), stream_ptr(dev.index)))
    return out


def _xyw(X, Y, w):
    dev = _dev(X)
    X, Y = _as(X, torch.float32, dev), _as(Y, torch.float32, dev)
    w = _as(w, torch.float32, dev).reshape(-1)
    if X.shape != Y.shape or X.dim() != 2 or X.shape[1] != 3 or w.shape[0] != X.shape[0]:
        raise ValueError('X, Y must be [N,3] and w [N] / [N,1]')
    return dev, X, Y, w


def weighted_procrustes(X, Y, w, eps=F32_EPS):
    lib = _lib.load()
    dev, X, Y, w = _xyw(X, Y, w)
    R = (C.c_float * 9)()
    t = (C.c_float * 3)()
    check(lib.dgr_weighted_procrustes(get_ctx(dev), ptr(X), ptr(Y), ptr(w), X.shape[0], float(eps), R, t,
                                      stream_ptr(dev.index)))
    return np.array(R, np.float32).reshape(3, 3), np.array(t, np.float32)


def se3_refine(X, Y, w, quantization_size=1.0, max_iter=1000, max_break_count=20,
               break_threshold_ratio=1e-5):
    lib = _lib.load()
    dev, X, Y, w = _xyw(X, Y, w)
    R = (C.c_float * 9)()
    t = (C.c_float * 3)()
    it, bc, loss = C.c_int32(0), C.c_int32(0), C.c_float(0)
    check(lib.dgr_se3_refine(get_ctx(dev), ptr(X), ptr(Y), ptr(w), X.shape[0], float(quantization_size),
                             int(max_iter), int(max_break_count), float(break_threshold_ratio), R, t,
                             C.byref(it), C.byref(loss), C.byref(bc), stream_ptr(dev.index)))
    return (np.array(R, np.float32).reshape(3, 3), np.array(t, np.float32),
            {'iterations': it.value, 'loss': loss.value, 'break_count': bc.value})


def se3_refine_from(X, Y, w, state, max_iter, quantization_size=1.0, max_break_count=10 ** 9,
                    break_threshold_ratio=1e-5):
    lib = _lib.load()
    dev, X, Y, w = _xyw(X, Y, w)
    si = (C.c_double * 30)(*([float(v) for v in state['prm']] + [float(v) for v in state['m']] + [float(v) for v in state['v']]
                             + [float(state['i']), float(state['loss_prev']), float(state['breaks'])]))
    so = (C.c_double * 30)()
    check(lib.dgr_debug_se3_refine_from(get_ctx(dev), ptr(X), ptr(Y), ptr(w), X.shape[0], float(quantization_size),
                                        int(max_iter), int(max_break_count), float(break_threshold_ratio), si, so,
                                        stream_ptr(dev.index)))
    so = np.array(so, np.float64)
    return {'prm': so[:9].copy(), 'm': so[9:18].copy(), 'v': so[18:27].copy(), 'i': int(so[27]), 'loss_prev': float(so[28]),
            'breaks': int(so[29])}


def _xyz_dev(a, dev=None):
    t = a if torch.is_tensor(a) else torch.as_tensor(np.asarray(a))
    if dev is None:
        dev = t.device if t.is_cuda else torch.device('cuda', torch.cuda.current_device())
    t = t.to(device=dev, dtype=torch.float32).contiguous()
    if t.dim() != 2 or t.shape[1] != 3:
        raise ValueError(f'expected [N,3] points, got {tuple(t.shape)}')
    return t


def _xyz_any_dev(a):
    t = a if torch.is_tensor(a) else torch.from_numpy(np.ascontiguousarray(a))
    return t if t.is_cuda else t.to(torch.device('cuda', torch.cuda.current_device()))


def icp_point_to_point(source, target, max_correspondence_distance, init=None, max_iter=30,
                       relative_fitness=1e-6, relative_rmse=1e-6):
    lib = _lib.load()
    src = _xyz_dev(source)
    dst = _xyz_dev(target, src.device)
    Ti = None
    if init is not None:
        init = np.ascontiguousarray(np.asarray(init, np.float64))
        if init.shape != (4, 4):
            raise ValueError('init must be a 4x4 matrix')
        Ti = (C.c_double * 16)(*init.reshape(-1))
    T = (C.c_double * 16)()
    st = (C.c_double * 3)()
    check(lib.dgr_icp_point_to_point(get_ctx(src.device), ptr(src), src.shape[0], ptr(dst), dst.shape[0],
                                     float(max_correspondence_distance), Ti, int(max_iter), float(relative_fitness),
                                     float(relative_rmse), T, st, stream_ptr(src.device.index)))
    return np.array(T, np.float64).reshape(4, 4), float(st[0]), float(st[1]), int(st[2])


def ransac_correspondence(X, Y, distance_threshold, num_hypotheses, seed=0):
    lib = _lib.load()
    X = _xyz_dev(X)
    Y = _xyz_dev(Y, X.device)
    if X.shape != Y.shape:
        raise ValueError('X and Y must have the same shape')
    T = (C.c_double * 16)()
    st = (C.c_double * 3)()
    check(lib.dgr_ransac_correspondence(get_ctx(X.device), ptr(X), ptr(Y), X.shape[0], float(distance_threshold),
                                        int(num_hypotheses), int(seed) & 0xffffffff, T, st, stream_ptr(X.device.index)))
    return np.array(T, np.float64).reshape(4, 4), int(st[0]), int(st[1]), float(st[2])


def _offsets(off, name, total=None):
    o = np.ascontiguousarray(np.asarray(off), dtype=np.int64).reshape(-1)
    if len(o) < 2 or o[0] != 0 or bool((np.diff(o) < 0).any()):
        raise ValueError(f'{name} must be [npairs+1] row offsets that start at 0 and do not decrease')
    if total is not None and o[-1] != total:
        raise ValueError(f'{name} ends at {int(o[-1])}, the array has {int(total)} rows')
    return o


def _rows(a, width, name):
    shape = tuple(a.shape) if hasattr(a, 'shape') else np.asarray(a).shape
    if len(shape) != 2 or shape[1] != width:
        raise ValueError(f'{name} must be [N,{width}], got {shape}')
    return shape[0]


def check_radius_args(radius, K, T, npairs):
    if isinstance(radius, (bool, np.bool_)) or not isinstance(radius, (int, float, np.integer, np.floating)) \
            or not np.isfinite(radius) or radius <= 0:
        raise ValueError(f'radius must be a positive finite number, got {radius!r}')
    if K is not None and (isinstance(K, (bool, np.bool_)) or not isinstance(K, (int, np.integer)) or K < 1
                          or K > np.iinfo(np.int32).max):
        raise ValueError(f'K must be None or an integer >= 1, got {K!r}')
    T = T.detach().cpu().numpy() if torch.is_tensor(T) else np.asarray(T)
    if T.shape == (4, 4) and npairs == 1:
        T = T[None]
    if T.shape != (npairs, 4, 4):
        raise ValueError(f'T must be [{npairs},4,4], got {T.shape}')
    T = np.ascontiguousarray(T, dtype=np.float64).reshape(npairs, 16)
    if not np.isfinite(T).all():
        raise ValueError('T must be finite')
    return float(radius), 0 if K is None else int(K), T


def radius_pairs_batch(xyz0, off0, xyz1, off1, T, radius, K=None):
    n0, n1 = _rows(xyz0, 3, 'xyz0'), _rows(xyz1, 3, 'xyz1')
    o0, o1 = _offsets(off0, 'off0', n0), _offsets(off1, 'off1', n1)
    if len(o0) != len(o1):
# ... 620 lines not shown
```

### include/dgr_hip.h

```cpp
#ifndef DGR_HIP_H
#define DGR_HIP_H

#include <stdint.h>

#ifdef __cplusplus
extern "C" {
#endif

typedef struct dgr_ctx dgr_ctx;
typedef struct dgr_net dgr_net;
typedef struct dgr_maps dgr_maps;
typedef void *dgr_stream;

enum {
  DGR_OK = 0,
  DGR_EINVAL = -1,
  DGR_EHIP = -2,
  DGR_ENOMEM = -3,
  DGR_ESVD = -4,
  DGR_EINTERNAL = -5
};

enum { DGR_STATUS_OK = 0, DGR_STATUS_LOW_CONFIDENCE = 1, DGR_STATUS_SVD_FAILED = 2,
       DGR_STATUS_SAFEGUARD = 3 ,
       DGR_STATUS_FLAG_ICP_SKIPPED = 0x100, DGR_STATUS_MASK = 0xff,
       DGR_STATUS_EXCHANGE_TIMEOUT = 0x7f };

const char *dgr_last_error(void);
const char *dgr_version(void);

int dgr_ctx_create(int device, dgr_ctx **out);
void dgr_ctx_destroy(dgr_ctx *ctx);
int64_t dgr_ctx_workspace_bytes(dgr_ctx *ctx);
int dgr_ctx_create_partition_stream(dgr_ctx *ctx, int part, int nparts, dgr_stream *out);

int dgr_voxelize(dgr_ctx *ctx, const void *xyz, int is_f64, int64_t M, double voxel_size,
                 int32_t batch_index, int64_t *sel_out, int32_t *coords_out, float *xyz_out,
                 int64_t *n_out, dgr_stream stream);

typedef struct {
  const char *name;
  const float *data;
  int64_t numel;
} dgr_weight_desc;

int dgr_net_create(dgr_ctx *ctx, int D, int in_channels, int out_channels, int conv1_kernel_size,
                   int normalize_feature, const dgr_weight_desc *weights, int n_weights,
                   dgr_net **out);
int dgr_net_create_device(dgr_ctx *ctx, int D, int in_channels, int out_channels, int conv1_kernel_size,
                          int normalize_feature, const dgr_weight_desc *weights, int n_weights,
                          dgr_net **out);
void dgr_net_destroy(dgr_net *net);
int64_t dgr_net_param_bytes(const dgr_net *net);
int dgr_net_share(dgr_ctx *ctx, const dgr_net *src, dgr_net **out);
int dgr_net_sharers(const dgr_net *net);

int dgr_resunet_forward(dgr_ctx *ctx, dgr_net *net, const int32_t *coords, const float *feats,
                        int64_t N, float *out, dgr_stream stream);
int dgr_net_get_intermediate(dgr_ctx *ctx, dgr_net *net, const char *name, float *host_out,
                             int64_t capacity, int64_t *rows, int64_t *cols);
#define DGR_TENSOR_F32 0
#define DGR_TENSOR_AMAX 1
#define DGR_TENSOR_SPLIT_PLANES 2
#define DGR_TENSOR_SPLIT_SCALE 3
#define DGR_TENSOR_DENSE_SPLIT 4
int dgr_net_get_tensor(dgr_ctx *ctx, dgr_net *net, const char *name, int repr, void *host_out,
                       int64_t capacity_bytes, int64_t *rows, int64_t *row_bytes);
int dgr_net_layer_stats(dgr_ctx *ctx, dgr_net *net, int layer, int64_t stats[8]);
int dgr_net_num_layers(const dgr_net *net);
int dgr_net_rerun_layer(dgr_ctx *ctx, dgr_net *net, int layer, int reps, float *gemm_ms, float *reduce_ms);

int dgr_maps_create(dgr_ctx *ctx, const int32_t *coords, int64_t N, int D, int conv1_kernel_size,
                    dgr_maps **out, dgr_stream stream);
void dgr_maps_destroy(dgr_maps *maps);
int dgr_maps_get_coords(dgr_maps *maps, int ts, int32_t *host_out, int64_t capacity, int64_t *n);
int dgr_maps_get_kernel_map(dgr_maps *maps, int kind, int ts, int32_t *rule_ptr, int64_t rule_cap,
                            int32_t *pair_in, int32_t *pair_out, int64_t pair_cap, int64_t *K,
                            int64_t *P);
#define DGR_MAPS_LEAN 1
int dgr_maps_create_ex(dgr_ctx *ctx, const int32_t *coords, int64_t N, int D, int conv1_kernel_size, int flags,
                       dgr_maps **out, dgr_stream stream);
int dgr_maps_get_raw(dgr_maps *maps, const char *kind, int ts, const char *field, void *host_out,
                     int64_t capacity_bytes, int64_t *count, int64_t *elem_bytes);

int dgr_knn1_l2(dgr_ctx *ctx, const float *F0, int64_t N0, const float *F1, int64_t N1, int C,
                int squared, int64_t *idx_out, float *dist_out, dgr_stream stream);

int dgr_knn1_l2_batch(dgr_ctx *ctx, const float *F0, const int64_t *off0, const float *F1,
                      const int64_t *off1, int npairs, int C, int squared, int64_t *idx_out,
                      float *dist_out, dgr_stream stream);

#define DGR_KNN_MAX_K 32
int dgr_knn_l2(dgr_ctx *ctx, const float *F0, int64_t N0, const float *F1, int64_t N1, int C, int k,
               int squared, int64_t *idx_out, float *dist_out, dgr_stream stream);

int dgr_knn_l2_batch(dgr_ctx *ctx, const float *F0, const int64_t *off0, const float *F1,
                     const int64_t *off1, int npairs, int C, int k, int squared, int64_t *idx_out,
                     float *dist_out, dgr_stream stream);

int dgr_inlier_inputs(dgr_ctx *ctx, const int32_t *coords0, const float *xyz0, int64_t N0,
                      const int32_t *coords1, const float *xyz1, int64_t N1, const int64_t *idx1,
                      int feature_type, int32_t *coords6_out, float *feats_out, dgr_stream stream);

int dgr_sigmoid_clip_sum(dgr_ctx *ctx, const float *logit, int64_t N, float clip, float *weights_out,
                         double *wsum, dgr_stream stream);

int dgr_gather_rows3(dgr_ctx *ctx, const float *src, const int64_t *idx, int64_t N, float *dst,
                     dgr_stream stream);

int dgr_weighted_procrustes(dgr_ctx *ctx, const float *X, const float *Y, const float *w, int64_t N,
                            float eps, float *R9, float *t3, dgr_stream stream);

int dgr_se3_refine(dgr_ctx *ctx, const float *X, const float *Y, const float *w, int64_t N,
                   float quantization_size, int max_iter, int max_break_count,
                   double break_threshold_ratio, float *R9, float *t3, int32_t *iterations,
                   float *loss, int32_t *break_count, dgr_stream stream);

int dgr_icp_point_to_point(dgr_ctx *ctx, const float *src, int64_t N0, const float *dst, int64_t N1,
                           double max_correspondence_distance, const double *T_init, int max_iter,
                           double relative_fitness, double relative_rmse, double *T_out, double *stats_out,
                           dgr_stream stream);

int dgr_ransac_correspondence(dgr_ctx *ctx, const float *X, const float *Y, int64_t N, double distance_threshold,
                              int64_t num_hypotheses, uint32_t seed, double *T_out, double *stats_out,
                              dgr_stream stream);

typedef struct {
  float clip_weight_thresh;
  float voxel_size;
  int inlier_feature_type;
  int max_iter;
  int max_break_count;
  double break_threshold_ratio;
  int skip_refinement;
  int safeguard;
  int64_t ransac_hypotheses;
  uint32_t ransac_seed;
  int use_icp;
} dgr_params;

int dgr_register_batch(dgr_ctx *ctx, dgr_net *fcgf, dgr_net *inlier, const int32_t *coords0,
                       const float *xyz0, const int64_t *off0, const int32_t *coords1,
                       const float *xyz1, const int64_t *off1, int npairs, const dgr_params *params,
                       const int64_t *override_idx1, const float *forced_logit, float *T_out,
                       int32_t *status_out,
                       float *stats_out, dgr_stream stream);
int dgr_register_pairs(dgr_ctx *ctx, dgr_net *inlier, const int32_t *bank_coords, const float *bank_xyz,
                       const float *bank_F, const int64_t *bank_off, int nfrag, int C, const int32_t *pair_ids,
                       int npairs, const dgr_params *params, const int64_t *override_idx1,
                       const float *forced_logit, float *T_out, int32_t *status_out, float *stats_out,
                       dgr_stream stream);
int dgr_register_batch_output(dgr_ctx *ctx, int which, void *dst_dev, int64_t capacity_bytes,
                              int64_t *numel, dgr_stream stream);
int dgr_register_batch_f64(dgr_ctx *ctx, double *T_out, int64_t capacity_pairs, int64_t *npairs);

int dgr_ctx_set_profiling(dgr_ctx *ctx, int enable);
#define DGR_NUM_STAGE_TIMES 9
int dgr_ctx_stage_times_v2(dgr_ctx *ctx, float *times_ms, int capacity, int *n);
int dgr_ctx_stage_times(dgr_ctx *ctx, float *times_ms);
int64_t dgr_ctx_conv_launches(dgr_ctx *ctx);
int dgr_ctx_conv_launch_times(dgr_ctx *ctx, float *times_ms, float *gemm_ms, int64_t capacity, int64_t *n);
int dgr_ctx_conv_launch_kernel_us(dgr_ctx *ctx, float *us, int64_t capacity, int64_t *n);
int dgr_ctx_conv_launch_kinds(dgr_ctx *ctx, char *buf, int64_t capacity, int64_t *n);

int dgr_radius_pairs_batch(dgr_ctx *ctx, const float *xyz0, const int64_t *off0, const float *xyz1,
                           const int64_t *off1, int npairs, const double *T, double radius, int K,
                           int32_t *counts_out, int64_t *pairs_out, int64_t capacity, int64_t *total_out,
                           dgr_stream stream);
int dgr_pairs_isin_batch(dgr_ctx *ctx, const int64_t *pos, const int64_t *pos_off, const int64_t *pred,
                         const int64_t *pred_off, int npairs, const int64_t *M_per_pair, uint8_t *out,
                         dgr_stream stream);
int dgr_validation_counts(dgr_ctx *ctx, const uint8_t *label, const float *weights, float threshold,
                          const int64_t *off, int npairs, int64_t *counts_out, dgr_stream stream);

#define DGR_SCORE_WIDTH 11
int dgr_score_pairs(dgr_ctx *ctx, const float *bank_xyz, const int64_t *bank_off, int nfrag, const int32_t *pair_ids,
                    int npairs, const double *T, double radius, double *sums_out, dgr_stream stream);

#define DGR_PG_MAX_NODES 128
typedef struct {
  double mu;
  int reference_node;
  int max_iter;
  double rel_tol;
} dgr_pg_params;
int dgr_pose_graph_optimize(dgr_ctx *ctx, int ngraphs, const int64_t *node_off, const int64_t *edge_off,
                            const int32_t *edge_ids, const double *edge_T, const double *edge_info,
                            const uint8_t *edge_uncertain, const double *pose_init, const dgr_pg_params *params,
                            double *pose_out, double *line_out, double *stats_out, dgr_stream stream);

#define DGR_VM_FRAC_BITS 40
int dgr_voxel_mean(dgr_ctx *ctx, const void *xyz, int is_f64, const int64_t *off, int nfrag, const int32_t *frag_ids,
                   int nsel, const double *T, const double *origin, double voxel_size, int64_t *first_out,
                   int32_t *coords_out, int32_t *count_out, int64_t *fsum_out, double *mean_out, int64_t *n_out,
                   int64_t *dropped_out, dgr_stream stream);

#define DGR_TSDF_BLOCK_LIMIT 67108864
int dgr_tsdf_fragment(dgr_ctx *ctx, const uint16_t *depth, int nframes, int height, int width, const double *intrinsic,
                      const double *pose, const double *extrinsic, double voxel_length, double sdf_trunc,
                      double depth_scale, double depth_trunc, int block, int stride, int min_weight, double *xyz_out,
                      int64_t max_points, int32_t *blocks_out, float *tsdf_out, int32_t *weight_out, int64_t max_blocks,
                      int64_t *n_blocks_out, int64_t *n_points_out, int64_t *kept_out, dgr_stream stream);

int dgr_tsdf_mesh(dgr_ctx *ctx, const int32_t *blocks, int64_t n_blocks, const float *tsdf, const int32_t *weight, int block,
                  double voxel_length, int min_weight, double *xyz_out, double *normal_out, int64_t max_vertices,
                  int32_t *tri_out, int64_t max_triangles, int64_t *n_vertices_out, int64_t *n_triangles_out,
                  dgr_stream stream);

int dgr_debug_ortho2rotation(dgr_ctx *ctx, const float *p6, int64_t n, const float *grad_R9, float *R9_out,
                             float *grad_p6_out, dgr_stream stream);
int dgr_debug_se3_refine_from(dgr_ctx *ctx, const float *X, const float *Y, const float *w, int64_t N,
                              float quantization_size, int max_iter, int max_break_count,
                              double break_threshold_ratio, const double *state_in, double *state_out,
                              dgr_stream stream);
int dgr_debug_smooth_l1(dgr_ctx *ctx, const float *X, const float *Y, int64_t n, float quantization_size,
                        float *per_point_out, dgr_stream stream);

int dgr_debug_conv_layer(dgr_ctx *ctx, dgr_net *net, int layer, const int32_t *coords, const float *in, int in_relu,
                         int64_t N, float *out, dgr_stream stream);

#ifdef __cplusplus
}
#endif
#endif
```

Baseline: 401.8.

## Run coarse 3-D FCGF 27-tap layers on rule-major wide split-f16 kernel

For the 3-D FCGF net, the coarse 27-tap convolutions with at least 128 input and output channels now use the wide split-f16 MFMA kernel instead of the neighbour-table kernel. This requires rule-major kernel maps, which are built from the existing neighbour tables by a new count, scan and fill pass. Split-row conversion and row-amax computation are deferred to just before the consuming layer. It adds map-build kernels, memory for pair lists and extra weight copies, and is enabled by default through wide_coarse for D=3.

After: 411.6 (median of 6 runs). 1.02x the previous value.

```diff
diff --git a/deepglobalregistration_amd/_lib.py b/deepglobalregistration_amd/_lib.py
--- a/deepglobalregistration_amd/_lib.py
+++ b/deepglobalregistration_amd/_lib.py
@@ -48,6 +48,7 @@
     'dgr_net_param_bytes': (C.c_int64, [vp]),
     'dgr_net_share': (C.c_int, [vp, vp, C.POINTER(vp)]),
     'dgr_net_sharers': (C.c_int, [vp]),
+    'dgr_net_set_wide_coarse': (C.c_int, [vp, C.c_int]),
     'dgr_resunet_forward': (C.c_int, [vp, vp, vp, vp, C.c_int64, vp, vp]),
     'dgr_net_get_intermediate': (C.c_int, [vp, vp, C.c_char_p, vp, C.c_int64, c_i64p, c_i64p]),
     'dgr_net_get_tensor': (C.c_int, [vp, vp, C.c_char_p, C.c_int, vp, C.c_int64, c_i64p, c_i64p]),
diff --git a/deepglobalregistration_amd/csrc/dgr_internal.h b/deepglobalregistration_amd/csrc/dgr_internal.h
--- a/deepglobalregistration_amd/csrc/dgr_internal.h
+++ b/deepglobalregistration_amd/csrc/dgr_internal.h
@@ -134,7 +134,7 @@
 
 int dgr_build_maps(DgrArena &arena, const int32_t *coords, int64_t N, int D, int conv1_ks,
                    DgrMapSet *ms, hipStream_t stream, bool skip_conv1_map = false, bool lean = false,
-                   bool nbr_tables = false);
+                   bool nbr_tables = false, bool nbr_lists = false);
 int dgr_nbr_counts(const DgrNbrTable &t, const int32_t *n_out_dev, int64_t counts[27]);
 int dgr_conv1_probe(DgrArena &arena, const DgrCoordMap &cm, int ks, const float *in, int in_ld, int cin,
                     const float *w_tiled, const float *shift, float *out, int out_ld, int32_t *pair_count,
diff --git a/deepglobalregistration_amd/csrc/kmap.hip b/deepglobalregistration_amd/csrc/kmap.hip
--- a/deepglobalregistration_amd/csrc/kmap.hip
+++ b/deepglobalregistration_amd/csrc/kmap.hip
@@ -830,12 +830,134 @@
   return DGR_OK;
 }
 
+constexpr int NL_JOBS = 3;
+struct NbrListJobs {
+  const int32_t *nbr[NL_JOBS], *n_out_dev[NL_JOBS];
+  long long n_pad[NL_JOBS], n_cap[NL_JOBS];
+  int RB[NL_JOBS];
+  int32_t *counts[NL_JOBS], *cnt_out[NL_JOBS];
+  const int32_t *base[NL_JOBS], *out_ptr[NL_JOBS];
+  int32_t *pair_in[NL_JOBS], *out_pos[NL_JOBS];
+};
+__global__ void __launch_bounds__(KM_THREADS) nbr_list_count(NbrListJobs J) {
+  __shared__ int wcnt[KM_THREADS / 64][27];
+  const int m = blockIdx.y, b = blockIdx.x;
+  if (b >= J.RB[m]) return;
+  const int64_t o = (int64_t)b * KM_THREADS + threadIdx.x, n_pad = J.n_pad[m];
+  const int32_t *__restrict__ nbr = J.nbr[m];
+  const bool live = o < *J.n_out_dev[m];
+  int mine = 0;
+#pragma unroll
+  for (int k = 0; k < 27; ++k) {
+    const bool hit = live && nbr[(int64_t)k * n_pad + o] >= 0;
+    mine += hit;
+    const unsigned long long bal = __ballot(hit);
+    if ((threadIdx.x & 63) == 0) wcnt[threadIdx.x >> 6][k] = __popcll(bal);
+  }
+  __syncthreads();
+  if (threadIdx.x < 27) {
+    int n = 0;
+    for (int w = 0; w < KM_THREADS / 64; ++w) n += wcnt[w][threadIdx.x];
+    J.counts[m][(int64_t)threadIdx.x * J.RB[m] + b] = n;
+  }
+  if (o <= J.n_cap[m]) J.cnt_out[m][o] = mine;
+}
+__global__ void __launch_bounds__(KM_THREADS) nbr_list_fill(NbrListJobs J) {
+  __shared__ int wcnt[KM_THREADS / 64][27];
+  const int m = blockIdx.y, b = blockIdx.x;
+  if (b >= J.RB[m]) return;
+  const int64_t o = (int64_t)b * KM_THREADS + threadIdx.x, n_pad = J.n_pad[m];
+  const int32_t *__restrict__ nbr = J.nbr[m];
+  if ((int64_t)b * KM_THREADS >= *J.n_out_dev[m]) return;
+  const bool live = o < *J.n_out_dev[m];
+  const int lane = threadIdx.x & 63, wave = threadIdx.x >> 6;
+#pragma unroll
+  for (int k = 0; k < 27; ++k) {
+    const unsigned long long bal = __ballot(live && nbr[(int64_t)k * n_pad + o] >= 0);
+    if (lane == 0) wcnt[wave][k] = __popcll(bal);
+  }
+  __syncthreads();
+  int slot = live ? J.out_ptr[m][o] : 0;
+  int32_t *__restrict__ pair_in = J.pair_in[m], *__restrict__ out_pos = J.out_pos[m];
+#pragma unroll
+  for (int k = 0; k < 27; ++k) {
+    const int v = live ? nbr[(int64_t)k * n_pad + o] : -1;
+    const unsigned long long bal = __ballot(v >= 0);
+    if (v < 0) continue;
+    int pos = J.base[m][(int64_t)k * J.RB[m] + b] + __popcll(bal & ((1ull << lane) - 1ull));
+    for (int w = 0; w < wave; ++w) pos += wcnt[w][k];
+    pair_in[pos] = v;
+    out_pos[slot++] = pos;
+  }
+}
+
+struct NbrListSpec {
+  const DgrNbrTable *t;
+  const DgrCoordMap *out;
+  DgrKernelMap *km;
+};
+static int build_nbr_lists3(DgrArena &arena, const NbrListSpec *specs, int nj, hipStream_t stream) {
+  DGR_REQUIRE(nj >= 1 && nj <= NL_JOBS && 2 * nj <= DGR_SCAN_MAX, "neighbour-table lists: %d maps per call", nj);
+  NbrListJobs J = {};
+  FinalizeJobs fj = {};
+  for (int m = 0; m < nj; ++m) {
+    DgrKernelMap *km = specs[m].km;
+    const int64_t n_cap = specs[m].out->n_cap;
+    DGR_REQUIRE(specs[m].t->built && specs[m].t->n_pad >= n_cap, "neighbour-table lists: table %d is not built", m);
+    km->K = 27;
+    km->pair_cap = 27 * n_cap;
+    DGR_REQUIRE(km->pair_cap < (1ll << 31), "kernel map too large (%lld pairs)", (long long)km->pair_cap);
+    km->tile_cap = km->pair_cap / DGR_TILE_M + 27;
+    DGR_ALLOC(km->rule_ptr, arena, int32_t, 28);
+    DGR_ALLOC(km->tile_ptr, arena, int32_t, 28);
+    DGR_ALLOC(km->pair_in, arena, int32_t, km->pair_cap);
+    DGR_ALLOC(km->tile_desc, arena, int4, km->tile_cap);
+    DGR_ALLOC(km->out_ptr, arena, int32_t, n_cap + 1);
+    DGR_ALLOC(km->out_pos, arena, int32_t, km->pair_cap);
+    km->pair_out = nullptr; km->pair_k = nullptr; km->in_ptr = km->in_pos = nullptr;
+  }
+  DgrArena::Mark mk = arena.mark();
+  const int32_t *ins[2 * NL_JOBS];
+  int32_t *outs[2 * NL_JOBS], *tots[2 * NL_JOBS];
+  int64_t ns[2 * NL_JOBS];
+  int max_rb = 0;
+  long long max_tiles = 0;
+  for (int m = 0; m < nj; ++m) {
+    DgrKernelMap *km = specs[m].km;
+    const int64_t n_cap = specs[m].out->n_cap;
+    const int RB = (int)dgr_ceil_div(n_cap + 1, KM_THREADS);
+    int32_t *counts, *base, *total, *cnt_out;
+    DGR_ALLOC(counts, arena, int32_t, (int64_t)27 * RB);
+    DGR_ALLOC(base, arena, int32_t, (int64_t)27 * RB);
+    DGR_ALLOC(total, arena, int32_t, 1);
+    DGR_ALLOC(cnt_out, arena, int32_t, n_cap + 1);
+    J.nbr[m] = specs[m].t->nbr; J.n_out_dev[m] = specs[m].out->n_dev; J.n_pad[m] = specs[m].t->n_pad; J.n_cap[m] = n_cap;
+    J.RB[m] = RB; J.counts[m] = counts; J.cnt_out[m] = cnt_out; J.base[m] = base; J.out_ptr[m] = km->out_ptr;
+    J.pair_in[m] = km->pair_in; J.out_pos[m] = km->out_pos;
+    ins[2 * m] = cnt_out; outs[2 * m] = km->out_ptr; tots[2 * m] = nullptr; ns[2 * m] = n_cap + 1;
+    ins[2 * m + 1] = counts; outs[2 * m + 1] = base; tots[2 * m + 1] = total; ns[2 * m + 1] = (int64_t)27 * RB;
+    finalize_job(fj, m, base, total, 27, RB, km);
+    max_rb = std::max(max_rb, RB);
+    max_tiles = std::max<long long>(max_tiles, km->tile_cap);
+  }
+  nbr_list_count<<<dim3((unsigned)max_rb, (unsigned)nj), KM_THREADS, 0, stream>>>(J);
+  DGR_LAUNCH_CHECK();
+  DGR_CHECK(dgr_exclusive_scan_multi(arena, 2 * nj, ins, outs, ns, tots, stream));
+  kmap_finalize<<<nj, 1024, 0, stream>>>(fj);
+  tile_desc_kernel<<<dim3((unsigned)dgr_ceil_div(max_tiles, 256), (unsigned)nj), 256, 0, stream>>>(fj);
+  nbr_list_fill<<<dim3((unsigned)max_rb, (unsigned)nj), KM_THREADS, 0, stream>>>(J);
+  DGR_LAUNCH_CHECK();
+  arena.rewind(mk);
+  for (int m = 0; m < nj; ++m) specs[m].km->built = true;
+  return DGR_OK;
+}
+
 int dgr_build_coord_maps(DgrArena &arena, const int32_t *coords, int64_t N, DgrMapSet *ms,
                          hipStream_t stream);
 int dgr_build_half_buckets(DgrArena &arena, DgrCoordMap *cm, DgrHalfBuckets *hb, int levels, int renumber_from, hipStream_t stream);
 
 int dgr_build_maps(DgrArena &arena, const int32_t *coords, int64_t N, int D, int conv1_ks,
-                   DgrMapSet *ms, hipStream_t stream, bool skip_conv1_map, bool lean, bool nbr_tables) {
+                   DgrMapSet *ms, hipStream_t stream, bool skip_conv1_map, bool lean, bool nbr_tables, bool nbr_lists) {
   DGR_REQUIRE(D == 3 || D == 6, "D=%d not supported (the DGR path uses D=3 and D=6)", D);
   DGR_REQUIRE(conv1_ks % 2 == 1 && conv1_ks >= 1, "conv1 kernel size must be odd");
   DGR_REQUIRE(N > 0 && N < (1ll << 30), "N=%lld out of range", (long long)N);
@@ -874,6 +996,11 @@
       cls_fill_kernel<<<dim3((unsigned)max_nb, 3), KM_THREADS, 0, stream>>>(cj);
       DGR_LAUNCH_CHECK();
     }
+    if (lean && nbr_lists) {
+      const NbrListSpec specs[3] = {{&ms->nsame[2], &ms->cm[2], &ms->same[2]}, {&ms->nsame[3], &ms->cm[3], &ms->same[3]},
+                                    {&ms->ndown[2], &ms->cm[3], &ms->down[2]}};
+      DGR_CHECK(build_nbr_lists3(arena, specs, 3, stream));
+    }
     if (lean) {
       if (conv1_ks != 3 && !skip_conv1_map)
         DGR_CHECK(build_kernel_map3(arena, ms->cm[0], ms->cm[0], conv1_ks, 1024, false, false, true, &ms->conv1, ms->overflow,
@@ -916,7 +1043,9 @@
 static int maps_create(dgr_ctx *ctx, const int32_t *coords, int64_t N, int D, int conv1_kernel_size, int flags,
                        dgr_maps **out, dgr_stream stream_) {
   DGR_REQUIRE(ctx && coords && out, "dgr_maps_create: NULL argument");
-  DGR_REQUIRE((flags & ~DGR_MAPS_LEAN) == 0, "dgr_maps_create_ex: unknown flags 0x%x", flags);
+  DGR_REQUIRE((flags & ~(DGR_MAPS_LEAN | DGR_MAPS_NBR_LISTS)) == 0, "dgr_maps_create_ex: unknown flags 0x%x", flags);
+  DGR_REQUIRE(!(flags & DGR_MAPS_NBR_LISTS) || ((flags & DGR_MAPS_LEAN) && D == 3),
+              "dgr_maps_create_ex: DGR_MAPS_NBR_LISTS goes with DGR_MAPS_LEAN and D = 3");
   const bool lean = (flags & DGR_MAPS_LEAN) != 0;
   const bool skip_conv1_map = lean && D == 3;
   hipStream_t stream = (hipStream_t)stream_;
@@ -930,7 +1059,8 @@
     if (!m->coords_copy) { rc = DGR_ENOMEM; break; }
     if (hipMemcpyAsync(m->coords_copy, coords, (size_t)N * (D + 1) * sizeof(int32_t),
                        hipMemcpyDeviceToDevice, stream) != hipSuccess) { rc = DGR_EHIP; break; }
-    rc = dgr_build_maps(m->arena, m->coords_copy, N, D, conv1_kernel_size, &m->ms, stream, skip_conv1_map, lean, D == 3);
+    rc = dgr_build_maps(m->arena, m->coords_copy, N, D, conv1_kernel_size, &m->ms, stream, skip_conv1_map, lean, D == 3,
+                        (flags & DGR_MAPS_NBR_LISTS) != 0);
     if (rc != DGR_OK) break;
     int32_t flag = 0;
     if (hipMemcpyAsync(&flag, m->ms.overflow, sizeof(int32_t), hipMemcpyDeviceToHost, stream) != hipSuccess ||
diff --git a/deepglobalregistration_amd/csrc/net.hip b/deepglobalregistration_amd/csrc/net.hip
--- a/deepglobalregistration_amd/csrc/net.hip
+++ b/deepglobalregistration_amd/csrc/net.hip
@@ -95,6 +95,7 @@
   std::map<std::string, DgrTensorRef> inter;
   std::map<std::string, DgrTensorRec> tensors;
   uint64_t run_generation = 0;
+  bool wide_coarse = false;
 };
 
 static int round_up(int v, int m) { return (v + m - 1) / m * m; }
@@ -231,7 +232,10 @@
   const float w_scale = ldexpf(1.f, 15 - ex);
   L.w_unscale = ldexpf(1.f, ex - 15);
   const bool use_wide = K > 1 && !dgr_exact_f32() && dgr_conv_wide_supported(L.cin_pad, cin, cout) && !(net->D == 3 && K == 27);
-  if (use_wide) {
+  const bool transposed = name.size() > 3 && name.compare(name.size() - 3, 3, "_tr") == 0;
+  const bool wide3 = net->D == 3 && K == 27 && net->cin <= 8 && net->conv1_ks <= 7 && !transposed && !dgr_exact_f32() &&
+                     cin >= 128 && cout >= 128 && dgr_conv_wide_supported(L.cin_pad, cin, cout);
+  if (use_wide || wide3) {
     const int S16 = cin / 16, NB32 = cout / 32;
     L.wb_piece = (int64_t)K * S16 * NB32 * 64;
     const int64_t ne = L.wb_piece * 8;
@@ -248,7 +252,8 @@
       dst[ne + o] = dgr_f16_bits_dev(xs - dgr_f16_val_dev(xs));
     }));
     W.param_bytes += (size_t)2 * ne * sizeof(uint16_t);
-  } else {
+  }
+  if (!use_wide) {
     const int S = L.cin_pad / 8, NBLK = L.cout_pad / 32;
     const int64_t ne = (int64_t)K * S * NBLK * 256;
     DGR_CHECK(W.alloc(&L.w, ne));
@@ -422,7 +427,15 @@
   net->D = src->D; net->cin = src->cin; net->cout = src->cout;
   net->conv1_ks = src->conv1_ks; net->normalize = src->normalize;
   net->W = src->W;
+  net->wide_coarse = src->wide_coarse;
   *out = net;
+  return DGR_OK;
+}
+
+extern "C" int dgr_net_set_wide_coarse(dgr_net *net, int on) {
+  DGR_REQUIRE(net, "dgr_net_set_wide_coarse: NULL argument");
+  DGR_REQUIRE(net->D == 3 || !on, "dgr_net_set_wide_coarse: a D = 3 option (the 6-D net runs its wide layers rule-major anyway)");
+  net->wide_coarse = on != 0;
   return DGR_OK;
 }
 
@@ -439,6 +452,7 @@
   uint32_t *amax = nullptr, *amax2 = nullptr;
   unsigned char *dsplit = nullptr;
   bool dsplit_only = false;
+  bool split_pending = false, amax_pending = false;
 };
 
 struct Fwd {
@@ -448,6 +462,7 @@
   DgrMapSet ms;
   bool prof;
   bool l2_next = false;
+  bool wide3 = false;
 
   float *ybuf = nullptr;
 
@@ -461,7 +476,8 @@
     a.y = ybuf; a.shift = L.shift;
     a.w = L.w;
     a.cin = L.cin; a.cin_pad = L.cin_pad; a.cout = L.cout; a.cout_pad = L.cout_pad; a.K = L.K;
-    if (km && ms.use_nbr) {
+    const bool wide3_layer = wide3 && km && ms.use_nbr && L.wb && !swapped && km->built;
+    if (km && ms.use_nbr && !wide3_layer) {
       a.pair_in = a.pair_out = a.tile_ptr = a.rule_ptr = nullptr;
       a.tile_desc = nullptr; a.n_rows_dev = nullptr; a.tile_bound = 0;
     } else if (km) {
@@ -487,7 +503,7 @@
       if (!e0 || !em || !e1) return DGR_EHIP;
       DGR_HIP_CHECK(hipEventRecord(e0, stream));
     }
-    if (km && ms.use_nbr) {
+    if (km && ms.use_nbr && !wide3_layer) {
       const DgrNbrTable *t = nullptr;
       for (int l = 0; l < 4; ++l)
         if (km == &ms.same[l]) t = &ms.nsame[l];
@@ -507,6 +523,8 @@
       o.w_unscale = L.w_unscale; o.n_in_cap = cin_map.n_cap;
       if (L.w16b && !dgr_exact_f32()) {
         o.row_amax = in.amax;
+        if (in.amax && in.amax_pending)
+          DGR_CHECK(dgr_row_amax(in.ptr, in.ld, L.cin, in.relu, cin_map.n_dev, cin_map.n_cap, in.amax, stream));
         if (!o.row_amax) {
           uint32_t *mx;
           DGR_ALLOC(mx, ctx->arena, uint32_t, cin_map.n_cap);
@@ -559,6 +577,8 @@
                                    out.ptr, out.ld, stream));
     else if (wide) {
       DGR_REQUIRE(in.split.planes, "layer %s: the wide-layer kernel needs its input as split rows", L.name.c_str());
+      if (in.split_pending)
+        DGR_CHECK(dgr_split_rows(in.ptr, in.ld, in.relu, cin_map.n_dev, cin_map.n_cap, in.split, stream));
       if (prof) {
         DGR_ALLOC(a.clk, ctx->arena, unsigned long long, 2);
         DGR_HIP_CHECK(hipMemsetAsync(a.clk, 0xff, sizeof(unsigned long long), stream));
@@ -618,7 +638,9 @@
   f.ms.overflow = ctx->flag_dev;
   const bool use_nbr = net->D == 3 && net->cin <= 8 && net->conv1_ks <= 7;
   const bool conv1_fused = use_nbr;
-  DGR_CHECK(dgr_build_maps(A, coords, N, net->D, net->conv1_ks, &f.ms, stream, conv1_fused, true, use_nbr));
+  static const bool no_wide3 = getenv("DGR_NO_WIDE3") != nullptr || getenv("DGR_OS_LISTS") != nullptr;
+  f.wide3 = net->wide_coarse && use_nbr && !no_wide3 && !dgr_exact_f32() && net->W->layers[7].wb && 27 * N * 256 * (int64_t)sizeof(float) <= (16ll << 30);
+  DGR_CHECK(dgr_build_maps(A, coords, N, net->D, net->conv1_ks, &f.ms, stream, conv1_fused, true, use_nbr, f.wide3));
   if (f.prof) {
     DGR_HIP_CHECK(hipEventRecord(m1, stream));
     (net->D == 3 ? ctx->map3_spans : ctx->map6_spans).push_back({m0, m1});
@@ -627,8 +649,8 @@
     const DgrMapSet &m = f.ms;
     int64_t need = m.use_nbr ? 64 : m.conv1.pair_cap * 32;
     const int64_t same_c[4] = {64, 64, 128, 256}, down_c[3] = {64, 128, 256};
-    for (int l = 0; l < 4; ++l) need = std::max(need, m.same[l].pair_cap * same_c[l]);
-    for (int l = 0; l < 3; ++l) need = std::max(need, m.down[l].pair_cap * down_c[l]);
+    for (int l = 0; l < 4; ++l) if (m.same[l].built) need = std::max(need, m.same[l].pair_cap * same_c[l]);
+    for (int l = 0; l < 3; ++l) if (m.down[l].built) need = std::max(need, m.down[l].pair_cap * down_c[l]);
     DGR_ALLOC(f.ybuf, A, float, need);
   }
   const DgrMapSet &ms = f.ms;
@@ -666,7 +688,7 @@
         {&V4, 14, 128, n4, true}, {&U2, 16, 64, n2, false}, {&V2, 17, 64, n2, true}, {&U1, 19, 64, n1, false},
         {&V1, 20, 64, n1, true}};
     for (auto &e : sp) {
-      if (!net->W->layers[e.consumer].wb) continue;
+      if (!net->W->layers[e.consumer].wb || (net->D == 3 && !f.wide3)) continue;
       e.t->split.channels = e.channels;
       e.t->split_only = e.middle;
       DGR_ALLOC(e.t->split.planes, A, unsigned char, (size_t)e.rows * 4 * e.channels);
@@ -689,6 +711,12 @@
     for (Tensor *t : {&T8, &Y8, &S8}) t->amax = take(n8);
     S2.amax2 = CAT2.amax; S2T.amax2 = CAT2.amax;
     S4.amax2 = CAT4.amax; S4T.amax2 = CAT4.amax;
+    if (f.wide3) {
+      for (Tensor *t : {&Y4, &S4, &T8, &Y8, &V4}) t->amax = nullptr;
+      S4.amax2 = S4T.amax2 = nullptr;
+      S8.amax_pending = CAT4.amax_pending = true;
+      T4.split_pending = U4.split_pending = true;
+    }
   }
 
   if (use_nbr && !getenv("DGR_NO_DSPLIT")) {
@@ -919,7 +947,7 @@
   const int64_t n_cap = f.ms.cm[0].n_cap;
   if (!f.ms.use_nbr) DGR_ALLOC(f.ybuf, A, float, f.ms.same[0].pair_cap * L.cout);
   Tensor tin{const_cast<float *>(in), L.cin, in_relu}, tout{out, L.cout, 0};
-  if (L.wb) {
+  if (L.wb && !f.ms.use_nbr) {
     tin.split.channels = L.cin;
     DGR_ALLOC(tin.split.planes, A, unsigned char, (size_t)n_cap * 4 * L.cin);
     DGR_ALLOC(tin.split.scale, A, float, n_cap);
diff --git a/deepglobalregistration_amd/model/resunet.py b/deepglobalregistration_amd/model/resunet.py
--- a/deepglobalregistration_amd/model/resunet.py
+++ b/deepglobalregistration_amd/model/resunet.py
@@ -77,12 +77,13 @@
             share = getattr(self, '_share', None)
             if share is not None:
                 self._net = ops.NetHandle(None, self.D, self.in_channels, self.out_channels, self.conv1_kernel_size,
-                                          self.normalize_feature, self.device, share_from=share._net)
+                                          self.normalize_feature, self.device, share_from=share._net, wide_coarse=self.D == 3)
                 return self._net
             if self._state is None:
                 raise RuntimeError('load_state_dict() must be called before the first forward')
             self._net = ops.NetHandle(self._state, self.D, self.in_channels, self.out_channels,
-                                      self.conv1_kernel_size, self.normalize_feature, self.device)
+                                      self.conv1_kernel_size, self.normalize_feature, self.device,
+                                      wide_coarse=self.D == 3)
         return self._net
 
     def forward(self, x):
diff --git a/deepglobalregistration_amd/ops.py b/deepglobalregistration_amd/ops.py
--- a/deepglobalregistration_amd/ops.py
+++ b/deepglobalregistration_amd/ops.py
@@ -48,8 +48,9 @@
 class NetHandle:
 
     def __init__(self, state_dict, D, in_channels, out_channels, conv1_kernel_size,
-                 normalize_feature, device='cuda', share_from=None):
+                 normalize_feature, device='cuda', share_from=None, wide_coarse=False):
         lib = _lib.load()
+        self.wide_coarse = bool(wide_coarse)
         self.device = torch.device(device)
         self.D, self.cin, self.cout = D, in_channels, out_channels
         self.conv1_ks, self.normalize = int(conv1_kernel_size), bool(normalize_feature)
@@ -61,6 +62,7 @@
             with torch.cuda.device(self.device):
                 check(lib.dgr_net_share(get_ctx(self.device), share_from.handle, C.byref(h)))
             self.handle = h
+            check(lib.dgr_net_set_wide_coarse(h, int(self.wide_coarse)))
             return
         keep, descs = [], []
         items = [(n, t) for n, t in state_dict.items() if not n.endswith('num_batches_tracked')]
@@ -87,6 +89,8 @@
                          conv1_kernel_size, int(bool(normalize_feature)), arr, len(descs),
                          C.byref(h)))
         self.handle = h
+        if self.wide_coarse:
+            check(lib.dgr_net_set_wide_coarse(h, 1))
 
     def __del__(self):
         try:
@@ -177,15 +181,17 @@
 
 class Maps:
 
-    def __init__(self, coords, D, conv1_kernel_size=3, device='cuda', lean=False):
+    def __init__(self, coords, D, conv1_kernel_size=3, device='cuda', lean=False, nbr_lists=False):
         lib = _lib.load()
         self.device = torch.device(device)
         coords = _as(coords, torch.int32, self.device)
         self.D, self.lean = D, bool(lean)
         h = vp()
         if lean:
-            check(lib.dgr_maps_create_ex(get_ctx(self.device), ptr(coords), coords.shape[0], D, conv1_kernel_size, 1,
-                                         C.byref(h), stream_ptr(self.device.index)))
+            check(lib.dgr_maps_create_ex(get_ctx(self.device), ptr(coords), coords.shape[0], D, conv1_kernel_size,
+                                         1 | (2 if nbr_lists else 0), C.byref(h), stream_ptr(self.device.index)))
+        elif nbr_lists:
+            raise ValueError('nbr_lists goes with lean=True')
         else:
             check(lib.dgr_maps_create(get_ctx(self.device), ptr(coords), coords.shape[0], D, conv1_kernel_size,
                                       C.byref(h), stream_ptr(self.device.index)))
diff --git a/include/dgr_hip.h b/include/dgr_hip.h
--- a/include/dgr_hip.h
+++ b/include/dgr_hip.h
@@ -54,6 +54,7 @@
 int64_t dgr_net_param_bytes(const dgr_net *net);
 int dgr_net_share(dgr_ctx *ctx, const dgr_net *src, dgr_net **out);
 int dgr_net_sharers(const dgr_net *net);
+int dgr_net_set_wide_coarse(dgr_net *net, int on);
 
 int dgr_resunet_forward(dgr_ctx *ctx, dgr_net *net, const int32_t *coords, const float *feats,
                         int64_t N, float *out, dgr_stream stream);
@@ -78,6 +79,7 @@
                             int32_t *pair_in, int32_t *pair_out, int64_t pair_cap, int64_t *K,
                             int64_t *P);
 #define DGR_MAPS_LEAN 1
+#define DGR_MAPS_NBR_LISTS 2
 int dgr_maps_create_ex(dgr_ctx *ctx, const int32_t *coords, int64_t N, int D, int conv1_kernel_size, int flags,
                        dgr_maps **out, dgr_stream stream);
 int dgr_maps_get_raw(dgr_maps *maps, const char *kind, int ts, const char *field, void *host_out,
```
